# alshai/pfbwt-f

Hardware: AMD Instinct MI355X
Metric: Gbases/s end-to-end BWT+SA build; bit-exact .bwt/.sa vs reference (higher is better)
Workload: dtype u8 text / u32 indices / u64 hash; 1 GPU; S-32G; L=32000000, H=1000, seed=1000, w=10, p=100, flags=-r, uint_t=64, n=32000010000, r=83625322, input=text resident in HBM, outputs (.bwt, .ssa, .esa) left in HBM, per_rank=single GPU

## Files before the change

### include/pfbwt_hip_dev.h

```cpp
#ifndef PFBWT_HIP_DEV_H
#define PFBWT_HIP_DEV_H
#include "pfbwt_hip.h"

#ifdef __cplusplus
extern "C" {
#endif

int pfp_profile_enable(pfp_ctx *ctx, int on);
int pfp_profile_select(pfp_ctx *ctx, const char *kernel_name);
int pfp_profile_reset(pfp_ctx *ctx);
int pfp_profile_get(pfp_ctx *ctx, int idx, const char **name, uint64_t *launches, double *ms, double *bytes);
int pfp_stage_ms(pfp_ctx *ctx, double out[3]);
int pfp_debug_set(pfp_ctx *ctx, const char *key, long long value);
int pfp_debug_sort(pfp_ctx *ctx, uint64_t n, int bits, int reps, double *ms_out, uint32_t *unsorted_pairs);
int pfp_debug_checksum(pfp_ctx *ctx, const void *d_buf, uint64_t bytes, uint64_t global_offset, uint64_t out[2]);

int pfp_debug_check_sample_order(pfp_ctx *ctx, uint64_t out[5]);
int pfp_debug_check_sa(pfp_ctx *ctx, uint64_t out[5]);
int pfp_debug_check_samples(pfp_ctx *ctx, uint64_t out[3]);
int pfp_debug_rows_windowed(pfp_ctx *ctx, uint64_t window_rows, void *host_sa, void *host_lcp);
int pfp_debug_wordsum(pfp_ctx *ctx, const void *d_buf, uint64_t bytes, uint64_t out[2]);

#ifdef __cplusplus
}
#endif
#endif
```

### pfbwt-f_amd/csrc/common.h

```cpp
#pragma once
#include <hip/hip_runtime.h>
#include <cstdint>
#include <cstdio>
#include <cstdlib>
#include <cstring>
#include <chrono>
#include <string>
#include <vector>
#include "../../include/pfbwt_hip.h"
#include "devmem.h"
#include "../../include/pfbwt_hip_dev.h"

namespace pfp {

typedef uint32_t idx_t;

constexpr int BLOCK = 256;
constexpr int WAVE = 64;

constexpr uint8_t Dollar = 2, EndOfWord = 1, EndOfDict = 0;

enum KernelId {
    K_TRIGGER_SCAN, K_PHRASE_ENDS, K_PHRASE_HASH, K_PHRASE_HASH_LONG, K_DEDUP_HEADS, K_DEDUP_LONG,
    K_DICT_BUILD, K_RADIX_HIST, K_RADIX_SCATTER, K_SCAN_REDUCE, K_SCAN_SPINE, K_SCAN_APPLY,
    K_SS_INIT_KEYS, K_SS_HEADS, K_SS_MAKE_KEYS, K_SS_WRITE_RANK, K_SS_FLAG_ACTIVE, K_COMPACT,
    K_WORD_RANK, K_PARSE_RANKS, K_DICT_SORTED, K_PBWT_ROWS, K_EMIT_COUNT, K_EMIT, K_RUNS, K_SAMPLES, K_MISC, K_EMIT_BIG, K_FILL, K_CLASS_SORT, K_FASTA, K_EMIT_LARGE, K_REC_PARSE, K_REC_DEDUP, K_REC_ASSEMBLE, K_DOC, K_LCP_PAIRS, K_LCP_LONG, K_LCP_GATHER, K_THR_TILES, K_THR_QUERIES, K_THR_LONG, K_PLCP_BUILD, K_LCP_SPARSE, K_RUN_MASKS, K_MS_INDEX, K_MS_POINTERS, K_MS_BREAKS, K_MS_LONG, K_MS_FILL,
    K_COUNT_
};
static const char *const kernel_names[K_COUNT_] = {
    "trigger_scan", "phrase_ends", "phrase_hash", "phrase_hash_long", "dedup_heads", "dedup_long",
    "dict_build", "radix_hist", "radix_scatter", "scan_reduce", "scan_spine", "scan_apply",
    "ss_init_keys", "ss_heads", "ss_make_keys", "ss_write_rank", "ss_flag_active", "compact",
    "word_rank", "parse_ranks", "dict_sorted", "pbwt_rows", "emit_count", "emit", "runs", "samples", "misc", "emit_big", "fill", "class_sort", "fasta_strip", "emit_large", "rec_parse", "rec_dedup", "rec_assemble", "doc_array", "lcp_pairs", "lcp_long", "lcp_gather", "thr_tiles", "thr_queries", "thr_long", "plcp_build", "lcp_sparse", "run_masks", "ms_index", "ms_pointers", "ms_breaks", "ms_long", "ms_fill"};

struct ProfRec { uint64_t launches = 0; double ms = 0, bytes = 0; };

struct Arena {
    VmRegion vm;
    char *base = nullptr;
    size_t cap = 0, lo = 0, hi = 0, want = 0;
    size_t peak_lo = 0, peak_hi_bytes = 0;
    bool failed = false;
    void reset() { lo = 0; hi = cap; failed = false; }
    void *alloc_lo(size_t bytes)
    {
        size_t a = (lo + 255) & ~(size_t)255;
        if (a + bytes > hi || !vm.commit(a, a + bytes)) { failed = true; want += bytes; return nullptr; }
        lo = a + bytes; if (lo > peak_lo) peak_lo = lo;
        return base + a;
    }
    void *alloc_hi(size_t bytes)
    {
        size_t b = (bytes + 255) & ~(size_t)255;
        if (b > hi || hi - b < lo || !vm.commit(hi - b, hi)) { failed = true; want += bytes; return nullptr; }
        hi -= b; if (cap - hi > peak_hi_bytes) peak_hi_bytes = cap - hi;
        return base + hi;
    }
    void *reserve_lo(size_t bytes)
    {
        size_t a = (lo + 255) & ~(size_t)255;
        if (a + bytes > hi) { failed = true; want += bytes; return nullptr; }
        lo = a + bytes;
        return base + a;
    }
    bool commit_range(const void *p, size_t bytes) { const size_t o = (size_t)((const char *)p - base); return vm.commit(o, o + bytes); }
    size_t offset_of(const void *p) const { return (size_t)((const char *)p - base); }
    size_t mark_hi() const { return hi; }
    void release_hi(size_t m) { hi = m; }
    size_t mark_lo() const { return lo; }
    void release_lo(size_t m) { lo = m; }
};

struct ResultSlot {
    void *p[3] = {nullptr, nullptr, nullptr};
    size_t lo_mark = (size_t)-1, lo_end = 0;
};
struct MsIndex {
    void *thr = nullptr, *lfhead = nullptr; uint8_t *head = nullptr; uint32_t *sorted = nullptr, *sym = nullptr, *dir = nullptr;
    uint32_t B = 0;
};

struct Tunables {
    int verbose = 0;
    int seg_grid = 768;
    int seg_stage = 1;
    int sort_k = 0;
    int sort_no_table = 0;
    uint32_t class_sort_maxrange = 0;
    int dedup_table_log2 = 0;
    int no_trigger_table = 0;
    uint64_t emit_chunk_rows = 3ULL << 30;
    uint32_t fill_subs = 2;
    int fill_masks = 1;
    int fill_skip = 1;
    uint64_t sample_cap = ~0ULL;
    int no_runaware = 0;
    long big_group_members = -2;
    int force_wide_rows = 0;
    uint64_t ingest_block_bytes = 0;
    int expand_dma = 1;
    int ingest_readers = 0;
    uint32_t emit_group_rows = 4096;
    int dict_text_rounds = -1;
    int force_run_round = 0;
    int int_key_symbols = 3;
    int no_slot_records = 0;
    int group_reduce = 1;
    uint64_t fasta_chunk_bytes = 0;
    int parse_rec = -1;
    int parse_rec_p2 = 4;
    uint64_t parse_rec_min = 1u << 21;
    int parse_rec_depth = 1;
    uint32_t parse_rec_tile_rows = 0;
    int dict_rec = -1;
    int dict_rec_p2 = 16;
    int dedup_variant = -1;
    int64_t dedup_period = 0;
    int64_t dedup_chunk = 0;
    int dedup_packed = 1;
    int scan_waves = 16;
    int dedup_phases = 0;
    int parse_rec_table_log2 = 0;
    uint32_t doc_lds_max = 8192;
    uint32_t lcp_long_min = 512;
    uint32_t thr_long_min = 128;
    uint32_t thr_tile = 1024;
    uint64_t thr_window_rows = 1ULL << 30;
    int ms_dir_log2 = -1;
    uint32_t ms_long_min = 512;
    int plcp_block_log2 = -1;
};

}

struct pfp_ctx {
    int w = 10; uint64_t p = 100; unsigned flags = 0; int device = 0;
    hipStream_t stream = nullptr;
    pfp::Arena arena;
    size_t arena_request = 0;
    uint64_t err_pos = 0; int err_ch = 0;
    pfp::VmRegion text;
    uint8_t *tb = nullptr; size_t tb_cap = 0; uint64_t n = 0; uint64_t text_hint = 0; uint64_t nseq = 0 ;
    struct RowViewPending { const uint8_t *src = nullptr; uint64_t count = 0, len = 0, stride = 0; } view;
    uint64_t left_ctx = 0;
    uint64_t tb_n = 0;
    int stage = 0;
    uint64_t m = 0, dwords = 0, dsize = 0;
    uint64_t *d_ye = nullptr;
    uint32_t *d_pid = nullptr;
    uint32_t *d_parse = nullptr;
    uint8_t *d_last = nullptr;
    uint8_t *d_dict = nullptr;
    uint32_t *d_ws = nullptr;
    uint32_t *d_wordid = nullptr;
    uint32_t *d_wrank = nullptr;
    uint32_t *d_occ = nullptr;
    uint8_t *d_sdict = nullptr;
    uint32_t *d_gsa = nullptr;
    uint8_t *d_sflag = nullptr;
    uint32_t *d_srank = nullptr;
    uint2 *d_grank = nullptr;
    bool gsa_valid = false;
    uint64_t nrows = 0;
    uint8_t *d_bwlast = nullptr; uint32_t *d_ilist = nullptr; uint64_t *d_bwsai = nullptr;
    uint8_t *d_bwl_il = nullptr;
    uint64_t nout = 0, runs = 0, esa_pairs = 0, easy = 0, hard = 0, slice_begin = 0, slice_rows = 0;
    uint8_t *d_bwt = nullptr; void *d_sa = nullptr; void *d_ssa = nullptr; void *d_esa = nullptr;
    bool have_sa = false, have_rssa = false;
    pfp::ResultSlot ma; uint64_t ma_words = 0;
    pfp::ResultSlot da;
    pfp::ResultSlot lcp;
    pfp::ResultSlot thr;
    pfp::ResultSlot msi; pfp::MsIndex msx;
    pfp::ResultSlot ms; uint64_t ms_patterns = 0, ms_bases = 0;
    std::vector<uint64_t> ms_off;
    size_t lo_after_parse = 0, lo_after_pbwt = 0, emit_scratch_mark = 0;
    bool prof_on = false; uint64_t prof_mask = ~0ULL;
    pfp::ProfRec prof[pfp::K_COUNT_];
    struct PendingEv { hipEvent_t a, b; int id; double bytes; };
    std::vector<PendingEv> pending;
    std::vector<hipEvent_t> ev_pool;
    double stage_ms[3] = {0, 0, 0};
    int hip_err = 0;
    uint8_t *hstage[2] = {nullptr, nullptr}; hipEvent_t hstage_ev[2] = {nullptr, nullptr}; bool hstage_used[2] = {false, false};
    pfp::Tunables tun;
    struct FastaIngest {
        uint8_t *raw[2] = {nullptr, nullptr}; size_t rawcap = 0; bool used[2] = {false, false};
        hipStream_t copy = nullptr; bool copy_ready = false; hipEvent_t ev_copied[2] = {nullptr, nullptr}, ev_free[2] = {nullptr, nullptr};
        uint8_t *tiles = nullptr; size_t tiles_cap = 0;
        unsigned long long *d_tot = nullptr, *h_tot = nullptr;
        uint32_t state = 2; bool started = false; uint64_t records = 0;
        std::vector<uint64_t> rec_raw, rec_pos;
    } fa;
    uint8_t *h_bwt = nullptr; void *h_sa = nullptr;
    uint8_t *ing_buf[16] = {};
    uint64_t ing_next_off = 0;
    std::vector<std::string> doc_names; std::vector<uint64_t> doc_starts;
    uint64_t hash_seed = 0x9E3779B97F4A7C15ULL;
    int num_cus = 0;
    uint32_t *d_trigtab = nullptr;
};

namespace pfp {

inline hipEvent_t ev_get(pfp_ctx *c)
{
    if (!c->ev_pool.empty()) { hipEvent_t e = c->ev_pool.back(); c->ev_pool.pop_back(); return e; }
    hipEvent_t e; (void)hipEventCreate(&e); return e;
}
inline void prof_collect(pfp_ctx *c)
{
    if (c->pending.empty()) return;
    (void)hipStreamSynchronize(c->stream);
    for (auto &pe : c->pending) {
        float ms = 0; (void)hipEventElapsedTime(&ms, pe.a, pe.b);
        c->prof[pe.id].launches++; c->prof[pe.id].ms += ms; c->prof[pe.id].bytes += pe.bytes;
        c->ev_pool.push_back(pe.a); c->ev_pool.push_back(pe.b);
    }
    c->pending.clear();
}
struct ProfScope {
    pfp_ctx *c; int id; double bytes; hipEvent_t a = nullptr; bool on = false;
    ProfScope(pfp_ctx *c_, int id_, double bytes_) : c(c_), id(id_), bytes(bytes_)
    {
        on = c->prof_on && ((c->prof_mask >> id) & 1ULL);
        if (on) { a = ev_get(c); (void)hipEventRecord(a, c->stream); }
    }
    ~ProfScope()
    {
        if (on) {
            hipEvent_t b = ev_get(c); (void)hipEventRecord(b, c->stream);
            c->pending.push_back({a, b, id, bytes});
            if (c->pending.size() > 4096) prof_collect(c);
        }
    }
};

#define PFP_LAUNCH(ctx, id, bytes, kernel, grid, ...)                                             \
    do {                                                                                          \
        pfp::ProfScope ps_((ctx), (id), (double)(bytes));                                         \
        if ((ctx)->tun.verbose >= 3) { fprintf(stderr, "[pfbwt_hip] launch %s grid %u\n", #kernel, (unsigned)(grid)); fflush(stderr); } \
        hipLaunchKernelGGL(kernel, dim3((unsigned)(grid)), dim3(pfp::BLOCK), 0, (ctx)->stream, __VA_ARGS__); \
        hipError_t le_ = hipGetLastError();             \
        if ((ctx)->tun.verbose >= 3 && le_ == hipSuccess) le_ = hipStreamSynchronize((ctx)->stream);    \
        if (le_ != hipSuccess) { (ctx)->hip_err = (int)le_; (ctx)->err_ch = (int)le_;                 \
            fprintf(stderr, "[pfbwt_hip] launch of %s failed: %s (%s:%d)\n", #kernel, hipGetErrorString(le_), __FILE__, __LINE__); \
            return PFP_E_HIP; }                                                                       \
    } while (0)

#define PFP_LAUNCH_B(ctx, id, bytes, kernel, grid, block, ...)                                    \
    do {                                                                                          \
        pfp::ProfScope ps_((ctx), (id), (double)(bytes));                                         \
        hipLaunchKernelGGL(kernel, dim3((unsigned)(grid)), dim3((unsigned)(block)), 0, (ctx)->stream, __VA_ARGS__); \
        hipError_t le_ = hipGetLastError();                                                       \
        if (le_ != hipSuccess) { (ctx)->hip_err = (int)le_; (ctx)->err_ch = (int)le_;                 \
            fprintf(stderr, "[pfbwt_hip] launch of %s failed: %s (%s:%d)\n", #kernel, hipGetErrorString(le_), __FILE__, __LINE__); \
            return PFP_E_HIP; }                                                                       \
    } while (0)

#define PFP_HIP(ctx, expr)                                                                        \
    do {                                                                                          \
        hipError_t e_ = (expr);                                                                   \
        if (e_ != hipSuccess) { (ctx)->hip_err = (int)e_; (ctx)->err_ch = (int)e_;                \
            fprintf(stderr, "[pfbwt_hip] %s failed: %s (%s:%d)\n", #expr, hipGetErrorString(e_), __FILE__, __LINE__); \
            return PFP_E_HIP; }                                                                   \
    } while (0)

#define PFP_TRY(expr) do { int rc_ = (expr); if (rc_ != PFP_OK) return rc_; } while (0)

#define PFP_ALLOC_HI(ctx, ptr, T, count)                                                          \
    do { (ptr) = (T *)(ctx)->arena.alloc_hi(sizeof(T) * (size_t)((count) ? (count) : 1));         \
         if (!(ptr)) return PFP_E_NOMEM; } while (0)
#define PFP_ALLOC_LO(ctx, ptr, T, count)                                                          \
    do { (ptr) = (T *)(ctx)->arena.alloc_lo(sizeof(T) * (size_t)((count) ? (count) : 1));         \
         if (!(ptr)) return PFP_E_NOMEM; } while (0)

inline unsigned nblocks(uint64_t items, uint64_t per_block) { return (unsigned)((items + per_block - 1) / per_block); }
inline int bits_for(uint64_t maxval) { int b = 1; while (b < 64 && (maxval >> b)) ++b; return b; }

struct PostResult {
    pfp_ctx *c; ResultSlot &s; size_t mark;
    PostResult(pfp_ctx *c_, ResultSlot &s_) : c(c_), s(s_)
    {
        if (s.lo_mark != (size_t)-1 && c->arena.lo == s.lo_end) c->arena.release_lo(s.lo_mark);
        s = ResultSlot();
        mark = c->arena.mark_lo();
    }
    void commit(void *p0, void *p1 = nullptr, void *p2 = nullptr) { s.p[0] = p0; s.p[1] = p1; s.p[2] = p2; s.lo_mark = mark; s.lo_end = c->arena.mark_lo(); }
};
inline void drop_post_results(pfp_ctx *c) { c->ma = c->da = c->lcp = c->thr = c->msi = c->ms = ResultSlot(); c->ma_words = 0; c->msx = MsIndex(); c->ms_patterns = c->ms_bases = 0; c->ms_off.clear(); }

struct HostTimer {
    std::chrono::steady_clock::time_point t0 = std::chrono::steady_clock::now();
    double ms() const { return std::chrono::duration<double, std::milli>(std::chrono::steady_clock::now() - t0).count(); }
};

}
```

### pfbwt-f_amd/csrc/emit.h

```cpp
#pragma once
#include "prims.h"
#include "parse.h"

namespace pfp {

__global__ __launch_bounds__(BLOCK) void k_pbwt_pack(const uint32_t *P, const uint8_t *last, const tpos_t *sai, uint64_t m, uint4 *rec)
{
    const uint64_t j = (uint64_t)blockIdx.x * BLOCK + threadIdx.x;
    if (j >= m) return;
    const uint64_t v = sai ? (uint64_t)sai[j] : 0ULL;
    rec[j] = make_uint4((uint32_t)v, (uint32_t)(v >> 32), P[j], (uint32_t)last[j ? j - 1 : m - 1]);
}
constexpr int BWL_SHIFT = 29;
__device__ __forceinline__ uint32_t bwl_code(uint32_t c) { return c == 0 ? 0u : c == Dollar ? 1u : c == '-' ? 2u : c == 'A' ? 3u : c == 'C' ? 4u : c == 'G' ? 5u : c == 'N' ? 6u : c == 'T' ? 7u : 8u; }
__device__ __forceinline__ uint8_t bwl_byte(uint32_t code) { return code == 0 ? (uint8_t)0 : code == 1 ? Dollar : code == 2 ? (uint8_t)'-' : code == 3 ? (uint8_t)'A' : code == 4 ? (uint8_t)'C' : code == 5 ? (uint8_t)'G' : code == 6 ? (uint8_t)'N' : (uint8_t)'T'; }
__global__ __launch_bounds__(BLOCK) void k_pbwt_rows(const uint32_t *SAP, const uint4 *rec, uint64_t m, uint8_t *bwlast, tpos_t *bwsai, uint32_t *W, uint32_t *rowid, int pack, uint32_t *bad)
{
    const uint64_t i = (uint64_t)blockIdx.x * BLOCK + threadIdx.x;
    if (i > m) return;
    const uint32_t s = SAP[i];
    if (s == 0) { bwlast[i] = 0; if (bwsai) bwsai[i] = 0; W[i] = 0; rowid[i] = (uint32_t)i; return; }
    const uint4 R = rec[s - 1];
    bwlast[i] = (uint8_t)R.w;
    if (bwsai) bwsai[i] = (tpos_t)(((uint64_t)R.y << 32) | R.x);
    W[i] = R.z;
    uint32_t id = (uint32_t)i;
    if (pack) { const uint32_t code = bwl_code(R.w & 0xFFu); if (code > 7u) *bad = 1u; else id |= code << BWL_SHIFT; }
    rowid[i] = id;
}
__global__ __launch_bounds__(BLOCK) void k_ilist_split(const uint32_t *packed, uint64_t n, uint32_t *ilist, uint8_t *bwl_il)
{
    const uint64_t k = (uint64_t)blockIdx.x * BLOCK + threadIdx.x;
    if (k >= n) return;
    const uint32_t v = packed[k];
    ilist[k] = v & ((1u << BWL_SHIFT) - 1u); bwl_il[k] = bwl_byte(v >> BWL_SHIFT);
}
__global__ __launch_bounds__(BLOCK) void k_bwsai_by_ilist(const uint32_t *ilist, const tpos_t *bwsai, uint64_t n, tpos_t *out)
{
    const uint64_t k = (uint64_t)blockIdx.x * BLOCK + threadIdx.x;
    if (k < n) out[k] = bwsai[ilist[k]];
}
__global__ __launch_bounds__(BLOCK) void k_ilist_gather(const uint32_t *packed, uint64_t n, uint32_t mask, const uint8_t *bwlast, uint32_t *ilist, uint8_t *bwl_il)
{
    const uint64_t k = (uint64_t)blockIdx.x * BLOCK + threadIdx.x;
    if (k >= n) return;
    const uint32_t q = packed[k] & mask;
    ilist[k] = q; bwl_il[k] = bwlast[q];
}

__global__ __launch_bounds__(BLOCK) void k_u32_add_store(const uint32_t *in, uint64_t n, uint32_t add, uint32_t *out)
{
    const uint64_t i = (uint64_t)blockIdx.x * BLOCK + threadIdx.x;
    if (i < n) out[i] = in[i] + add;
}

__global__ __launch_bounds__(BLOCK) void k_wordstart_keys(const uint32_t *ws, const uint2 *grank, uint64_t dwords, uint32_t *keys, uint32_t *vals)
{
    const uint64_t id = (uint64_t)blockIdx.x * BLOCK + threadIdx.x;
    if (id >= dwords) return;
    keys[id] = grank[ws[id]].x; vals[id] = (uint32_t)id;
}
__global__ __launch_bounds__(BLOCK) void k_word_rank(const uint32_t *sorted_ids, uint64_t dwords, const uint32_t *occw, uint32_t *wrank, uint32_t *idofrank, uint32_t *occ)
{
    const uint64_t r = (uint64_t)blockIdx.x * BLOCK + threadIdx.x;
    if (r >= dwords) return;
    const uint32_t id = sorted_ids[r];
    wrank[id] = (uint32_t)r; idofrank[r] = id; occ[r] = occw[id];
}
constexpr int WF_PER_THREAD = 16, WF_TILE = BLOCK * WF_PER_THREAD;
__device__ __forceinline__ uint32_t wf_mask16(const uint8_t *sflag, uint64_t i0, uint64_t n)
{
    uint32_t m = 0;
#pragma unroll
    for (int k = 0; k < WF_PER_THREAD; ++k) if (i0 + k < n && sflag[i0 + k]) m |= 1u << k;
    return m;
}
__global__ __launch_bounds__(BLOCK) void k_flag_tile_count(const uint8_t *sflag, uint64_t n, uint32_t *tilecnt)
{
    __shared__ uint32_t red[4];
    const uint64_t i0 = ((uint64_t)blockIdx.x * BLOCK + threadIdx.x) * WF_PER_THREAD;
    uint32_t tot;
    (void)block_excl_sum((uint32_t)__popc(wf_mask16(sflag, i0, n)), red, &tot);
    if (threadIdx.x == 0) tilecnt[blockIdx.x] = tot;
}
__global__ __launch_bounds__(BLOCK) void k_word_rank_flags(const uint8_t *sflag, const uint32_t *tilebase, const uint32_t *SA, const uint32_t *wordid, uint64_t dsize, uint32_t dwords,
                                                         const uint32_t *occw, uint32_t *wrank, uint32_t *idofrank, uint32_t *occ)
{
    __shared__ uint32_t red[4];
    const uint64_t i0 = ((uint64_t)blockIdx.x * BLOCK + threadIdx.x) * WF_PER_THREAD;
    uint32_t m = wf_mask16(sflag, i0, dsize), tot;
    uint32_t r = tilebase[blockIdx.x] + block_excl_sum((uint32_t)__popc(m), red, &tot);
    while (m) {
        const int k = __ffs((int)m) - 1; m &= m - 1;
        const uint32_t id = wordid[SA[i0 + k]];
        if (r < dwords && id < dwords) { wrank[id] = r; idofrank[r] = id; occ[r] = occw[id]; }
        ++r;
    }
}
__global__ __launch_bounds__(BLOCK) void k_parse_ranks(const uint32_t *pid, const uint32_t *wrank, uint64_t m, uint32_t *parse)
{
    const uint64_t j = (uint64_t)blockIdx.x * BLOCK + threadIdx.x;
    if (j < m) parse[j] = wrank[pid[j]] + 1u;
}
__global__ __launch_bounds__(BLOCK) void k_sorted_lengths(const uint32_t *ws, const uint32_t *idofrank, uint64_t dwords, uint32_t *len1, tpos_t *srcstart)
{
    const uint64_t r = (uint64_t)blockIdx.x * BLOCK + threadIdx.x;
    if (r >= dwords) return;
    const uint32_t id = idofrank[r];
    len1[r] = ws[id + 1] - ws[id]; srcstart[r] = ws[id];
}

__global__ __launch_bounds__(BLOCK) void k_eow_flags(const uint8_t *D, uint64_t dsize, uint32_t *flag)
{
    const uint64_t x = (uint64_t)blockIdx.x * BLOCK + threadIdx.x;
    if (x < dsize) flag[x] = D[x] == EndOfWord ? 1u : 0u;
}
__global__ __launch_bounds__(BLOCK) void k_ws_from_flags(const uint8_t *D, uint64_t dsize, const uint32_t *wordid, uint32_t *ws)
{
    const uint64_t x = (uint64_t)blockIdx.x * BLOCK + threadIdx.x;
    if (x >= dsize) return;
    if (x == 0) ws[0] = 0;
    if (D[x] == EndOfWord) ws[wordid[x] + 1] = (uint32_t)x + 1u;
}

struct EmitArgs {
    const uint8_t *D = nullptr; uint64_t dsize = 0; uint32_t dwords = 0; int w = 0;
    const uint32_t *SA = nullptr, *ws = nullptr, *wrank = nullptr , *occ = nullptr, *F = nullptr, *ilist = nullptr;
    const uint32_t *srank = nullptr;
    const tpos_t *bwsai = nullptr;
    const uint2 *posinfo = nullptr;
    const uint4 *prec = nullptr;
    const uint32_t *wordid = nullptr;
    int use_prec = 0;
    int use_e0 = 0;
    const uint4 *winfo = nullptr;
    const uint8_t *bwlast = nullptr;
    const uint8_t *bwl_il = nullptr;
    const tpos_t *bwsai_il = nullptr;
    const void *EB = nullptr;
    const uint32_t *s_sl = nullptr;
    const uint32_t *s_fb = nullptr;
    const uint8_t *s_fl = nullptr;
    const uint8_t *s_pc = nullptr;
    const uint32_t *s_g0 = nullptr;
    const uint32_t *gk = nullptr;
    const void *cnt = nullptr;
    const uint4 *sinfo = nullptr;
    const uint32_t *tile_slot = nullptr;
    uint64_t *big_keys = nullptr; uint32_t *big_vals = nullptr; unsigned long long *big_count = nullptr;
    uint64_t big_cap = 0, big_total = 0;
    uint64_t nout = 0, n = 0;
    uint64_t e0 = 0, e1 = 0;
    uint64_t w0 = 0, w1 = 0;
    const void *ENB = nullptr; const uint32_t *etile_slot = nullptr, *elist = nullptr, *cpos = nullptr; uint32_t ecount = 0; int special = 0; uint64_t q0 = 0;
    const uint32_t *qspec = nullptr;
    const uint32_t *gqf = nullptr, *gql = nullptr;
    uint8_t *gleft = nullptr, *tile_left = nullptr; uint32_t group_rows_cap = 0; uint32_t rank_members_max = 0;
    const uint4 *cinfo = nullptr;
    const unsigned long long *cgb = nullptr;
    const uint32_t *town = nullptr;
    uint32_t *lglist = nullptr; unsigned long long *lgcount = nullptr; uint64_t lgcap = 0; int qpasses = 0 ;
    unsigned long long *gstat = nullptr;
};
constexpr uint8_t SF_MULTI = 1, SF_FULL = 2, SF_BIG = 4, SF_GFULL = 8, SF_NONUNI = 16, SF_E0 = 32;
__device__ __forceinline__ bool slot_is_special(uint32_t fl) { return (fl & (SF_FULL | SF_GFULL | SF_NONUNI)) != 0; }
constexpr int EG_SLOTS = 2 * BLOCK;
constexpr uint32_t BIG_GROUP_MEMBERS = 64;
constexpr uint32_t WID_MASK = 0x0FFFFFFFu;
__device__ __forceinline__ uint32_t dict_code4(uint32_t c) { return c <= 2 ? c : (c == '-') ? 3u : (c == 'A') ? 4u : (c == 'C') ? 5u : (c == 'G') ? 6u : (c == 'N') ? 7u : 8u; }
__device__ __forceinline__ uint8_t dict_byte4(uint32_t code) { return code <= 2 ? (uint8_t)code : code == 3 ? (uint8_t)'-' : code == 4 ? (uint8_t)'A' : code == 5 ? (uint8_t)'C' : code == 6 ? (uint8_t)'G' : code == 7 ? (uint8_t)'N' : (uint8_t)'T'; }
__global__ __launch_bounds__(BLOCK) void k_pack_winfo(const uint32_t *ws, const uint32_t *wrank , const uint32_t *occ, const uint32_t *F, uint64_t dwords, uint4 *winfo)
{
    const uint64_t id = (uint64_t)blockIdx.x * BLOCK + threadIdx.x;
    if (id >= dwords) return;
    const uint32_t rk = wrank ? wrank[id] : (uint32_t)id;
    winfo[id] = make_uint4(ws[id], ws[id + 1] - 1u, F[rk], occ[rk]);
}
__global__ __launch_bounds__(BLOCK) void k_pack_posinfo(const uint8_t *D, const uint32_t *wordid, uint64_t dsize, uint2 *posinfo)
{
    const uint64_t x = (uint64_t)blockIdx.x * BLOCK + threadIdx.x;
    if (x >= dsize) return;
    posinfo[x] = make_uint2(wordid[x] | (dict_code4(x ? D[x - 1] : 0u) << 28), 0u);
}

constexpr uint32_t PREC_SL_BITS = 26, PREC_FULL = 1u << 30, PREC_VALID = 1u << 31;
__global__ __launch_bounds__(BLOCK) void k_pack_prec(const uint8_t *D, const uint32_t *wordid, const uint4 *winfo, uint64_t dsize, uint32_t dwords, uint4 *prec, const tpos_t *bwsai_il )
{
    const uint64_t x = (uint64_t)blockIdx.x * BLOCK + threadIdx.x;
    if (x >= dsize) return;
    const uint32_t id = wordid[x];
    uint4 R = make_uint4(0u, 0u, 0u, 0u);
    if (id < dwords) {
        const uint4 W = winfo[id];
        uint32_t code = 0, full = 0;
        if ((uint32_t)x == W.x) full = PREC_FULL;
        else { code = dict_code4(D[x - 1]); if (code == Dollar && (uint32_t)x - 1u == W.x) code = 0; }
        R.y = W.z; R.z = W.w; R.w = (W.y - (uint32_t)x) | (code << PREC_SL_BITS) | full | PREC_VALID;
        if (bwsai_il) { if (W.w == 1u) R.x = (uint32_t)bwsai_il[W.z]; }
        else R.x = id;
    }
    prec[x] = R;
}
__global__ __launch_bounds__(BLOCK) void k_pack_wpq(const uint32_t *ilist, const uint32_t *wrank , const uint32_t *occ, const uint32_t *F, uint64_t dwords, uint2 *wpq)
{
    const uint64_t id = (uint64_t)blockIdx.x * BLOCK + threadIdx.x;
    if (id >= dwords) return;
    const uint32_t rk = wrank ? wrank[id] : (uint32_t)id, o = occ[rk], f = F[rk];
    wpq[id] = o ? make_uint2(ilist[f], ilist[f + o - 1u]) : make_uint2(~0u, 0u);
}
__global__ __launch_bounds__(BLOCK) void k_max_word_length(const uint32_t *ws, uint64_t dwords, uint32_t *out)
{
    __shared__ uint32_t red[4];
    const uint64_t id = (uint64_t)blockIdx.x * BLOCK + threadIdx.x;
    uint32_t tot;
    (void)block_incl_max(id < dwords ? ws[id + 1] - ws[id] : 0u, red, &tot);
    if (threadIdx.x == 0) atomicMax(out, tot);
}

__device__ __forceinline__ uint32_t word_rank_of(const EmitArgs &a, uint32_t id) { return a.wrank ? a.wrank[id] : id; }

template <typename T> __device__ __forceinline__ uint32_t upper_bound_t(const T *a, uint32_t n, T x)
{
    uint32_t lo = 0, hi = n;
    while (lo < hi) { uint32_t mid = lo + ((hi - lo) >> 1); if (a[mid] <= x) lo = mid + 1; else hi = mid; }
    return lo;
}

template <typename EBT> __global__ __launch_bounds__(BLOCK) void k_emit_slots(EmitArgs a, EBT *cnt, unsigned long long *hard_rows, uint32_t *s_sl, uint32_t *s_fb, uint8_t *s_fl, uint8_t *s_pc,
                                                                             uint32_t *s_g0, uint32_t *gk , uint8_t *gfl ,
                                                                             uint8_t *gnu ,
                                                                             const uint2 *wpq , uint32_t *gqf, uint32_t *gql)
{
    __shared__ uint8_t hd[BLOCK + 1];
    __shared__ uint8_t pcl[BLOCK + 1];
    __shared__ uint32_t red[4];
    const uint64_t i = (uint64_t)blockIdx.x * BLOCK + threadIdx.x;
    const bool valid = i < a.dsize;
    uint32_t x = 0; uint2 P = make_uint2(0, 0); uint4 R = make_uint4(0, 0, 0, 0);
    if (valid) { x = a.SA[i]; if (a.prec) R = a.prec[x]; else P = a.posinfo[x]; P.y = a.srank[i]; }
    hd[threadIdx.x] = (valid && P.y == (uint32_t)i) ? 1 : 0;
    if (threadIdx.x == 0) {
        const uint64_t nx = (uint64_t)(blockIdx.x + 1) * BLOCK;
        uint8_t h = 1, hp = 0xFF;
        if (nx < a.dsize) {
            const uint32_t xn = a.SA[nx];
            if (a.prec) {
                const uint4 Rn = a.prec[xn];
                h = a.srank[nx] == (uint32_t)nx ? 1 : 0;
                if (!h && (Rn.w & PREC_VALID) && !(Rn.w & PREC_FULL)) hp = dict_byte4((Rn.w >> PREC_SL_BITS) & 15u);
            } else {
            const uint2 Pn = a.posinfo[xn];
            h = a.srank[nx] == (uint32_t)nx ? 1 : 0;
            if (!h) {
                const uint32_t idn = Pn.x & WID_MASK;
                if (idn < a.dwords) {
                    const uint32_t wsn = a.winfo[idn].x;
                    if (xn != wsn) { hp = dict_byte4(Pn.x >> 28); if (hp == Dollar && xn - 1 == wsn) hp = 0; }
                }
            }
            }
        }
        hd[BLOCK] = h; pcl[BLOCK] = hp;
    }
    __syncthreads();
    uint32_t c = 0, sl = 0, fb = 0; uint8_t fl = 0, pc = 0;
    if (a.prec) {
        if (valid && (R.w & PREC_VALID)) {
            sl = R.w & ((1u << PREC_SL_BITS) - 1u);
            if (sl > (uint32_t)a.w) {
                c = R.z; fb = R.y;
                if (!hd[threadIdx.x] || (i + 1 < a.dsize && !hd[threadIdx.x + 1])) fl |= SF_MULTI;
                if (R.w & PREC_FULL) fl |= SF_FULL; else pc = dict_byte4((R.w >> PREC_SL_BITS) & 15u);
                if (a.use_e0 && c == 1u && !(fl & SF_MULTI)) { fl |= SF_E0; P.y = R.x; }
            }
        }
    } else {
    const uint32_t id = P.x & WID_MASK;
    if (valid && id < a.dwords) {
        const uint4 W = a.winfo[id];
        const uint32_t wsid = W.x;
        sl = W.y - x;
        if (sl > (uint32_t)a.w) {
            c = W.w; fb = W.z;
            if (!hd[threadIdx.x] || (i + 1 < a.dsize && !hd[threadIdx.x + 1])) fl |= SF_MULTI;
            if (x == wsid) fl |= SF_FULL;
            else { pc = dict_byte4(P.x >> 28); if (pc == Dollar && x - 1 == wsid) pc = 0; }
        }
    }
    }
    pcl[threadIdx.x] = (fl & SF_FULL) ? (uint8_t)0xFF : pc;
    __syncthreads();
    if (valid) {
        cnt[i] = (EBT)c; s_sl[i] = sl; s_fb[i] = fb; s_fl[i] = fl; s_pc[i] = pc; s_g0[i] = P.y;
        if (fl & SF_MULTI) {
            const bool lastm = i + 1 >= a.dsize || hd[threadIdx.x + 1];
            if (lastm) gk[P.y] = (uint32_t)i - P.y + 1u;
            if (fl & SF_FULL) gfl[P.y] = 1;
            else if (!lastm && pcl[threadIdx.x + 1] != 0xFF && pcl[threadIdx.x + 1] != pc) gnu[P.y] = 1;
        }
    }
    if (wpq && !(a.prec && a.use_e0)) {
        __shared__ uint32_t wk0[BLOCK / WAVE], wkl[BLOCK / WAVE], wmn[BLOCK / WAVE], wmx[BLOCK / WAVE];
        __shared__ uint8_t wef[BLOCK / WAVE], wsp[BLOCK / WAVE];
        const int lane = (int)(threadIdx.x & (WAVE - 1)), wv = (int)(threadIdx.x / WAVE);
        const bool part = (fl & SF_MULTI) != 0;
        uint32_t key = ~0u, mn = ~0u, mx = 0u, ef = 0u;
        if (part) {
            const uint2 q = wpq[a.prec ? R.x : (P.x & WID_MASK)];
            key = P.y; mn = q.x; mx = q.y; ef = (i + 1 >= a.dsize || hd[threadIdx.x + 1]) ? 1u : 0u;
        }
        for (int d = 1; d < WAVE; d <<= 1) {
            const uint32_t k2 = __shfl_down(key, (unsigned)d), n2 = __shfl_down(mn, (unsigned)d), x2 = __shfl_down(mx, (unsigned)d), e2 = __shfl_down(ef, (unsigned)d);
            if (lane + d < WAVE && k2 == key) { mn = n2 < mn ? n2 : mn; mx = x2 > mx ? x2 : mx; ef = e2; }
        }
        const uint32_t klast = __shfl(key, WAVE - 1), kprev = __shfl_up(key, 1u);
        if (lane == 0) { wk0[wv] = key; wmn[wv] = mn; wmx[wv] = mx; wef[wv] = (uint8_t)ef; wsp[wv] = key == klast ? 1 : 0; }
        if (lane == WAVE - 1) wkl[wv] = key;
// ... 228 lines not shown
    const uint32_t lo = a.tile_slot[tb], hi = a.tile_slot[tb + 1];
    return lo + upper_bound_t<EBT>(EB + lo, hi - lo + 1u, (EBT)o) - 1u;
}

template <typename SAT, typename EBT> __global__ __launch_bounds__(BLOCK) void k_emit(EmitArgs a, uint8_t *bwt, SAT *sa, uint32_t *qrow )
{
    __shared__ uint32_t eb[EMIT_LDS_SLOTS];
    __shared__ uint32_t rs[EMIT_TILE];
    __shared__ uint32_t red[4];
    const EBT *EB = reinterpret_cast<const EBT *>(a.EB);
    const EBT *ENB = reinterpret_cast<const EBT *>(a.ENB);
    if (a.tile_left && !a.tile_left[blockIdx.x]) return;
    const uint64_t tb = a.e0 / EMIT_TILE + blockIdx.x;
    const uint64_t o0 = tb * EMIT_TILE > a.e0 ? tb * EMIT_TILE : a.e0;
    const uint64_t o1 = ((tb + 1) * EMIT_TILE < a.e1) ? (tb + 1) * EMIT_TILE : a.e1;
    const uint32_t i0 = a.etile_slot[tb], i1 = a.etile_slot[tb + 1];
    const uint32_t ns = i1 - i0 + 1u;
    const uint64_t ebase = (uint64_t)ENB[i0];
    const bool in_lds = ns <= (uint32_t)EMIT_LDS_SLOTS && o1 - ebase < 0xFFFFFFFFULL;
    if (in_lds) for (uint32_t k = threadIdx.x; k < ns; k += BLOCK) eb[k] = (uint32_t)((uint64_t)ENB[i0 + k] - ebase);
    for (int k = threadIdx.x; k < EMIT_TILE; k += BLOCK) rs[k] = 0;
    __syncthreads();
    if (in_lds) {
        const uint32_t rel0 = (uint32_t)(o0 - ebase), nrow = (uint32_t)(o1 - o0);
        for (uint32_t t = threadIdx.x; t < ns; t += BLOCK) {
            const uint32_t e = eb[t];
            if (e <= rel0) atomicMax(&rs[0], t);
            else if (e - rel0 < nrow) atomicMax(&rs[e - rel0], t);
        }
        __syncthreads();
        uint32_t loc[EMIT_PER_THREAD], run = 0;
#pragma unroll
        for (int j = 0; j < EMIT_PER_THREAD; ++j) { const uint32_t v = rs[threadIdx.x * EMIT_PER_THREAD + j]; run = v > run ? v : run; loc[j] = run; }
        uint32_t tot;
        const uint32_t inc = block_incl_max(run, red, &tot);
        uint32_t prev = __shfl_up(inc, 1);
        if ((threadIdx.x & 63) == 0) prev = 0;
        __shared__ uint32_t wmax[BLOCK / WAVE];
        if ((threadIdx.x & 63) == 63) wmax[threadIdx.x >> 6] = inc;
        __syncthreads();
        if ((threadIdx.x & 63) == 0 && threadIdx.x) prev = wmax[(threadIdx.x >> 6) - 1];
#pragma unroll
        for (int j = 0; j < EMIT_PER_THREAD; ++j) rs[threadIdx.x * EMIT_PER_THREAD + j] = loc[j] > prev ? loc[j] : prev;
        __syncthreads();
    }
#pragma unroll 1
    for (int k = 0; k < EMIT_PER_THREAD; k += EMIT_ROWS_IN_FLIGHT) {
        uint64_t o[EMIT_ROWS_IN_FLIGHT]; uint32_t i[EMIT_ROWS_IN_FLIGHT], r[EMIT_ROWS_IN_FLIGHT], q[EMIT_ROWS_IN_FLIGHT];
        uint4 S[EMIT_ROWS_IN_FLIGHT]; uint8_t fl[EMIT_ROWS_IN_FLIGHT]; bool on[EMIT_ROWS_IN_FLIGHT]; uint64_t sv[EMIT_ROWS_IN_FLIGHT];
#pragma unroll
        for (int u = 0; u < EMIT_ROWS_IN_FLIGHT; ++u) {
            o[u] = o0 + (uint64_t)(k + u) * BLOCK + threadIdx.x;
            on[u] = o[u] < o1;
            const uint64_t oo = on[u] ? o[u] : o0;
            if (in_lds) { const uint32_t j = rs[(uint32_t)(oo - o0)]; i[u] = i0 + j; r[u] = (uint32_t)(oo - ebase) - eb[j]; }
            else { i[u] = upper_bound_t<EBT>(ENB, a.ecount, (EBT)oo) - 1u; r[u] = (uint32_t)(oo - (uint64_t)ENB[i[u]]); }
        }
        uint32_t jc[EMIT_ROWS_IN_FLIGHT];
#pragma unroll
        for (int u = 0; u < EMIT_ROWS_IN_FLIGHT; ++u) jc[u] = i[u];
        if (a.elist) {
#pragma unroll
            for (int u = 0; u < EMIT_ROWS_IN_FLIGHT; ++u) i[u] = a.elist[i[u]];
        }
#pragma unroll
        for (int u = 0; u < EMIT_ROWS_IN_FLIGHT; ++u) { S[u] = a.sinfo[i[u]]; fl[u] = (uint8_t)(S[u].w >> 24); }
        if (a.gleft) {
#pragma unroll
            for (int u = 0; u < EMIT_ROWS_IN_FLIGHT; ++u) {
                const uint32_t jh = (fl[u] & SF_MULTI) ? jc[u] - (i[u] - S[u].z) : jc[u];
                if (on[u] && !a.gleft[jh]) on[u] = false;
            }
        }
#pragma unroll
        for (int u = 0; u < EMIT_ROWS_IN_FLIGHT; ++u) {
            const bool needq = (fl[u] & SF_MULTI) || qrow || ((fl[u] & SF_FULL) && !a.bwl_il) || (sa && !a.bwsai_il);
            q[u] = needq ? a.ilist[S[u].x + r[u]] : 0u;
        }
#pragma unroll
        for (int u = 0; u < EMIT_ROWS_IN_FLIGHT; ++u) sv[u] = (sa && on[u] && !(fl[u] & SF_BIG)) ? ((fl[u] & SF_E0) ? (uint64_t)S[u].z : a.bwsai_il ? (uint64_t)a.bwsai_il[S[u].x + r[u]] : (uint64_t)a.bwsai[q[u]]) : 0ULL;
        uint32_t before[EMIT_ROWS_IN_FLIGHT], gk_[EMIT_ROWS_IN_FLIGHT], maxk = 0;
#pragma unroll
        for (int u = 0; u < EMIT_ROWS_IN_FLIGHT; ++u) {
            const bool plain = on[u] && (fl[u] & SF_MULTI) && !(fl[u] & (SF_GFULL | SF_BIG));
            gk_[u] = plain ? (S[u].w & 0xFFFFFFu) : 0u; before[u] = 0;
            maxk = gk_[u] > maxk ? gk_[u] : maxk;
        }
        for (uint32_t s0 = 0; s0 < maxk; s0 += EMIT_RANK_W) {
            uint32_t mem[EMIT_ROWS_IN_FLIGHT * EMIT_RANK_W], qq[EMIT_ROWS_IN_FLIGHT * EMIT_RANK_W], res[EMIT_ROWS_IN_FLIGHT * EMIT_RANK_W];
#pragma unroll
            for (int u = 0; u < EMIT_ROWS_IN_FLIGHT; ++u)
#pragma unroll
                for (int j = 0; j < EMIT_RANK_W; ++j) {
                    const uint32_t s = S[u].z + s0 + j;
                    mem[u * EMIT_RANK_W + j] = (s0 + j < gk_[u] && s != i[u]) ? s : ~0u; qq[u * EMIT_RANK_W + j] = q[u];
                }
            rank_lists<EMIT_ROWS_IN_FLIGHT * EMIT_RANK_W>(a, mem, qq, res);
#pragma unroll
            for (int u = 0; u < EMIT_ROWS_IN_FLIGHT; ++u)
#pragma unroll
                for (int j = 0; j < EMIT_RANK_W; ++j) before[u] += res[u * EMIT_RANK_W + j];
        }
#pragma unroll
        for (int u = 0; u < EMIT_ROWS_IN_FLIGHT; ++u) {
            const bool self_full = (fl[u] & SF_FULL) != 0;
            uint64_t pos = o[u];
            bool full_emits_eow = false;
            const bool big = on[u] && (fl[u] & SF_BIG) != 0;
            {
                const unsigned long long bm = __ballot(big);
                if (bm) {
                    const int lane = threadIdx.x & 63, leader = __ffsll((long long)bm) - 1;
                    unsigned long long basei = 0;
                    if (lane == leader) basei = atomicAdd(a.big_count, (unsigned long long)__popcll(bm));
                    basei = __shfl(basei, leader);
                    if (big) {
                        const unsigned long long idx = basei + (unsigned long long)__popcll(bm & (lane ? (~0ULL >> (64 - lane)) : 0ULL));
                        if (idx < a.big_cap) { a.big_keys[idx] = ((uint64_t)S[u].z << 32) | q[u]; a.big_vals[idx] = i[u]; }
                        else a.big_count[1] = 1;
                    }
                }
            }
            if (!on[u] || big) continue;
            uint32_t g = i[u];
            if (fl[u] & SF_GFULL) { pos = multi_group_pos<EBT>(a, i[u], r[u], q[u], self_full, &full_emits_eow); g = S[u].z; }
            else if (fl[u] & SF_MULTI) { pos = (uint64_t)EB[S[u].z] + before[u] + r[u]; g = S[u].z; }
            else if (a.special) pos = (uint64_t)EB[i[u]] + r[u];
            if (a.special && qrow) qrow[(uint64_t)ENB[a.cpos[g]] - a.q0 + (pos - (uint64_t)EB[g])] = q[u];
            const uint8_t c = self_full ? (full_emits_eow ? (uint8_t)EndOfWord : a.bwl_il ? a.bwl_il[S[u].x + r[u]] : a.bwlast[q[u]]) : a.s_pc[i[u]];
            if (pos < a.w0 || pos >= a.w1) continue;
            bwt[pos - a.w0] = c;
            if (sa) {
                SAT v = (SAT)((SAT)sv[u] - (SAT)a.s_sl[i[u]]);
                if (pos == 0) v = (SAT)a.n;
                sa[pos - a.w0] = v;
            }
            if (qrow && !a.special) qrow[pos - a.w0] = q[u];
        }
    }
}

constexpr int EG_BUF = 4096, EG_PER_THREAD = EG_BUF / BLOCK;
constexpr int EG1_BUF = 8192, EG2_BUF = 16384;
__device__ __forceinline__ uint32_t group_members(const EmitArgs &a, const uint4 &S) { const uint32_t k = S.w & 0xFFFFFFu; return k == 0xFFFFFFu ? a.gk[S.z] : k; }
template <typename EBT> __global__ __launch_bounds__(BLOCK) void k_special_pack(EmitArgs a, uint32_t nsp, uint4 *cinfo, unsigned long long *cgb)
{
    const uint64_t j = (uint64_t)blockIdx.x * BLOCK + threadIdx.x;
    if (j >= nsp) return;
    const uint32_t i = a.elist[j]; const uint4 S = a.sinfo[i];
    const uint32_t fl = S.w >> 24; const bool multi = (fl & SF_MULTI) != 0;
    cinfo[j] = make_uint4(S.x, multi ? group_members(a, S) : 1u, multi ? i - S.z : 0u, (uint32_t)a.s_pc[i] | (fl << 8));
    cgb[j] = (unsigned long long)reinterpret_cast<const EBT *>(a.EB)[multi ? S.z : i];
}
template <typename EBT> __device__ __forceinline__ uint64_t group_start_at_or_after(const EBT *ENB, const uint4 *cinfo, uint64_t nsp, uint64_t lo, uint64_t v)
{
    while (lo < nsp && (uint64_t)ENB[lo] < v) ++lo;
    if (lo >= nsp) return nsp;
    const uint4 ci = cinfo[lo];
    if (!((ci.w >> 8) & SF_MULTI)) return lo;
    const uint64_t head = lo - ci.z;
    return (uint64_t)ENB[head] < v ? head + ci.y : head;
}
template <typename EBT> __global__ __launch_bounds__(BLOCK) void k_tile_own(const EBT *ENB, const uint4 *cinfo, const uint32_t *etile_slot, uint64_t nsp, uint64_t ntiles, uint32_t *town)
{
    const uint64_t t = (uint64_t)blockIdx.x * BLOCK + threadIdx.x;
    if (t > ntiles) return;
    town[t] = (uint32_t)group_start_at_or_after<EBT>(ENB, cinfo, nsp, etile_slot[t], t * EMIT_TILE);
}
template <typename EBT> __global__ __launch_bounds__(BLOCK) void k_emit_groups(EmitArgs a, uint8_t *bwt, uint32_t *qrow)
{
    __shared__ uint32_t LQ[EG_BUF];
    __shared__ uint32_t s_eb[EG_SLOTS + 1], s_fb[EG_SLOTS], s_kf[EG_SLOTS], s_dl[EG_SLOTS];
    __shared__ uint64_t s_ob[EG_SLOTS];
    __shared__ uint8_t s_pc[EG_SLOTS];
    __shared__ uint32_t red[4];
    __shared__ uint64_t jb[2];
    const EBT *ENB = reinterpret_cast<const EBT *>(a.ENB);
    const uint64_t tile0 = a.e0 / EMIT_TILE, tb = tile0 + blockIdx.x;
    const uint64_t o0 = tb * EMIT_TILE > a.e0 ? tb * EMIT_TILE : a.e0;
    const uint64_t o1 = ((tb + 1) * EMIT_TILE < a.e1) ? (tb + 1) * EMIT_TILE : a.e1;
    if (threadIdx.x < 2) {
        const uint64_t v = threadIdx.x ? o1 : o0;
        const uint64_t tv = threadIdx.x ? tb + 1 : tb;
        uint64_t j;
        if (v == tv * EMIT_TILE) j = a.town[tv];
        else {
            uint64_t lo = a.etile_slot[tb], hi = (uint64_t)a.etile_slot[tb + 1] + 1u;
            if (hi > a.ecount) hi = a.ecount;
            if (lo > hi) lo = hi;
            while (lo < hi) { const uint64_t mid = lo + ((hi - lo) >> 1); if ((uint64_t)ENB[mid] < v) lo = mid + 1; else hi = mid; }
            j = group_start_at_or_after<EBT>(ENB, a.cinfo, a.ecount, lo, v);
        }
        jb[threadIdx.x] = j;
    }
    __syncthreads();
    uint64_t j = jb[0]; const uint64_t jE = jb[1];
    const uint32_t cap = a.group_rows_cap < (uint32_t)EG_BUF ? a.group_rows_cap : (uint32_t)EG_BUF;
    while (j < jE) {
        const uint32_t nload = jE - j < (uint64_t)EG_SLOTS ? (uint32_t)(jE - j) : (uint32_t)EG_SLOTS;
        const uint64_t B0 = (uint64_t)ENB[j];
        uint32_t cand[2] = {0u, 0u}, bad = 0xFFFFFFFFu;
#pragma unroll
        for (int t = 0; t < 2; ++t) {
            const uint32_t s = threadIdx.x + (uint32_t)t * BLOCK;
            if (s < nload) {
                const uint4 ci = a.cinfo[j + s];
                const uint32_t fl = ci.w >> 8, dl = ci.z, k = ci.y;
                const uint64_t e0 = (uint64_t)ENB[j + s] - B0, e1 = (uint64_t)ENB[j + s + 1] - B0;
                s_eb[s] = e0 < 0xFFFFFFFFull ? (uint32_t)e0 : 0xFFFFFFFFu;
                if (s + 1 == nload) s_eb[nload] = e1 < 0xFFFFFFFFull ? (uint32_t)e1 : 0xFFFFFFFFu;
                s_fb[s] = ci.x; s_kf[s] = (k < 0xFFFFFFu ? k : 0xFFFFFFu) | (fl << 24); s_dl[s] = dl; s_pc[s] = (uint8_t)ci.w;
                s_ob[s] = (uint64_t)a.cgb[j + s];
                if (((fl & (SF_GFULL | SF_BIG)) || k > a.rank_members_max) && s < bad) bad = s;
                if (dl + 1u == k && e1 <= (uint64_t)cap) cand[t] = s + 1u;
            }
        }
        uint32_t tot;
        (void)block_incl_max(~bad, red, &tot);
        const uint32_t firstbad = ~tot;
        uint32_t c = 0;
#pragma unroll
        for (int t = 0; t < 2; ++t) if (cand[t] && cand[t] <= firstbad && cand[t] > c) c = cand[t];
        uint32_t cut;
        (void)block_incl_max(c, red, &cut);
        if (cut == 0) {
            const uint32_t k0 = a.cinfo[j].y;
            const uint64_t r0 = B0, r1 = (uint64_t)ENB[j + k0];
            {
                const uint32_t f0 = s_kf[0] >> 24;
                if (threadIdx.x == 0) {
                    unsigned long long idx = ~0ULL;
                    if (a.lglist && (f0 & SF_MULTI) && !(f0 & (SF_GFULL | SF_BIG)) && k0 <= (uint32_t)EG_SLOTS && r1 - r0 <= (uint64_t)EG2_BUF) {
                        const int big = r1 - r0 > (uint64_t)EG1_BUF ? 1 : 0;
                        idx = atomicAdd(a.lgcount + big, 1ULL);
                        if (idx < a.lgcap) a.lglist[(uint64_t)big * a.lgcap + idx] = (uint32_t)j;
                    }
                    jb[0] = idx < a.lgcap ? 1 : 0;
                }
                __syncthreads();
                const bool taken = jb[0] != 0;
                __syncthreads();
                if (taken) { j += k0; continue; }
            }
            if (threadIdx.x == 0) a.gleft[j] = 1;
            if (a.gstat && threadIdx.x == 0) {
                const uint32_t f0 = s_kf[0] >> 24;
                atomicAdd(&a.gstat[(f0 & SF_GFULL) ? 0 : (f0 & SF_BIG) ? 1 : (r1 - r0 > (uint64_t)cap) ? 2 : 3], (unsigned long long)(r1 - r0));
                int b = 0; while (b < 7 && (1024ull << (2 * b)) <= r1 - r0) ++b;
                atomicAdd(&a.gstat[4 + b], (unsigned long long)(r1 - r0));
            }
            if (r1 > r0) for (uint64_t t = r0 / EMIT_TILE + threadIdx.x; t <= (r1 - 1) / EMIT_TILE; t += BLOCK) a.tile_left[t - tile0] = 1;
            j += k0;
            __syncthreads();
            continue;
        }
        __syncthreads();
        const uint32_t nrows = s_eb[cut];
#pragma unroll
        for (int t = 0; t < 2; ++t) { const uint32_t s = threadIdx.x + (uint32_t)t * BLOCK; if (s < cut) s_ob[s] -= (uint64_t)s_eb[s - s_dl[s]]; }
        uint32_t qv[EG_PER_THREAD], sv[EG_PER_THREAD]; uint8_t cv[EG_PER_THREAD];
#pragma unroll
        for (int it = 0; it < EG_PER_THREAD; ++it) {
            const uint32_t r = threadIdx.x + (uint32_t)it * BLOCK;
            sv[it] = 0; qv[it] = 0; cv[it] = 0;
            if (r < nrows) {
                const uint32_t s = upper_bound_t<uint32_t>(s_eb, cut, r) - 1u, at = s_fb[s] + (r - s_eb[s]);
                sv[it] = s; qv[it] = a.ilist[at];
                if (!((s_kf[s] >> 24) & SF_MULTI) && a.bwl_il) cv[it] = a.bwl_il[at];
            }
        }
#pragma unroll
        for (int it = 0; it < EG_PER_THREAD; ++it) {
            const uint32_t r = threadIdx.x + (uint32_t)it * BLOCK;
            if (r < nrows) { LQ[r] = qv[it]; const uint32_t fl = s_kf[sv[it]] >> 24; if (fl & SF_MULTI) cv[it] = s_pc[sv[it]]; else if (!a.bwl_il) cv[it] = a.bwlast[qv[it]]; }
        }
        __syncthreads();
#pragma unroll
        for (int it = 0; it < EG_PER_THREAD; ++it) {
            const uint32_t r = threadIdx.x + (uint32_t)it * BLOCK;
            if (r < nrows) {
                const uint32_t s = sv[it], kf = s_kf[s];
                uint32_t pos = r;
                if ((kf >> 24) & SF_MULTI) {
                    const uint32_t sh = s - s_dl[s], k = kf & 0xFFFFFFu, q = qv[it];
                    uint32_t before = 0;
                    for (uint32_t mm = 0; mm < k; ++mm) {
                        const uint32_t sm = sh + mm;
                        if (sm != s) before += lower_bound_u32(LQ + s_eb[sm], s_eb[sm + 1] - s_eb[sm], q);
                    }
                    pos = s_eb[sh] + before + (r - s_eb[s]);
                }
                if (qrow) qrow[B0 - a.q0 + pos] = qv[it];
                const uint64_t o = s_ob[s] + pos;
                if (o >= a.w0 && o < a.w1) bwt[o - a.w0] = cv[it];
            }
        }
        __syncthreads();
        j += cut;
    }
}

template <int ITEMS> __device__ __forceinline__ void lds_sort_pairs_u32(uint32_t *keys, uint16_t *vals, uint32_t n, int npass, uint32_t (*wh)[RS_RADIX], uint32_t *red)
{
    const int lane = threadIdx.x & 63, wave = threadIdx.x >> 6;
    const uint32_t nit = (n + BLOCK - 1) / BLOCK;
    for (uint32_t j = n + threadIdx.x; j < nit * BLOCK; j += BLOCK) { keys[j] = 0xFFFFFFFFu; vals[j] = 0; }
    const uint32_t base = (uint32_t)wave * (nit * WAVE) + lane;
    for (int p = 0; p < npass; ++p) {
        const int sh = 8 * p;
        uint32_t k[ITEMS], dg[ITEMS]; uint16_t v[ITEMS];
#pragma unroll
        for (int w = 0; w < BLOCK / WAVE; ++w) wh[w][threadIdx.x] = 0;
        __syncthreads();
#pragma unroll
        for (int it = 0; it < ITEMS; ++it) {
            if ((uint32_t)it < nit) {
                const uint32_t i = base + (uint32_t)it * WAVE;
                k[it] = keys[i]; v[it] = vals[i];
                const uint32_t d = (k[it] >> sh) & 255u;
                uint32_t plo = 0xFFFFFFFFu, phi = 0xFFFFFFFFu;
                same_digit_lanes(d, plo, phi);
                const int leader = plo ? __builtin_ctz(plo) : 32 + __builtin_ctz(phi);
                uint32_t old = 0;
                if (lane == leader) { old = wh[wave][d]; wh[wave][d] = old + (uint32_t)__builtin_popcount(plo) + (uint32_t)__builtin_popcount(phi); }
                old = __shfl(old, leader);
                dg[it] = d | ((old + __builtin_amdgcn_mbcnt_hi(phi, __builtin_amdgcn_mbcnt_lo(plo, 0u))) << 8);
            }
        }
        __syncthreads();
        {
            const unsigned d = threadIdx.x;
            uint32_t cw[BLOCK / WAVE]; uint32_t total = 0;
#pragma unroll
            for (int w = 0; w < BLOCK / WAVE; ++w) { cw[w] = wh[w][d]; total += cw[w]; }
            uint32_t tt;
            uint32_t run = block_excl_sum(total, red, &tt);
#pragma unroll
            for (int w = 0; w < BLOCK / WAVE; ++w) { wh[w][d] = run; run += cw[w]; }
        }
        __syncthreads();
#pragma unroll
        for (int it = 0; it < ITEMS; ++it) {
            if ((uint32_t)it < nit) { const uint32_t li = wh[wave][dg[it] & 255u] + (dg[it] >> 8); keys[li] = k[it]; vals[li] = v[it]; }
        }
        __syncthreads();
    }
}
template <typename EBT, int BUF> __global__ __launch_bounds__(BLOCK) void k_emit_groups_large(EmitArgs a, uint8_t *bwt, uint32_t *qrow)
{
    __shared__ uint32_t LQ[BUF];
    __shared__ uint16_t LS[BUF];
    __shared__ uint32_t wh[BLOCK / WAVE][RS_RADIX];
    __shared__ uint32_t s_eb[EG_SLOTS + 1], s_fb[EG_SLOTS];
    __shared__ uint8_t s_pc[EG_SLOTS];
    __shared__ uint32_t red[4];
    const EBT *ENB = reinterpret_cast<const EBT *>(a.ENB);
    constexpr int WHICH = BUF > EG1_BUF ? 1 : 0;
    const unsigned long long have = a.lgcount[WHICH];
    const uint64_t cnt = have < a.lgcap ? have : a.lgcap;
    for (uint64_t g = blockIdx.x; g < cnt; g += gridDim.x) {
        const uint64_t j = a.lglist[(uint64_t)WHICH * a.lgcap + g];
        const uint32_t k = a.cinfo[j].y;
        const uint64_t B0 = (uint64_t)ENB[j], outbase = (uint64_t)a.cgb[j];
        for (uint32_t s = threadIdx.x; s < k; s += BLOCK) {
            const uint4 ci = a.cinfo[j + s];
            s_eb[s] = (uint32_t)((uint64_t)ENB[j + s] - B0); s_fb[s] = ci.x; s_pc[s] = (uint8_t)ci.w;
            if (s + 1 == k) s_eb[k] = (uint32_t)((uint64_t)ENB[j + k] - B0);
        }
        __syncthreads();
        const uint32_t nrows = s_eb[k];
        for (uint32_t r = threadIdx.x; r < nrows; r += BLOCK) { const uint32_t s = upper_bound_t<uint32_t>(s_eb, k, r) - 1u; LQ[r] = a.ilist[s_fb[s] + (r - s_eb[s])]; LS[r] = (uint16_t)s; }
        __syncthreads();
        lds_sort_pairs_u32<BUF / BLOCK>(LQ, LS, nrows, a.qpasses, wh, red);
        for (uint32_t r = threadIdx.x; r < nrows; r += BLOCK) {
            if (qrow) qrow[B0 - a.q0 + r] = LQ[r];
            const uint64_t o = outbase + r;
            if (o >= a.w0 && o < a.w1) bwt[o - a.w0] = s_pc[LS[r]];
        }
        __syncthreads();
    }
}

template <typename EBT> __global__ __launch_bounds__(BLOCK) void k_slice_bounds(EmitArgs a, uint64_t lo, uint64_t hi, unsigned long long *out)
{
    if (blockIdx.x != 0 || threadIdx.x != 0) return;
    const EBT *EB = reinterpret_cast<const EBT *>(a.EB);
    const EBT *ENB = reinterpret_cast<const EBT *>(a.ENB);
    const uint32_t il = slot_of_row<EBT>(a, lo);
    const uint32_t gh = (a.s_fl[il] & SF_MULTI) ? a.s_g0[il] : il;
    out[0] = EB[gh];
    out[2] = a.special ? (unsigned long long)ENB[a.cpos[gh]] : 0ULL;
    out[4] = a.special ? (unsigned long long)a.cpos[gh] : 0ULL;
    if (hi >= a.nout) { out[1] = a.nout; out[3] = a.special ? (unsigned long long)ENB[a.ecount] : 0ULL; out[5] = a.special ? (unsigned long long)a.ecount : 0ULL; return; }
    uint32_t s = slot_of_row<EBT>(a, hi - 1);
    if (a.s_fl[s] & SF_MULTI) { const uint32_t g = a.s_g0[s]; while (s < a.dsize && (a.s_fl[s] & SF_MULTI) && a.s_g0[s] == g) ++s; }
    else ++s;
    {
        uint64_t lo_ = s, hi_ = a.dsize;
        while (lo_ < hi_) { const uint64_t mid = lo_ + ((hi_ - lo_) >> 1); if ((uint64_t)EB[mid] < hi) lo_ = mid + 1; else hi_ = mid; }
        s = (uint32_t)lo_;
    }
    out[1] = s < a.dsize ? (uint64_t)EB[s] : a.nout;
    const uint32_t js = a.special ? (s < a.dsize ? a.cpos[s] : a.ecount) : 0u;
    out[3] = a.special ? (unsigned long long)ENB[js] : 0ULL; out[5] = js;
}

#ifndef PFP_FILL_NT
#define PFP_FILL_NT 0
#endif
__device__ __forceinline__ void fill_store16(uint8_t *dst, uint32_t x0, uint32_t x1, uint32_t x2, uint32_t x3)
{
#if PFP_FILL_NT && !defined(PFBWT_EMU_HIP_RUNTIME_H)
    typedef uint32_t fill_v4u __attribute__((ext_vector_type(4)));
    fill_v4u v = {x0, x1, x2, x3};
    __builtin_nontemporal_store(v, reinterpret_cast<fill_v4u *>(dst));
#else
    *reinterpret_cast<uint4 *>(dst) = make_uint4(x0, x1, x2, x3);
#endif
}
constexpr int FILL_PER_THREAD = 16, FILL_SUB = BLOCK * FILL_PER_THREAD;
constexpr int FILL_GROUPS = 4;
constexpr uint32_t FILL_MAX_SUBS = 8;
static_assert(FILL_SUB % EMIT_TILE == 0, "fill tiles are whole emission tiles");
__device__ __forceinline__ uint32_t run_bits16(uint64_t lo, uint64_t hi, uint64_t prev)
{
    const uint64_t xl = lo ^ ((lo << 8) | prev), xh = hi ^ ((hi << 8) | (lo >> 56));
    uint32_t m = 0;
#pragma unroll
    for (int b = 0; b < 8; ++b) { m |= ((xl >> (8 * b)) & 0xff) ? (1u << b) : 0u; m |= ((xh >> (8 * b)) & 0xff) ? (1u << (8 + b)) : 0u; }
    return m;
}
template <typename EBT, bool MASKS> __global__ __launch_bounds__(BLOCK) void k_fill(EmitArgs a, uint8_t *bwt, uint32_t subs_per_wg, int skip, uint16_t *rmask, uint64_t mrow0)
{
    __shared__ uint32_t eb[FILL_SUB + 2];
    __shared__ uint8_t pcs[FILL_SUB + 2];
    __shared__ uint32_t wcnt[BLOCK / WAVE];
    __shared__ uint32_t sts[FILL_MAX_SUBS * FILL_GROUPS + 1];
    const EBT *EB = reinterpret_cast<const EBT *>(a.EB);
    const EBT *cnt = reinterpret_cast<const EBT *>(a.cnt);
    const uint64_t ntiles = (a.nout + EMIT_TILE - 1) / EMIT_TILE;
    constexpr uint64_t TPS = FILL_SUB / EMIT_TILE;
    constexpr uint64_t SUPER = (uint64_t)FILL_GROUPS * FILL_SUB;
    const uint64_t st0 = a.w0 / SUPER + (uint64_t)blockIdx.x * subs_per_wg;
    const int lane = threadIdx.x & 63, wave = threadIdx.x >> 6;
    const unsigned long long lt = lane ? (~0ULL >> (64 - lane)) : 0ULL;
    for (uint32_t k = threadIdx.x; k <= subs_per_wg * FILL_GROUPS; k += BLOCK) {
        const uint64_t t = (st0 * FILL_GROUPS + k) * TPS;
        sts[k] = a.tile_slot[t < ntiles ? t : ntiles];
    }
    __syncthreads();
    auto compact = [&](uint32_t i0, uint32_t i1, uint64_t base) -> uint32_t {
        const uint32_t ns = i1 - i0 + 1u;
        uint32_t nz = 0;
        for (uint32_t k0 = 0; k0 < ns;) {
            const uint32_t k = k0 + threadIdx.x;
            const EBT cn = k < ns ? cnt[i0 + k] : (EBT)0;
            const uint64_t e = k < ns ? (uint64_t)EB[i0 + k] : 0ULL;
            const uint8_t pc = k < ns ? a.s_pc[i0 + k] : (uint8_t)0;
            const bool has = cn != 0;
            const unsigned long long bal = __ballot(has);
            __syncthreads();
            if (lane == 0) wcnt[wave] = (uint32_t)__popcll(bal);
            __syncthreads();
            uint32_t pos = nz, tot = 0;
#pragma unroll
            for (int v = 0; v < BLOCK / WAVE; ++v) { const uint32_t cw = wcnt[v]; if (v < wave) pos += cw; tot += cw; }
            if (nz + tot > (uint32_t)FILL_SUB + 1u) return ~0u;
            if (has) { pos += (uint32_t)__popcll(bal & lt); eb[pos] = e > base ? (uint32_t)(e - base) : 0u; pcs[pos] = pc; }
            nz += tot;
            uint32_t kn = k0 + (uint32_t)BLOCK;
            if (skip && tot == 0 && kn < ns) {
                const EBT v = EB[i0 + k0];
                uint32_t lo_ = kn, hi_ = ns;
                while (hi_ - lo_ > 1u) { const uint32_t mid = lo_ + ((hi_ - lo_) >> 1); if (EB[i0 + mid] == v) lo_ = mid; else hi_ = mid; }
                kn = lo_;
            }
            k0 = kn;
        }
        if (threadIdx.x == 0) eb[nz] = 0xFFFFFFFFu;
        __syncthreads();
        return nz;
    };
    auto write_group = [&](uint64_t g0, uint64_t base, uint32_t nz) {
        const uint64_t o0 = g0 > a.w0 ? g0 : a.w0;
        const uint64_t o1 = g0 + FILL_SUB < a.w1 ? g0 + FILL_SUB : a.w1;
        const uint64_t ra = g0 + (uint64_t)threadIdx.x * FILL_PER_THREAD;
        const uint64_t lo = ra > o0 ? ra : o0, hi = ra + FILL_PER_THREAD < o1 ? ra + FILL_PER_THREAD : o1;
        if (lo >= hi) return;
        uint32_t wd[FILL_PER_THREAD / 4] = {0, 0, 0, 0};
        uint32_t rel = (uint32_t)(lo - base);
        uint32_t s = upper_bound_t<uint32_t>(eb, nz, rel) - 1u;
        uint32_t nxt = eb[s + 1], c = pcs[s];
        [[maybe_unused]] uint32_t pvb = 0, mk = 0;
        if constexpr (MASKS) pvb = rel > eb[s] ? c : s ? (uint32_t)pcs[s - 1u] : 0u;
        if (lo == ra && hi == ra + FILL_PER_THREAD && nxt >= rel + FILL_PER_THREAD) {
            wd[0] = wd[1] = wd[2] = wd[3] = c * 0x01010101u;
            if constexpr (MASKS) mk = pvb != c ? 1u : 0u;
        } else {
#pragma unroll
            for (int j = 0; j < FILL_PER_THREAD; ++j) {
                const uint64_t o = ra + j;
                if (o >= lo && o < hi) {
                    while (rel >= nxt) { ++s; nxt = eb[s + 1]; c = pcs[s]; }
                    wd[j >> 2] |= c << (8 * (j & 3));
                    ++rel;
                }
            }
            if constexpr (MASKS) mk = run_bits16((uint64_t)wd[0] | ((uint64_t)wd[1] << 32), (uint64_t)wd[2] | ((uint64_t)wd[3] << 32), (uint64_t)pvb);
        }
        uint8_t *dst = bwt + (ra - a.w0);
        if constexpr (MASKS) { if (lo == ra && hi == ra + FILL_PER_THREAD && ra >= mrow0) rmask[(ra - mrow0) / FILL_PER_THREAD] = (uint16_t)mk; }
        if (lo == ra && hi == ra + FILL_PER_THREAD) fill_store16(dst, wd[0], wd[1], wd[2], wd[3]);
        else for (uint64_t o = lo; o < hi; ++o) { const int j = (int)(o - ra); dst[j] = (uint8_t)(wd[j >> 2] >> (8 * (j & 3))); }
    };
    for (uint32_t ss = 0; ss < subs_per_wg; ++ss) {
        const uint64_t tstart = (st0 + ss) * SUPER;
        if (tstart >= a.w1) break;
        const uint64_t tend = tstart + SUPER < a.w1 ? tstart + SUPER : a.w1;
        const uint32_t ng = (uint32_t)((tend - tstart + FILL_SUB - 1) / FILL_SUB);
        const uint32_t *gs = sts + ss * FILL_GROUPS;
        uint32_t nz = compact(gs[0], gs[ng], tstart);
        if (nz != ~0u) {
            for (uint32_t g = 0; g < ng; ++g) write_group(tstart + (uint64_t)g * FILL_SUB, tstart, nz);
        } else {
            for (uint32_t g = 0; g < ng; ++g) {
                const uint64_t g0 = tstart + (uint64_t)g * FILL_SUB;
                nz = compact(gs[g], gs[g + 1], g0);
                write_group(g0, g0, nz);
            }
        }
    }
}

__global__ __launch_bounds__(BLOCK) void k_run_count(const uint8_t *bwt, uint64_t nout, int has_prev, unsigned long long *runs)
{
    __shared__ uint32_t red[4];
    const uint64_t o0 = ((uint64_t)blockIdx.x * BLOCK + threadIdx.x) * 16;
    uint32_t cntr = 0;
    if (o0 < nout) {
        uint8_t prev = (o0 || has_prev) ? *(bwt + o0 - 1) : (uint8_t)0;
        for (int k = 0; k < 16 && o0 + k < nout; ++k) { const uint8_t cc = bwt[o0 + k]; cntr += cc != prev; prev = cc; }
    }
    uint32_t tot;
    (void)block_excl_sum(cntr, red, &tot);
    if (threadIdx.x == 0 && tot) atomicAdd(runs, (unsigned long long)tot);
}
constexpr int RUN_PER_THREAD = 16, RUN_TILE = BLOCK * RUN_PER_THREAD;
__device__ __forceinline__ uint32_t run_mask16(const uint8_t *bwt, uint64_t j0, uint64_t rows, int has_prev)
{
    if (j0 >= rows) return 0;
    const uint64_t lo = ld8(bwt + j0), hi = ld8(bwt + j0 + 8);
    const uint64_t prev = (j0 || has_prev) ? (uint64_t)*(bwt + j0 - 1) : 0ULL;
    const uint32_t m = run_bits16(lo, hi, prev);
    const uint64_t left = rows - j0;
    return left >= 16 ? m : (m & ((1u << left) - 1u));
}
__global__ __launch_bounds__(BLOCK) void k_run_tile_count(const uint8_t *bwt, uint64_t rows, int has_prev, uint32_t *tilecnt, uint16_t *rmask)
{
    __shared__ uint32_t red[4];
    const uint64_t g = (uint64_t)blockIdx.x * BLOCK + threadIdx.x;
    const uint32_t m = run_mask16(bwt, g * RUN_PER_THREAD, rows, has_prev);
    if (rmask) rmask[g] = (uint16_t)m;
    uint32_t tot;
    (void)block_excl_sum((uint32_t)__popc(m), red, &tot);
    if (threadIdx.x == 0) tilecnt[blockIdx.x] = tot;
}
template <typename EBT> __global__ __launch_bounds__(BLOCK) void k_run_masks_fix(EmitArgs a, const uint8_t *bwt, uint64_t cs, uint64_t rows, int has_prev, uint64_t j0, uint64_t j1, uint32_t nsb, uint16_t *rmask)
{
    __shared__ uint32_t pcx[BLOCK + 1];
    __shared__ uint64_t pf[BLOCK];
    __shared__ uint32_t red[4];
    const uint64_t npieces = (rows + RUN_PER_THREAD - 1) / RUN_PER_THREAD, ce = cs + rows;
    if (blockIdx.x >= nsb) {
        const uint64_t t = (uint64_t)(blockIdx.x - nsb) * BLOCK + threadIdx.x;
        uint64_t p = 0;
        if (t == 1) p = npieces - 1;
        else if (t > 1) {
            const uint64_t r = (cs / FILL_SUB + (t - 1)) * FILL_SUB;
            if (r >= ce) return;
            p = (r - cs) / RUN_PER_THREAD;
        }
        rmask[p] = (uint16_t)run_mask16(bwt, p * RUN_PER_THREAD, rows, has_prev);
        return;
    }
    const EBT *ENB = reinterpret_cast<const EBT *>(a.ENB);
    const uint64_t j = j0 + (uint64_t)blockIdx.x * BLOCK + threadIdx.x;
    uint32_t np = 0; uint64_t first = 0;
    if (j < j1) {
        uint64_t head, gb; uint32_t k;
        if (a.cinfo) { const uint4 ci = a.cinfo[j]; head = j - ci.z; k = ci.y; gb = (uint64_t)a.cgb[j]; }
        else {
            const uint32_t i = a.elist[j]; const uint4 S = a.sinfo[i]; const bool multi = ((S.w >> 24) & SF_MULTI) != 0;
            head = multi ? (uint64_t)a.cpos[S.z] : j; k = multi ? group_members(a, S) : 1u; gb = (uint64_t)reinterpret_cast<const EBT *>(a.EB)[multi ? S.z : i];
        }
        if (head == j && j + k <= (uint64_t)a.ecount) {
            const uint64_t ge = gb + ((uint64_t)ENB[j + k] - (uint64_t)ENB[j]);
            if (ge > gb && ge >= cs && gb < ce) {
                const uint64_t r0 = gb > cs ? gb : cs, r1 = ge < ce - 1 ? ge : ce - 1;
                first = (r0 - cs) / RUN_PER_THREAD; np = (uint32_t)((r1 - cs) / RUN_PER_THREAD - first + 1);
            }
        }
    }
    uint32_t tot;
    pcx[threadIdx.x] = block_excl_sum(np, red, &tot); pf[threadIdx.x] = first;
    __syncthreads();
    for (uint32_t t = threadIdx.x; t < tot; t += BLOCK) {
        const uint32_t s = upper_bound_t<uint32_t>(pcx, BLOCK, t) - 1u;
        const uint64_t p = pf[s] + (t - pcx[s]);
        rmask[p] = (uint16_t)run_mask16(bwt, p * RUN_PER_THREAD, rows, has_prev);
    }
}
// ... 84 lines not shown
```

### pfbwt-f_amd/csrc/emit_host.h

```cpp
#pragma once

__global__ __launch_bounds__(BLOCK) void k_flag_special(const uint8_t *s_fl, uint64_t dsize, uint32_t *flag)
{
    const uint64_t i = (uint64_t)blockIdx.x * BLOCK + threadIdx.x;
    if (i < dsize) flag[i] = slot_is_special(s_fl[i]) ? 1u : 0u;
}
template <typename EBT> __global__ __launch_bounds__(BLOCK) void k_gather_counts(const EBT *cnt, const uint32_t *list, uint64_t n, EBT *out)
{
    const uint64_t j = (uint64_t)blockIdx.x * BLOCK + threadIdx.x;
    if (j < n) out[j] = cnt[list[j]];
}

struct EmitVisit { uint64_t window_rows; std::function<int(uint64_t first_row, uint64_t rows, const void *d_sa_window)> fn; };
struct EmitWin { uint64_t cs, ce, cl, e0, e1, q0, q1, j0, j1; };
static uint64_t slice_first_row(uint64_t total, int slice, int nslices)
{
    const uint64_t k = (uint64_t)nslices, s = (uint64_t)slice;
    return total / k * s + (total % k) * s / k;
}
static void print_left_rows(const unsigned long long *d_gstat)
{
    unsigned long long h[12];
    if (hipMemcpy(h, d_gstat, 96, hipMemcpyDeviceToHost) != hipSuccess) return;
    fprintf(stderr, "[pfbwt_hip] special rows left to the row-wise kernel (counted once per window that enumerates them): whole-word member %llu, sort route %llu, too many rows %llu, too many slots %llu; by group rows (<1K <4K <16K <64K <256K <1M <4M more):",
            h[0], h[1], h[2], h[3]);
    for (int b = 0; b < 8; ++b) fprintf(stderr, " %llu", h[4 + b]);
    fprintf(stderr, "\n");
}

template <typename SAT, typename EBT> struct Emission {
    pfp_ctx *const c; EmitArgs ea; const bool want_rssa; const uint64_t tot2 ; const EmitVisit *const visit;
    const uint64_t total, s0, s1;
    const uint64_t lead;
    const uint64_t nrows, chunk_rows, nchunks;
    const bool windowed, runaware;
    const bool keep_sa;
    uint8_t *bwtbuf = nullptr; SAT *sabuf = nullptr; unsigned long long *d_b = nullptr;
    std::vector<EmitWin> wins; uint64_t maxq = 0, maxrows = 0;
    uint64_t *bk0 = nullptr, *bk1 = nullptr; uint32_t *bv0 = nullptr, *bv1 = nullptr, *btg = nullptr;
    uint32_t *tilecnt = nullptr, *tilebase = nullptr, *d_cnt = nullptr, *qtmp = nullptr; uint16_t *rmask = nullptr;
    bool fill_masks = false;
    std::vector<hipEvent_t> wev;

    Emission(pfp_ctx *c_, const EmitArgs &ea_, bool want_sa, bool want_rssa_, int slice, int nslices, uint64_t tot2_, const EmitVisit *visit_)
        : c(c_), ea(ea_), want_rssa(want_rssa_), tot2(tot2_), visit(visit_), total(ea_.nout), s0(slice_first_row(total, slice, nslices)), s1(slice_first_row(total, slice + 1, nslices)),
          lead(s0 ? 1 : 0), nrows(s1 - s0), chunk_rows(visit_ ? visit_->window_rows : c_->tun.emit_chunk_rows ? c_->tun.emit_chunk_rows : (3ULL << 30)), nchunks((nrows + chunk_rows - 1) / chunk_rows),
          windowed(nslices > 1 || nchunks > 1), runaware(ea_.special != 0), keep_sa(want_sa && !visit_) {}
    ~Emission() { for (auto e : wev) (void)hipEventDestroy(e); }

    int run()
    {
        PFP_TRY(place_outputs());
        PFP_TRY(plan_windows());
        PFP_TRY(alloc_routes());
        struct LeftRows { const EmitArgs &ea; ~LeftRows() { if (ea.gstat) print_left_rows(ea.gstat); } } left_rows{ea};
        if (visit) return run_visit();
        if (!want_rssa || keep_sa) return run_bwt_then_exact_samples(false);
        bool overflow = false;
        PFP_TRY(run_one_pass_samples(&overflow));
        return overflow ? run_bwt_then_exact_samples(true) : PFP_OK;
    }

    int place_outputs()
    {
        if (!visit) { c->slice_begin = s0; c->slice_rows = nrows; }
        uint8_t *bwtraw = nullptr;
        if (!visit) PFP_ALLOC_LO(c, bwtraw, uint8_t, nrows + lead + 48);
        bwtbuf = bwtraw + ((s0 - lead) & 15);
        if (keep_sa) PFP_ALLOC_LO(c, sabuf, SAT, nrows + lead);
        if (!visit) { c->d_bwt = bwtbuf + lead; c->d_sa = sabuf ? sabuf + lead : nullptr; c->d_ssa = c->d_esa = nullptr; }
        PFP_ALLOC_HI(c, d_b, unsigned long long, 6);
        return PFP_OK;
    }
    uint8_t *bwt_of(const EmitWin &wn) const { return bwtbuf + (wn.cs - wn.cl - (s0 - lead)); }
    SAT *sa_of(const EmitWin &wn) const { return sabuf ? sabuf + (wn.cs - wn.cl - (s0 - lead)) : (SAT *)nullptr; }

    int plan_windows()
    {
        wins.resize((size_t)nchunks);
        for (uint64_t ch = 0; ch < nchunks; ++ch) {
            EmitWin &wn = wins[(size_t)ch];
            wn.cs = s0 + ch * chunk_rows; wn.ce = (wn.cs + chunk_rows < s1) ? wn.cs + chunk_rows : s1; wn.cl = wn.cs ? 1 : 0;
            wn.e0 = 0; wn.e1 = total; wn.q0 = 0; wn.q1 = tot2; wn.j0 = 0; wn.j1 = runaware ? ea.ecount : 0;
        }
        if (windowed) {
            unsigned long long *d_bounds; PFP_ALLOC_HI(c, d_bounds, unsigned long long, 6 * nchunks);
            for (uint64_t ch = 0; ch < nchunks; ++ch)
                PFP_LAUNCH(c, K_MISC, 64, (k_slice_bounds<EBT>), 1, ea, wins[(size_t)ch].cs - wins[(size_t)ch].cl, wins[(size_t)ch].ce, d_bounds + 6 * ch);
            std::vector<unsigned long long> hb(6 * (size_t)nchunks);
            PFP_HIP(c, hipMemcpyAsync(hb.data(), d_bounds, hb.size() * 8, hipMemcpyDeviceToHost, c->stream));
            PFP_HIP(c, hipStreamSynchronize(c->stream));
            for (uint64_t ch = 0; ch < nchunks; ++ch) { EmitWin &wn = wins[(size_t)ch]; const unsigned long long *b = &hb[6 * (size_t)ch]; wn.e0 = b[0]; wn.e1 = b[1]; wn.q0 = b[2]; wn.q1 = b[3]; wn.j0 = b[4]; wn.j1 = b[5]; }
        }
        for (const EmitWin &wn : wins) { if (wn.q1 - wn.q0 > maxq) maxq = wn.q1 - wn.q0; if (wn.ce - wn.cs > maxrows) maxrows = wn.ce - wn.cs; }
        return PFP_OK;
    }

    int alloc_routes()
    {
        if (ea.big_total) {
            if (ea.big_total >= 0xFFFFFFF0ULL) return PFP_E_TOO_LARGE;
            PFP_ALLOC_HI(c, bk0, uint64_t, ea.big_total); PFP_ALLOC_HI(c, bk1, uint64_t, ea.big_total);
            PFP_ALLOC_HI(c, bv0, uint32_t, ea.big_total); PFP_ALLOC_HI(c, bv1, uint32_t, ea.big_total); PFP_ALLOC_HI(c, btg, uint32_t, ea.big_total);
        }
        ea.big_keys = bk0; ea.big_vals = bv0; ea.big_count = d_b + 4; ea.big_cap = ea.big_total;
        ea.group_rows_cap = c->tun.emit_group_rows; ea.rank_members_max = c->tun.big_group_members != -2 ? 0xFFFFFFFFu : c->tun.emit_group_rows >= (uint32_t)EG_BUF ? BIG_GROUP_MEMBERS : 3u;
        const uint64_t max_etiles = maxq / EMIT_TILE + 3;
        if (runaware && ea.group_rows_cap && tot2 && ea.cinfo) {
            PFP_ALLOC_HI(c, ea.gleft, uint8_t, (size_t)ea.ecount + 1); PFP_ALLOC_HI(c, ea.tile_left, uint8_t, max_etiles);
            PFP_HIP(c, hipMemsetAsync(ea.gleft, 0, (size_t)ea.ecount + 1, c->stream));
        }
        ea.qpasses = (bits_for(c->nrows ? c->nrows : 0xFFFFFFFFULL) + 7) / 8;
        if (ea.gleft) {
            const uint32_t cap = ea.group_rows_cap < (uint32_t)EG_BUF ? ea.group_rows_cap : (uint32_t)EG_BUF;
            ea.lgcap = maxq / cap + 2;
            PFP_ALLOC_HI(c, ea.lglist, uint32_t, 2 * ea.lgcap); PFP_ALLOC_HI(c, ea.lgcount, unsigned long long, 2);
        }
        if (ea.gleft && c->tun.verbose) { PFP_ALLOC_HI(c, ea.gstat, unsigned long long, 12); PFP_HIP(c, hipMemsetAsync(ea.gstat, 0, 96, c->stream)); }
        return PFP_OK;
    }

    int emit_window(const EmitWin &wn, uint8_t *bwt_at, SAT *sa_at, uint32_t *q_at, bool fill)
    {
        ea.w0 = wn.cs - wn.cl; ea.w1 = wn.ce;
        if (ea.big_total) PFP_HIP(c, hipMemsetAsync(ea.big_count, 0, 16, c->stream));
        if (runaware) PFP_TRY(emit_runaware(wn, bwt_at, q_at, fill));
        else PFP_TRY(emit_all_rows(wn, bwt_at, sa_at, q_at));
        return ea.big_total ? place_big_groups(bwt_at, sa_at, q_at) : PFP_OK;
    }
    int emit_runaware(const EmitWin &wn, uint8_t *bwt_at, uint32_t *q_at, bool fill)
    {
        ea.e0 = wn.q0; ea.e1 = wn.q1; ea.q0 = wn.q0;
        if (fill) {
            const uint32_t fill_subs = c->tun.fill_subs < 1u ? 1u : c->tun.fill_subs > FILL_MAX_SUBS ? FILL_MAX_SUBS : c->tun.fill_subs;
            const uint64_t super = (uint64_t)FILL_GROUPS * FILL_SUB;
            const uint64_t nsub = (ea.w1 - 1) / super - ea.w0 / super + 1;
            const int skip = c->tun.fill_skip ? 1 : 0;
            if (fill_masks) PFP_LAUNCH(c, K_FILL, (ea.w1 - ea.w0) * 9 / 8, (k_fill<EBT, true>), nblocks(nsub, fill_subs), ea, bwt_at, fill_subs, skip, rmask, wn.cs);
            else PFP_LAUNCH(c, K_FILL, ea.w1 - ea.w0, (k_fill<EBT, false>), nblocks(nsub, fill_subs), ea, bwt_at, fill_subs, skip, (uint16_t *)nullptr, (uint64_t)0);
        }
        if (ea.e1 <= ea.e0) return PFP_OK;
        const unsigned ge = (unsigned)((ea.e1 - 1) / EMIT_TILE - ea.e0 / EMIT_TILE + 1);
        if (ea.gleft) {
            PFP_HIP(c, hipMemsetAsync(ea.tile_left, 0, (size_t)ge, c->stream));
            PFP_HIP(c, hipMemsetAsync(ea.lgcount, 0, 16, c->stream));
            PFP_LAUNCH(c, K_EMIT, (ea.e1 - ea.e0) * (1 + 4 + (q_at ? 4 : 0)), (k_emit_groups<EBT>), ge, ea, bwt_at, q_at);
            PFP_LAUNCH(c, K_EMIT_LARGE, 0, (k_emit_groups_large<EBT, EG1_BUF>), ge < 1024u ? ge : 1024u, ea, bwt_at, q_at);
            PFP_LAUNCH(c, K_EMIT_LARGE, 0, (k_emit_groups_large<EBT, EG2_BUF>), ge < 512u ? ge : 512u, ea, bwt_at, q_at);
            PFP_LAUNCH(c, K_EMIT_BIG, 0, (k_emit<SAT, EBT>), ge, ea, bwt_at, (SAT *)nullptr, q_at);
        } else
            PFP_LAUNCH(c, K_EMIT, (ea.e1 - ea.e0) * (1 + 4 + (q_at ? 4 : 0)), (k_emit<SAT, EBT>), ge, ea, bwt_at, (SAT *)nullptr, q_at);
        return PFP_OK;
    }
    int emit_all_rows(const EmitWin &wn, uint8_t *bwt_at, SAT *sa_at, uint32_t *q_at)
    {
        ea.e0 = wn.e0; ea.e1 = wn.e1; ea.q0 = 0;
        PFP_LAUNCH(c, K_EMIT, (ea.w1 - ea.w0) * (1 + 4 + (sa_at ? 8 + sizeof(SAT) : 0) + (q_at ? 4 : 0)),
                   (k_emit<SAT, EBT>), (unsigned)((ea.e1 - 1) / EMIT_TILE - ea.e0 / EMIT_TILE + 1), ea, bwt_at, sa_at, q_at);
        return PFP_OK;
    }
    int place_big_groups(uint8_t *bwt_at, SAT *sa_at, uint32_t *q_at)
    {
        unsigned long long hb[2];
        PFP_HIP(c, hipMemcpyAsync(hb, ea.big_count, 16, hipMemcpyDeviceToHost, c->stream));
        PFP_HIP(c, hipStreamSynchronize(c->stream));
        if (hb[1] || hb[0] > ea.big_total) return PFP_E_CORRUPT;
        const uint64_t nb = hb[0];
        if (!nb) return PFP_OK;
        const BitRange big_ranges[2] = {{0, bits_for(c->nrows)}, {32, 32 + bits_for(ea.dsize)}};
        uint64_t *sk; uint32_t *sv;
        PFP_TRY(radix_sort_pairs<uint64_t>(c, bk0, bv0, bk1, bv1, nb, big_ranges, 2, &sk, &sv));
        PFP_LAUNCH(c, K_EMIT_BIG, nb * 12, k_big_heads, nblocks(nb, BLOCK), (const uint64_t *)sk, nb, btg);
        PFP_TRY((device_scan<uint32_t, 1>(c, btg, btg, nb, nullptr)));
        PFP_LAUNCH(c, K_EMIT_BIG, nb * (30 + sizeof(SAT)), (k_big_place<SAT, EBT>), nblocks(nb, BLOCK), ea, (const uint64_t *)sk, (const uint32_t *)sv, (const uint32_t *)btg, nb, bwt_at, sa_at, q_at);
        return PFP_OK;
    }

    int stream_out(const EmitWin &wn)
    {
        if (!c->h_bwt && !c->h_sa) return PFP_OK;
        const uint64_t r0 = wn.cs - wn.cl < s0 ? s0 : wn.cs - wn.cl, r1 = wn.ce == s1 ? wn.ce : wn.ce - 1;
        if (r1 <= r0) return PFP_OK;
        hipEvent_t e; PFP_HIP(c, hipEventCreateWithFlags(&e, hipEventDisableTiming)); wev.push_back(e);
        PFP_HIP(c, hipEventRecord(e, c->stream));
        PFP_HIP(c, hipStreamWaitEvent(c->fa.copy, e, 0));
        const uint64_t rows = r1 - r0;
        if (c->h_bwt) PFP_HIP(c, hipMemcpyAsync(c->h_bwt + (r0 - s0), bwtbuf + (r0 - (s0 - lead)), (size_t)rows, hipMemcpyDeviceToHost, c->fa.copy));
        if (c->h_sa && sabuf) PFP_HIP(c, hipMemcpyAsync((char *)c->h_sa + (r0 - s0) * sizeof(SAT), sabuf + (r0 - (s0 - lead)), (size_t)rows * sizeof(SAT), hipMemcpyDeviceToHost, c->fa.copy));
        return PFP_OK;
    }

    int alloc_sample_scratch(bool with_q)
    {
        const uint64_t maxtiles = nblocks(maxrows, RUN_TILE);
        PFP_ALLOC_HI(c, tilecnt, uint32_t, maxtiles); PFP_ALLOC_HI(c, tilebase, uint32_t, maxtiles); PFP_ALLOC_HI(c, d_cnt, uint32_t, 1);
        PFP_ALLOC_HI(c, rmask, uint16_t, maxtiles * BLOCK);
        qtmp = nullptr;
        if (with_q) PFP_ALLOC_HI(c, qtmp, uint32_t, (runaware ? maxq : maxrows) + 1);
        ea.qspec = qtmp;
        return PFP_OK;
    }
    int count_window_runs(const EmitWin &wn, uint32_t *rc, bool masks_filled)
    {
        const uint64_t rows = wn.ce - wn.cs, ntiles = nblocks(rows, RUN_TILE);
        const uint8_t *bytes = bwt_of(wn) + wn.cl;
        if (masks_filled) {
            const uint64_t nsp = wn.j1 > wn.j0 ? wn.j1 - wn.j0 : 0, nedge = 2 + (wn.ce - 1) / FILL_SUB - wn.cs / FILL_SUB;
            const unsigned nsb = nblocks(nsp, BLOCK);
            PFP_LAUNCH(c, K_RUN_MASKS, (wn.q1 - wn.q0) * 9 / 8 + nsp * 24, (k_run_masks_fix<EBT>), nsb + nblocks(nedge, BLOCK), ea, bytes, wn.cs, rows, (int)wn.cl, wn.j0, wn.j1, (uint32_t)nsb, rmask);
            PFP_LAUNCH(c, K_RUN_MASKS, rows / 8, k_mask_tile_count, nblocks(ntiles, MT_TILES), (const uint16_t *)rmask, rows, (uint64_t)ntiles, tilecnt);
        } else
            PFP_LAUNCH(c, K_RUNS, rows, k_run_tile_count, ntiles, bytes, rows, (int)wn.cl, tilecnt, rmask);
        PFP_TRY((device_scan<uint32_t, 0>(c, tilecnt, tilebase, ntiles, d_cnt)));
        return d2h_u32(c, d_cnt, rc);
    }
    int sample_window(const EmitWin &wn, uint32_t rc, uint64_t run_base, uint64_t r_total, SAT *ssa, SAT *esa_w, const SAT *sa_win)
    {
        const uint64_t rows = wn.ce - wn.cs, ntiles = nblocks(rows, RUN_TILE);
        const bool last = wn.ce == total;
        PFP_LAUNCH(c, K_SAMPLES, rows / 8 + (uint64_t)rc * 4 * sizeof(SAT), (k_sample_rows<SAT>), nblocks(ntiles, SR_TILES), (const uint16_t *)rmask, rows, (uint64_t)ntiles, (const uint32_t *)tilebase, wn.cs, run_base, total,
                   last ? r_total + 1 : (uint64_t)0, ssa, esa_w);
        PFP_LAUNCH(c, K_SAMPLES, (uint64_t)rc * (2 * 60 + 4 * sizeof(SAT)), (k_sample_values<SAT, EBT>), nblocks((uint64_t)rc + 1, BLOCK), ea, sa_win, (const uint32_t *)qtmp, wn.cs - wn.cl, (uint64_t)rc, run_base,
                   (int)last, last ? (uint64_t)(r_total - 1) : (uint64_t)0, ssa, esa_w);
        return PFP_OK;
    }
    void publish_run_count(uint64_t r) { c->runs = r; c->esa_pairs = r - (s0 == 0 ? 1 : 0) + (s1 == total ? 1 : 0); }

    int run_visit()
    {
        const uint64_t wrows = (chunk_rows < nrows ? chunk_rows : nrows) + 1;
        uint8_t *wbraw; SAT *wsa;
        PFP_ALLOC_HI(c, wbraw, uint8_t, wrows + 48); PFP_ALLOC_HI(c, wsa, SAT, wrows);
        for (const EmitWin &wn : wins) {
            PFP_TRY(emit_window(wn, wbraw + ((wn.cs - wn.cl) & 15), wsa, (uint32_t *)nullptr, false));
            PFP_TRY(visit->fn(wn.cs, wn.ce - wn.cs, (const void *)(wsa + wn.cl)));
        }
        return PFP_OK;
    }

    int run_one_pass_samples(bool *overflowed)
    {
        const size_t lo_mark = c->arena.mark_lo(), hi_mark = c->arena.mark_hi();
        PFP_TRY(alloc_sample_scratch(true));
        fill_masks = c->tun.fill_masks && runaware;
        for (const EmitWin &wn : wins) if (wn.cs % FILL_PER_THREAD) fill_masks = false;
        struct MasksOff { bool &f; ~MasksOff() { f = false; } } masks_off{fill_masks};
        const bool masks_filled = fill_masks;
        const size_t freeb = c->arena.hi > c->arena.lo + ((size_t)256 << 20) ? c->arena.hi - c->arena.lo - ((size_t)256 << 20) : 0;
        uint64_t cap = freeb / (4 * sizeof(SAT));
        if (cap > nrows) cap = nrows;
        if (c->tun.sample_cap < cap) cap = c->tun.sample_cap;
        SAT *samp = nullptr;
        if (cap) { samp = (SAT *)c->arena.reserve_lo(sizeof(SAT) * (4 * cap + 4)); if (!samp) return PFP_E_NOMEM; }
        SAT *ssa = samp, *esa = samp ? samp + 2 * cap : nullptr;
        SAT *esa_w = esa ? esa + 2 * lead : nullptr;
        uint64_t run_base = 0; bool overflow = cap == 0;
        for (const EmitWin &wn : wins) {
            PFP_TRY(emit_window(wn, bwt_of(wn), (SAT *)nullptr, qtmp, true));
            PFP_TRY(stream_out(wn));
            uint32_t rc = 0; PFP_TRY(count_window_runs(wn, &rc, masks_filled));
            if (!overflow && run_base + rc > cap) overflow = true;
            if (!overflow && !(c->arena.commit_range(ssa + 2 * run_base, sizeof(SAT) * (2 * (size_t)rc + 4)) && c->arena.commit_range(esa + 2 * run_base, sizeof(SAT) * (2 * (size_t)rc + 8)))) overflow = true;
            if (!overflow) PFP_TRY(sample_window(wn, rc, run_base, run_base + rc, ssa, esa_w, (const SAT *)nullptr));
            run_base += rc;
        }
        publish_run_count(run_base);
        c->arena.release_hi(hi_mark);
        *overflowed = overflow;
        if (overflow) { c->arena.release_lo(lo_mark); return PFP_OK; }
        c->d_ssa = ssa; c->d_esa = esa;
        c->arena.release_lo(c->arena.offset_of(esa) + sizeof(SAT) * (2 * (size_t)run_base + 8));
        return PFP_OK;
    }

    int run_bwt_then_exact_samples(bool bwt_done)
    {
        if (!bwt_done) {
            for (const EmitWin &wn : wins) {
                PFP_TRY(emit_window(wn, bwt_of(wn), sa_of(wn), (uint32_t *)nullptr, true));
                PFP_TRY(stream_out(wn));
            }
            PFP_TRY(count_slice_runs());
        }
        return want_rssa ? exact_samples() : PFP_OK;
    }
    int count_slice_runs()
    {
        unsigned long long *d_runs = d_b + 2;
        PFP_HIP(c, hipMemsetAsync(d_runs, 0, 8, c->stream));
        PFP_LAUNCH(c, K_RUNS, nrows, k_run_count, nblocks(nrows, 16 * BLOCK), (const uint8_t *)c->d_bwt, nrows, (int)lead, d_runs);
        unsigned long long r = 0;
        PFP_HIP(c, hipMemcpyAsync(&r, d_runs, 8, hipMemcpyDeviceToHost, c->stream));
        PFP_HIP(c, hipStreamSynchronize(c->stream));
        publish_run_count(r);
        return PFP_OK;
    }
    int exact_samples()
    {
        const uint64_t r = c->runs;
        if (sabuf) {
            PFP_HIP(c, hipStreamSynchronize(c->stream));
            c->arena.release_hi(c->emit_scratch_mark);
        }
        SAT *ssa, *esa;
        PFP_ALLOC_LO(c, ssa, SAT, 2 * r + 2); PFP_ALLOC_LO(c, esa, SAT, 2 * r + 4);
        c->d_ssa = ssa; c->d_esa = esa;
        SAT *esa_w = esa + 2 * lead;
        PFP_TRY(alloc_sample_scratch(!sabuf));
        uint64_t run_base = 0;
        for (const EmitWin &wn : wins) {
            if (!sabuf) PFP_TRY(emit_window(wn, bwt_of(wn), (SAT *)nullptr, qtmp, false));
            uint32_t rc = 0; PFP_TRY(count_window_runs(wn, &rc, false));
            if (run_base + rc > r) return PFP_E_CORRUPT;
            PFP_TRY(sample_window(wn, rc, run_base, r, ssa, esa_w, (const SAT *)sa_of(wn)));
            run_base += rc;
        }
        return run_base == r ? PFP_OK : PFP_E_CORRUPT;
    }
};

template <typename EBT> struct SlotStage {
    pfp_ctx *const c; EmitArgs ea; const bool runaware; const uint64_t dsize;
    EBT *cnt = nullptr, *EB = nullptr, *d_tot = nullptr, *cnt2 = nullptr; unsigned long long *d_hard = nullptr;
    uint32_t *s_g0 = nullptr, *gk = nullptr, *gqf = nullptr, *gql = nullptr; uint8_t *gfl = nullptr, *gnu = nullptr;
    bool gq_done = false;
    EBT tot = 0;
    unsigned long long hh[2] = {0, 0};
    uint64_t tot2 = 0;

    int alloc_slot_arrays()
    {
        PFP_ALLOC_HI(c, cnt, EBT, dsize); PFP_ALLOC_HI(c, EB, EBT, dsize); PFP_ALLOC_HI(c, d_hard, unsigned long long, 2); PFP_ALLOC_HI(c, d_tot, EBT, 2);
        PFP_HIP(c, hipMemsetAsync(d_hard, 0, 16, c->stream));
        PFP_ALLOC_HI(c, s_g0, uint32_t, dsize); PFP_ALLOC_HI(c, gk, uint32_t, dsize); PFP_ALLOC_HI(c, gfl, uint8_t, dsize); PFP_ALLOC_HI(c, gnu, uint8_t, dsize);
        PFP_HIP(c, hipMemsetAsync(gfl, 0, dsize, c->stream));
        PFP_HIP(c, hipMemsetAsync(gnu, 0, dsize, c->stream));
        if (runaware) {
            PFP_ALLOC_HI(c, cnt2, EBT, dsize); PFP_ALLOC_HI(c, gqf, uint32_t, dsize); PFP_ALLOC_HI(c, gql, uint32_t, dsize);
            PFP_HIP(c, hipMemsetAsync(gqf, 0xFF, dsize * 4, c->stream));
            PFP_HIP(c, hipMemsetAsync(gql, 0, dsize * 4, c->stream));
        }
        ea.EB = EB; ea.s_g0 = s_g0; ea.gk = gk; ea.cnt = cnt; ea.gqf = gqf; ea.gql = gql;
        return PFP_OK;
    }
    int slot_prepass()
    {
        const size_t mkp = c->arena.mark_hi();
        if (ea.use_prec) {
            uint4 *prec; PFP_ALLOC_HI(c, prec, uint4, dsize);
            PFP_LAUNCH(c, K_EMIT_COUNT, dsize * 29, k_pack_prec, nblocks(dsize, BLOCK), ea.D, ea.wordid, ea.winfo, dsize, ea.dwords, prec, ea.use_e0 ? ea.bwsai_il : (const tpos_t *)nullptr);
            ea.prec = prec;
        } else {
            uint2 *posinfo; PFP_ALLOC_HI(c, posinfo, uint2, dsize);
            PFP_LAUNCH(c, K_EMIT_COUNT, dsize * 17, k_pack_posinfo, nblocks(dsize, BLOCK), ea.D, ea.wordid, dsize, posinfo);
            ea.posinfo = posinfo;
        }
        uint2 *wpq = nullptr;
        if (runaware && c->tun.group_reduce && !ea.use_e0) {
            PFP_ALLOC_HI(c, wpq, uint2, ea.dwords);
            PFP_LAUNCH(c, K_EMIT_COUNT, (uint64_t)ea.dwords * 24, k_pack_wpq, nblocks(ea.dwords, BLOCK), ea.ilist, ea.wrank, ea.occ, ea.F, (uint64_t)ea.dwords, wpq);
        }
        PFP_LAUNCH(c, K_EMIT_COUNT, dsize * (30 + sizeof(EBT)) + (wpq ? dsize * 8 : 0), (k_emit_slots<EBT>), nblocks(dsize, BLOCK), ea, cnt, d_hard, (uint32_t *)ea.s_sl, (uint32_t *)ea.s_fb, (uint8_t *)ea.s_fl, (uint8_t *)ea.s_pc, s_g0, gk, gfl, gnu,
                   (const uint2 *)wpq, gqf, gql);
        if (wpq) gq_done = true;
        c->arena.release_hi(mkp);
        ea.prec = nullptr; ea.posinfo = nullptr;
        return PFP_OK;
    }
    int mark_big_groups()
    {
        uint4 *sinfo; PFP_ALLOC_HI(c, sinfo, uint4, dsize); ea.sinfo = sinfo;
        const long big_members = c->tun.big_group_members == -2 ? (long)BIG_GROUP_MEMBERS : c->tun.big_group_members;
        PFP_TRY((device_scan<EBT, 0>(c, cnt, EB, dsize, d_tot)));
        const uint32_t big_rows = !(runaware && big_members >= 0 && c->tun.emit_group_rows) ? 0u : c->tun.emit_group_rows >= (uint32_t)EG_BUF ? (uint32_t)EG2_BUF : 4u * c->tun.emit_group_rows;
        PFP_LAUNCH(c, K_EMIT_COUNT, dsize * 14, (k_big_mark<EBT>), nblocks(dsize, BLOCK), (const EBT *)cnt, (const uint32_t *)s_g0, (const uint32_t *)gk, (const uint8_t *)gfl, (const uint8_t *)gnu, (const uint32_t *)ea.s_fb, ea.ilist, dsize,
                   big_members >= 0 ? (uint32_t)big_members : 0xFFFFFFFFu, runaware ? 1 : 0, (uint8_t *)ea.s_fl, sinfo, cnt2, gq_done ? nullptr : gqf, gq_done ? nullptr : gql, d_hard + 1, (const EBT *)EB, (const EBT *)d_tot, big_rows, (big_rows && c->tun.big_group_members == -2) ? 1 : 0);
        PFP_HIP(c, hipMemcpyAsync(hh, d_hard, 16, hipMemcpyDeviceToHost, c->stream));
        PFP_HIP(c, hipMemcpyAsync(&tot, d_tot, sizeof(EBT), hipMemcpyDeviceToHost, c->stream));
        PFP_HIP(c, hipStreamSynchronize(c->stream));
        ea.big_total = hh[1];
        return PFP_OK;
    }
    int build_tile_index()
    {
        const uint64_t ntiles = ((uint64_t)tot + EMIT_TILE - 1) / EMIT_TILE;
        uint32_t *tile_slot; PFP_ALLOC_HI(c, tile_slot, uint32_t, ntiles + 1);
        PFP_LAUNCH(c, K_EMIT_COUNT, dsize * 2 * sizeof(EBT) + ntiles * 4, (k_tile_slots<EBT>), nblocks(dsize, BLOCK), (const EBT *)cnt, (const EBT *)EB, dsize, ntiles, tile_slot);
        ea.tile_slot = tile_slot;
        ea.ENB = EB; ea.etile_slot = tile_slot; ea.ecount = (uint32_t)dsize;
        return PFP_OK;
    }
    int build_special_list()
    {
        uint32_t *flag, *cpos, *spl, *d_cnt;
        PFP_ALLOC_HI(c, flag, uint32_t, dsize); PFP_ALLOC_HI(c, cpos, uint32_t, dsize + 1); PFP_ALLOC_HI(c, d_cnt, uint32_t, 1);
        PFP_LAUNCH(c, K_EMIT_COUNT, dsize * 5, k_flag_special, nblocks(dsize, BLOCK), (const uint8_t *)ea.s_fl, dsize, flag);
        PFP_TRY((device_scan<uint32_t, 0>(c, flag, cpos, dsize, d_cnt)));
        uint32_t nsp = 0; PFP_TRY(d2h_u32(c, d_cnt, &nsp));
        PFP_ALLOC_HI(c, spl, uint32_t, (size_t)nsp + 1);
        if (nsp) PFP_LAUNCH(c, K_COMPACT, dsize * 12, k_compact_scatter, nblocks(dsize, BLOCK), (const uint32_t *)nullptr, (const uint32_t *)flag, (const uint32_t *)cpos, dsize, spl);
        EBT *cntc, *ENBc;
        PFP_ALLOC_HI(c, cntc, EBT, (size_t)nsp + 1); PFP_ALLOC_HI(c, ENBc, EBT, (size_t)nsp + 1);
        uint64_t ntiles2 = 0;
        if (nsp) {
            PFP_LAUNCH(c, K_EMIT_COUNT, (uint64_t)nsp * (4 + 2 * sizeof(EBT)), (k_gather_counts<EBT>), nblocks(nsp, BLOCK), (const EBT *)cnt, (const uint32_t *)spl, (uint64_t)nsp, cntc);
            PFP_TRY((device_scan<EBT, 0>(c, cntc, ENBc, nsp, ENBc + nsp)));
            EBT t2 = 0;
            PFP_HIP(c, hipMemcpyAsync(&t2, ENBc + nsp, sizeof(EBT), hipMemcpyDeviceToHost, c->stream));
            PFP_HIP(c, hipStreamSynchronize(c->stream));
            tot2 = (uint64_t)t2;
            ntiles2 = (tot2 + EMIT_TILE - 1) / EMIT_TILE;
            uint32_t *et; PFP_ALLOC_HI(c, et, uint32_t, ntiles2 + 1);
            PFP_LAUNCH(c, K_EMIT_COUNT, (uint64_t)nsp * 2 * sizeof(EBT) + ntiles2 * 4, (k_tile_slots<EBT>), nblocks(nsp, BLOCK), (const EBT *)cntc, (const EBT *)ENBc, (uint64_t)nsp, ntiles2, et);
            ea.etile_slot = et;
        } else PFP_HIP(c, hipMemsetAsync(ENBc, 0, sizeof(EBT), c->stream));
        ea.ENB = ENBc; ea.elist = spl; ea.cpos = cpos; ea.ecount = nsp; ea.special = 1;
        if (nsp && c->tun.emit_group_rows) {
            uint4 *cinfo; unsigned long long *cgb; uint32_t *town;
            PFP_ALLOC_HI(c, cinfo, uint4, nsp); PFP_ALLOC_HI(c, cgb, unsigned long long, nsp); PFP_ALLOC_HI(c, town, uint32_t, ntiles2 + 1);
            PFP_LAUNCH(c, K_EMIT_COUNT, (uint64_t)nsp * 50, (k_special_pack<EBT>), nblocks(nsp, BLOCK), ea, nsp, cinfo, cgb);
            PFP_LAUNCH(c, K_EMIT_COUNT, (ntiles2 + 1) * 40, (k_tile_own<EBT>), nblocks(ntiles2 + 1, BLOCK), (const EBT *)ENBc, (const uint4 *)cinfo, (const uint32_t *)ea.etile_slot, (uint64_t)nsp, ntiles2, town);
            ea.cinfo = cinfo; ea.cgb = cgb; ea.town = town;
        }
        return PFP_OK;
    }
    int print_group_stats()
    {
        unsigned long long *d_hist, hist[64]; PFP_ALLOC_HI(c, d_hist, unsigned long long, 64);
        PFP_HIP(c, hipMemsetAsync(d_hist, 0, 512, c->stream));
        PFP_LAUNCH(c, K_MISC, dsize * 20, (k_group_stats<EBT>), nblocks(dsize, BLOCK), (const EBT *)cnt, (const EBT *)EB, (const uint32_t *)s_g0, (const uint32_t *)gk, (const uint8_t *)ea.s_fl, dsize, (uint64_t)tot, d_hist);
        PFP_HIP(c, hipMemcpyAsync(hist, d_hist, 512, hipMemcpyDeviceToHost, c->stream));
        PFP_HIP(c, hipStreamSynchronize(c->stream));
        fprintf(stderr, "[pfbwt_hip] rows by group members (rows) x group rows (cols: <1K <4K <16K <64K <256K <1M <4M more); hard %llu, sort-route %llu of %llu; run-aware %d: %llu rows of %u special slots enumerated\n",
                hh[0], hh[1], (unsigned long long)tot, (int)runaware, (unsigned long long)tot2, (unsigned)ea.ecount);
        static const char *kn[8] = {"1", "2-3", "4-7", "8-15", "16-31", "32-63", "64-127", "128+"};
        for (int a = 0; a < 8; ++a) { fprintf(stderr, "[pfbwt_hip]  k %-7s", kn[a]); for (int b = 0; b < 8; ++b) fprintf(stderr, " %13llu", hist[a * 8 + b]); fprintf(stderr, "\n"); }
        return PFP_OK;
    }
};
template <typename EBT> static int emit_stage(pfp_ctx *c, const EmitArgs &prepass, int want_sa, int want_rssa, int slice, int nslices, const EmitVisit *visit)
{
    SlotStage<EBT> st{c, prepass, !want_sa && !c->tun.no_runaware, c->dsize};
    PFP_TRY(st.alloc_slot_arrays());
    PFP_TRY(st.slot_prepass());
    PFP_TRY(st.mark_big_groups());
    PFP_TRY(st.build_tile_index());
    if (st.runaware) PFP_TRY(st.build_special_list());
    if (c->tun.verbose) PFP_TRY(st.print_group_stats());
    const uint64_t nout = st.tot;
    if (nout < 2) return PFP_E_CORRUPT;
    if (c->n && nout != c->n + 1) return PFP_E_CORRUPT;
    if (!c->n) c->n = nout - 1;
    st.ea.nout = nout; st.ea.n = c->n;
    if (!visit) { c->nout = nout; c->hard = st.hh[0]; c->easy = nout - st.hh[0]; }
    if (c->flags & PFP_FLAG_U64) return Emission<uint64_t, EBT>(c, st.ea, want_sa != 0, want_rssa != 0, slice, nslices, st.tot2, visit).run();
    if (nout > 0xFFFFFFFFULL) return PFP_E_TOO_LARGE;
    return Emission<uint32_t, EBT>(c, st.ea, want_sa != 0, want_rssa != 0, slice, nslices, st.tot2, visit).run();
}

static int emit_prepass_and_run(pfp_ctx *c, int want_sa, int want_rssa, int slice, int nslices, const EmitVisit *visit)
{
    const uint64_t dsize = c->dsize, dwords = c->dwords;
    uint32_t *F, *s_sl, *s_fb; uint8_t *s_fl, *s_pc; uint4 *winfo;
    if (dwords > WID_MASK) return PFP_E_TOO_LARGE;
    PFP_ALLOC_HI(c, F, uint32_t, dwords + 1);
    PFP_ALLOC_HI(c, s_sl, uint32_t, dsize); PFP_ALLOC_HI(c, s_fb, uint32_t, dsize);
    PFP_ALLOC_HI(c, s_fl, uint8_t, dsize); PFP_ALLOC_HI(c, s_pc, uint8_t, dsize);
    PFP_TRY((device_scan<uint32_t, 0>(c, c->d_occ, F, dwords, nullptr)));
    PFP_LAUNCH(c, K_MISC, dwords * 8, k_u32_add_store, nblocks(dwords, BLOCK), (const uint32_t *)F, dwords, 1u, F);
    EmitArgs ea;
    ea.D = c->d_dict; ea.dsize = dsize; ea.dwords = (uint32_t)dwords; ea.w = c->w;
    ea.SA = c->d_gsa; ea.srank = c->d_srank; ea.ws = c->d_ws; ea.wrank = c->d_wrank;
    ea.occ = c->d_occ; ea.F = F; ea.ilist = c->d_ilist; ea.bwsai = c->d_bwsai; ea.bwlast = c->d_bwlast; ea.bwl_il = c->d_bwl_il;
    PFP_ALLOC_HI(c, winfo, uint4, dwords);
    PFP_LAUNCH(c, K_MISC, dwords * 32, k_pack_winfo, nblocks(dwords, BLOCK), (const uint32_t *)c->d_ws, (const uint32_t *)c->d_wrank, (const uint32_t *)c->d_occ, (const uint32_t *)F, dwords, winfo);
    ea.winfo = winfo;
    uint32_t maxlen = 0;
    {
        uint32_t *d_ml; PFP_ALLOC_HI(c, d_ml, uint32_t, 1);
        PFP_HIP(c, hipMemsetAsync(d_ml, 0, 4, c->stream));
        PFP_LAUNCH(c, K_MISC, dwords * 4, k_max_word_length, nblocks(dwords, BLOCK), (const uint32_t *)c->d_ws, dwords, d_ml);
        PFP_TRY(d2h_u32(c, d_ml, &maxlen));
    }
    if (want_sa && c->d_bwsai && c->nrows) {
        tpos_t *E; PFP_ALLOC_HI(c, E, tpos_t, c->nrows);
        PFP_LAUNCH(c, K_MISC, c->nrows * 20, k_bwsai_by_ilist, nblocks(c->nrows, BLOCK), (const uint32_t *)c->d_ilist, (const tpos_t *)c->d_bwsai, c->nrows, E);
        ea.bwsai_il = E;
        ea.use_e0 = (c->n != 0 && c->n + (uint64_t)c->w + 2 < 0xFFFFFFFFULL && !c->tun.no_slot_records) ? 1 : 0;
    }
    ea.wordid = c->d_wordid; ea.use_prec = (maxlen < (1u << PREC_SL_BITS) && !c->tun.no_slot_records) ? 1 : 0;
    ea.s_sl = s_sl; ea.s_fb = s_fb; ea.s_fl = s_fl; ea.s_pc = s_pc;
    if (!visit) { c->have_sa = want_sa != 0; c->have_rssa = want_rssa != 0; }
    const bool force_wide = c->tun.force_wide_rows != 0;
    const bool wide = force_wide || c->n == 0 || c->n + 2 >= 0xFFFFFFFFULL;
    return wide ? emit_stage<uint64_t>(c, ea, want_sa, want_rssa, slice, nslices, visit) : emit_stage<uint32_t>(c, ea, want_sa, want_rssa, slice, nslices, visit);
}

static int bwt_build_body(pfp_ctx *c, int want_sa, int want_rssa, int slice, int nslices, pfp_bwt_sizes *out)
{
    HostTimer timer;
    const size_t mk = c->arena.mark_hi();
    c->emit_scratch_mark = mk;
    PFP_TRY(emit_prepass_and_run(c, want_sa, want_rssa, slice, nslices, nullptr));
    PFP_HIP(c, hipStreamSynchronize(c->stream));
    c->arena.release_hi(mk);
    c->stage = 3;
    c->stage_ms[2] = timer.ms();
    if (out) { out->nout = c->nout; out->r = c->runs; out->easy_cases = c->easy; out->hard_cases = c->hard; }
    return PFP_OK;
}
static int bwt_build_impl(pfp_ctx *c, int want_sa, int want_rssa, int slice, int nslices, pfp_bwt_sizes *out)
{
    if (!c || nslices < 1 || slice < 0 || slice >= nslices) return PFP_E_ARG;
    if (c->stage < 2) return PFP_E_STATE;
    if ((want_sa || want_rssa) && !c->d_bwsai) return PFP_E_STATE;
    PFP_HIP(c, hipSetDevice(c->device));
    c->arena.release_lo(c->lo_after_pbwt);
    drop_post_results(c);
    if (!c->gsa_valid) {
        ArenaGuard gs(c);
        const int rs = gs.done(sort_dict_suffixes(c));
        if (rs != PFP_OK) { c->gsa_valid = false; return rs; }
        c->lo_after_pbwt = c->arena.mark_lo();
    }
    ArenaGuard g(c);
    const int rc = g.done(bwt_build_body(c, want_sa, want_rssa, slice, nslices, out));
    if (rc != PFP_OK) { c->stage = 2; c->d_bwt = nullptr; c->d_sa = c->d_ssa = c->d_esa = nullptr; }
    return rc;
}
static int visit_sa_windows(pfp_ctx *c, uint64_t window_rows, std::function<int(uint64_t, uint64_t, const void *)> fn)
{
    if (!c->d_bwsai) return PFP_E_STATE;
    const size_t mk = c->arena.mark_hi();
    const EmitVisit visit{window_rows, std::move(fn)};
    PFP_TRY(emit_prepass_and_run(c, 1, 0, 0, 1, &visit));
    PFP_HIP(c, hipStreamSynchronize(c->stream));
    c->arena.release_hi(mk);
    return PFP_OK;
}

extern "C" {
int pfp_bwt_build(pfp_ctx *c, int want_sa, int want_rssa, pfp_bwt_sizes *out) { return bwt_build_impl(c, want_sa, want_rssa, 0, 1, out); }
int pfp_bwt_build_stream(pfp_ctx *c, int want_sa, int want_rssa, uint8_t *host_bwt, void *host_sa, pfp_bwt_sizes *out)
{
    if (!c || !host_bwt || (want_sa && !host_sa)) return PFP_E_ARG;
    PFP_HIP(c, hipSetDevice(c->device));
    PFP_TRY(ensure_copy_stream(c));
    c->h_bwt = host_bwt; c->h_sa = want_sa ? host_sa : nullptr;
    const int rc = bwt_build_impl(c, want_sa, want_rssa, 0, 1, out);
    c->h_bwt = nullptr; c->h_sa = nullptr;
    const hipError_t e = hipStreamSynchronize(c->fa.copy);
    if (rc == PFP_OK && e != hipSuccess) { c->hip_err = (int)e; return PFP_E_HIP; }
    return rc;
}
int pfp_text_length(pfp_ctx *c, uint64_t *n) { if (!c || !n) return PFP_E_ARG; *n = c->n; return PFP_OK; }
int pfp_bwt_build_slice(pfp_ctx *c, int want_sa, int want_rssa, int slice, int nslices, pfp_bwt_sizes *out, uint64_t *slice_begin, uint64_t *slice_rows, uint64_t *esa_pairs)
{
    int rc = bwt_build_impl(c, want_sa, want_rssa, slice, nslices, out);
    if (rc != PFP_OK) return rc;
    if (slice_begin) *slice_begin = c->slice_begin;
    if (slice_rows) *slice_rows = c->slice_rows;
    if (esa_pairs) *esa_pairs = c->esa_pairs;
    return PFP_OK;
}

int pfp_bwt_get(pfp_ctx *c, uint8_t *bwt, void *sa, void *ssa, void *esa)
{
    if (!c) return PFP_E_ARG;
    if (c->stage < 3) return PFP_E_STATE;
    PFP_HIP(c, hipSetDevice(c->device));
    const size_t U = (c->flags & PFP_FLAG_U64) ? 8 : 4;
    if (bwt) PFP_HIP(c, hipMemcpy(bwt, c->d_bwt, c->slice_rows, hipMemcpyDeviceToHost));
    if (sa) { if (!c->d_sa) return PFP_E_STATE; PFP_HIP(c, hipMemcpy(sa, c->d_sa, c->slice_rows * U, hipMemcpyDeviceToHost)); }
    if (ssa) { if (!c->d_ssa) return PFP_E_STATE; PFP_HIP(c, hipMemcpy(ssa, c->d_ssa, c->runs * 2 * U, hipMemcpyDeviceToHost)); }
    if (esa) { if (!c->d_esa) return PFP_E_STATE; PFP_HIP(c, hipMemcpy(esa, c->d_esa, c->esa_pairs * 2 * U, hipMemcpyDeviceToHost)); }
    return PFP_OK;
}

int pfp_bwt_device_ptrs(pfp_ctx *c, const void **d_bwt, const void **d_sa, const void **d_ssa, const void **d_esa)
{
    if (!c) return PFP_E_ARG;
    if (c->stage < 3) return PFP_E_STATE;
    if (d_bwt) *d_bwt = c->d_bwt;
    if (d_sa) *d_sa = c->d_sa;
    if (d_ssa) *d_ssa = c->d_ssa;
    if (d_esa) *d_esa = c->d_esa;
    return PFP_OK;
}
}
```

### pfbwt-f_amd/csrc/pfbwt_hip.hip

```cpp
#include "common.h"
#include "prims.h"
#include "parse.h"
#include "fasta.h"
#include "sufsort.h"
#include "recsort.h"
#include "dictrec.h"
#include "emit.h"
#include "markers.h"
#include "docarray.h"
#include "lcparray.h"
#include "thresholds.h"
#include "matchstats.h"
#include <algorithm>
#include <functional>
#include <map>
#include <sched.h>
#include <thread>
#if defined(__SSE2__)
#include <emmintrin.h>
#endif

using namespace pfp;

#ifndef PFP_BACKEND_NAME
#define PFP_BACKEND_NAME "hip-gfx950"
#endif

static int ensure_arena(pfp_ctx *c, uint64_t n_hint)
{
    size_t want = c->arena_request ? c->arena_request : (size_t)(96ULL * n_hint + (64ULL << 20));
    if (!c->arena_request) {
        size_t fr = 0, tot = 0;
        if (hipMemGetInfo(&fr, &tot) == hipSuccess) {
            const size_t avail = fr + c->arena.vm.committed;
            const size_t cap = avail - avail / 16;
            if (want > cap) want = cap;
        }
    }
    want &= ~(size_t)4095;
    if (c->arena.base && c->arena.cap >= want) return PFP_OK;
    VmRegion nv;
    if (nv.reserve(want, c->device) != hipSuccess) { c->arena.want = want; return PFP_E_NOMEM; }
    if (c->arena.base) { PFP_HIP(c, hipStreamSynchronize(c->stream)); (void)hipDeviceSynchronize(); c->arena.vm.destroy(); c->arena.base = nullptr; c->arena.cap = 0; }
    c->arena.vm = nv; nv.base = nullptr;
    c->arena.base = c->arena.vm.base; c->arena.cap = want; c->arena.reset();
    return PFP_OK;
}

static int ensure_text(pfp_ctx *c, uint64_t need_n)
{
    const size_t need = 16 + (((size_t)need_n + 4095) / 4096) * 4096 + 4096 + 64;
    if (c->tb && c->tb_cap >= need) return PFP_OK;
    if (!c->text.live() || need > c->text.va_bytes) {
        size_t fr = 0, tot = 0;
        if (hipMemGetInfo(&fr, &tot) != hipSuccess) { (void)hipGetLastError(); tot = (size_t)1 << 38; }
        size_t va = c->text_hint ? (size_t)c->text_hint + (size_t)c->text_hint / 8 + ((size_t)64 << 20) : (4 * need > ((size_t)64 << 20) ? 4 * need : ((size_t)64 << 20));
        if (!c->text_hint && c->text.live() && va < 2 * c->text.va_bytes) va = 2 * c->text.va_bytes;
        if (!c->text_hint && va > tot && tot > need + need / 4) va = tot;
        if (va < need) va = need + need / 4;
        VmRegion nr;
        if (nr.reserve(va, c->device) != hipSuccess) return PFP_E_NOMEM;
        if (c->tb) {
            if (!nr.commit(0, 16 + (size_t)c->n)) { nr.destroy(); return PFP_E_NOMEM; }
            PFP_HIP(c, hipMemcpyAsync(nr.base, c->tb, 16 + (size_t)c->n, hipMemcpyDeviceToDevice, c->stream));
            PFP_HIP(c, hipStreamSynchronize(c->stream));
            c->text.destroy();
        }
        c->text = nr; nr.base = nullptr;
        c->tb = (uint8_t *)c->text.base; c->tb_cap = 0;
    }
    if (!c->text.commit(0, need)) return PFP_E_NOMEM;
    c->tb_cap = c->text.vmm ? (c->text.lo_edge < c->text.va_bytes ? c->text.lo_edge : c->text.va_bytes) : c->text.va_bytes;
    return PFP_OK;
}

static void reset_results(pfp_ctx *c)
{
    c->stage = 0; c->n = 0; c->nseq = 0; c->tb_n = 0; c->left_ctx = 0; c->view.src = nullptr; c->m = c->dwords = c->dsize = 0; c->nrows = 0; c->nout = c->runs = c->esa_pairs = 0;
    c->gsa_valid = false; c->d_wrank = nullptr; c->d_bwt = nullptr; c->d_sa = c->d_ssa = c->d_esa = nullptr;
    c->d_bwlast = nullptr; c->d_ilist = nullptr; c->d_bwsai = nullptr; c->d_bwl_il = nullptr;
    drop_post_results(c);
    c->d_ye = nullptr; c->d_pid = nullptr; c->d_parse = nullptr; c->d_last = nullptr; c->d_dict = nullptr; c->d_ws = nullptr; c->d_wordid = nullptr;
    c->d_occ = nullptr; c->d_sdict = nullptr; c->d_gsa = nullptr; c->d_grank = nullptr; c->d_srank = nullptr; c->d_sflag = nullptr;
    c->arena.reset();
    c->fa.started = false; c->fa.state = 2; c->fa.records = 0; c->fa.rec_raw.clear(); c->fa.rec_pos.clear();
}

static const char *const tunable_names[] = {"verbose", "seg_grid", "seg_stage", "sort_k", "sort_no_table", "class_sort_maxrange", "dedup_table_log2", "no_trigger_table",
                                            "emit_chunk_rows", "fill_subs", "sample_cap", "no_runaware", "big_group_members", "force_wide_rows", "fasta_chunk_bytes", "ingest_block_bytes", "emit_group_rows", "no_slot_records", "dict_text_rounds", "int_key_symbols", "force_run_round",
                                            "ingest_readers", "expand_dma", "parse_rec", "parse_rec_p2", "parse_rec_min", "parse_rec_depth", "parse_rec_tile_rows", "parse_rec_table_log2", "dict_rec", "dict_rec_p2", "dedup_variant", "dedup_phases", "dedup_period", "dedup_chunk", "doc_lds_max", "dedup_packed", "group_reduce", "scan_waves", "lcp_long_min", "thr_long_min", "thr_tile", "thr_window_rows", "plcp_block_log2", "fill_masks", "fill_skip", "ms_dir_log2", "ms_long_min"};
static int set_tunable(pfp_ctx *c, const char *key, long long v)
{
    Tunables &t = c->tun;
    if (!strcmp(key, "verbose")) t.verbose = (int)v;
    else if (!strcmp(key, "seg_grid")) t.seg_grid = (int)v;
    else if (!strcmp(key, "seg_stage")) t.seg_stage = (int)v;
    else if (!strcmp(key, "sort_k")) t.sort_k = (int)v;
    else if (!strcmp(key, "sort_no_table")) t.sort_no_table = (int)v;
    else if (!strcmp(key, "class_sort_maxrange")) t.class_sort_maxrange = (uint32_t)v;
    else if (!strcmp(key, "dedup_table_log2")) t.dedup_table_log2 = (int)v;
    else if (!strcmp(key, "no_trigger_table")) t.no_trigger_table = (int)v;
    else if (!strcmp(key, "emit_chunk_rows")) t.emit_chunk_rows = v > 0 ? (uint64_t)v : (3ULL << 30);
    else if (!strcmp(key, "fill_subs")) t.fill_subs = (uint32_t)v;
    else if (!strcmp(key, "fill_masks")) t.fill_masks = (int)v;
    else if (!strcmp(key, "fill_skip")) t.fill_skip = (int)v;
    else if (!strcmp(key, "sample_cap")) t.sample_cap = v < 0 ? ~0ULL : (uint64_t)v;
    else if (!strcmp(key, "no_runaware")) t.no_runaware = (int)v;
    else if (!strcmp(key, "big_group_members")) t.big_group_members = (long)v;
    else if (!strcmp(key, "force_wide_rows")) t.force_wide_rows = (int)v;
    else if (!strcmp(key, "fasta_chunk_bytes")) t.fasta_chunk_bytes = v > 0 ? (uint64_t)v : 0;
    else if (!strcmp(key, "ingest_block_bytes")) t.ingest_block_bytes = v > 0 ? (uint64_t)v : 0;
    else if (!strcmp(key, "emit_group_rows")) t.emit_group_rows = v > 0 ? (uint32_t)v : 0u;
    else if (!strcmp(key, "no_slot_records")) t.no_slot_records = (int)v;
    else if (!strcmp(key, "dict_text_rounds")) t.dict_text_rounds = (int)v;
    else if (!strcmp(key, "int_key_symbols")) t.int_key_symbols = (int)v;
    else if (!strcmp(key, "force_run_round")) t.force_run_round = (int)v;
    else if (!strcmp(key, "ingest_readers")) t.ingest_readers = (int)v;
    else if (!strcmp(key, "expand_dma")) t.expand_dma = (int)v;
    else if (!strcmp(key, "parse_rec")) t.parse_rec = (int)v;
    else if (!strcmp(key, "parse_rec_p2")) t.parse_rec_p2 = (int)v;
    else if (!strcmp(key, "parse_rec_min")) t.parse_rec_min = v > 0 ? (uint64_t)v : 0;
    else if (!strcmp(key, "parse_rec_depth")) t.parse_rec_depth = (int)v;
    else if (!strcmp(key, "parse_rec_tile_rows")) t.parse_rec_tile_rows = v > 0 ? (uint32_t)v : 0u;
    else if (!strcmp(key, "parse_rec_table_log2")) t.parse_rec_table_log2 = (int)v;
    else if (!strcmp(key, "dict_rec")) t.dict_rec = (int)v;
    else if (!strcmp(key, "dict_rec_p2")) t.dict_rec_p2 = (int)v;
    else if (!strcmp(key, "dedup_variant")) t.dedup_variant = (int)v;
    else if (!strcmp(key, "dedup_phases")) t.dedup_phases = (int)v;
    else if (!strcmp(key, "dedup_packed")) t.dedup_packed = (int)v;
    else if (!strcmp(key, "group_reduce")) t.group_reduce = (int)v;
    else if (!strcmp(key, "scan_waves")) t.scan_waves = (int)v;
    else if (!strcmp(key, "dedup_period")) t.dedup_period = (int64_t)v;
    else if (!strcmp(key, "dedup_chunk")) t.dedup_chunk = (int64_t)v;
    else if (!strcmp(key, "doc_lds_max")) t.doc_lds_max = v < 2 ? 2u : v > (long long)DOC_LDS_CAP ? DOC_LDS_CAP : (uint32_t)v;
    else if (!strcmp(key, "lcp_long_min")) t.lcp_long_min = v < 16 ? 16u : v > (1LL << 30) ? (1u << 30) : (((uint32_t)v + 15u) & ~15u);
    else if (!strcmp(key, "thr_long_min")) t.thr_long_min = v < 1 ? 1u : v > (1LL << 30) ? (1u << 30) : (uint32_t)v;
    else if (!strcmp(key, "thr_tile")) { uint32_t p2 = 16; while (p2 < (1u << 20) && (long long)p2 < v) p2 *= 2; t.thr_tile = p2; }
    else if (!strcmp(key, "thr_window_rows")) t.thr_window_rows = v < 1 ? (1ULL << 30) : (uint64_t)v;
    else if (!strcmp(key, "plcp_block_log2")) t.plcp_block_log2 = v < 0 ? -1 : v > PLCP_BLOCK_LOG2_MAX ? PLCP_BLOCK_LOG2_MAX : (int)v;
    else if (!strcmp(key, "ms_dir_log2")) t.ms_dir_log2 = v < 0 ? -1 : v > MS_DIR_LOG2_MAX ? MS_DIR_LOG2_MAX : (int)v;
    else if (!strcmp(key, "ms_long_min")) t.ms_long_min = v < 1 ? 1u : v > (1LL << 30) ? (1u << 30) : (uint32_t)v;
    else return PFP_E_ARG;
    return PFP_OK;
}
static void load_tunables_from_env(pfp_ctx *c)
{
    if (getenv("PFP_VERBOSE")) c->tun.verbose = 1;
    const char *hooks = getenv("PFP_TEST_HOOKS");
    if (!hooks || strcmp(hooks, "1")) return;
    for (const char *name : tunable_names) {
        char env[64] = "PFP_"; size_t k = 4;
        for (const char *q = name; *q && k + 1 < sizeof env; ++q) env[k++] = (char)((*q >= 'a' && *q <= 'z') ? *q - 32 : *q);
        env[k] = 0;
        const char *e = getenv(env);
        if (e) (void)set_tunable(c, name, *e ? atoll(e) : 1LL);
    }
}

extern "C" {

const char *pfp_backend(void) { return PFP_BACKEND_NAME; }
int pfp_debug_set(pfp_ctx *c, const char *key, long long value) { return (c && key) ? set_tunable(c, key, value) : PFP_E_ARG; }

const char *pfp_strerror(int s)
{
    switch (s) {
    case PFP_OK: return "ok";
    case PFP_E_ARG: return "invalid argument";
    case PFP_E_INVALID_CHAR: return "error, invalid character";
    case PFP_E_TOO_LARGE: return "input too long for 32-bit device indices";
    case PFP_E_NOMEM: return "device workspace exhausted";
    case PFP_E_HIP: return "HIP runtime error";
    case PFP_E_ONE_WORD: return "error: only one dict word total. Re-run with a smaller p modulus";
    case PFP_E_STATE: return "call order violated";
    case PFP_E_CORRUPT: return "something went wrong!";
    case PFP_E_IO: return "failed to open file!";
    default: return "unknown status";
    }
}

pfp_ctx *pfp_create(int w, uint64_t p, unsigned flags, int device, uint64_t workspace_bytes, int *status)
{
    int st = PFP_OK;
    pfp_ctx *c = nullptr;
    if (w < 1 || w > 32 || p == 0) st = PFP_E_ARG;
    else {
        int ndev = 0;
        if (hipGetDeviceCount(&ndev) != hipSuccess || ndev <= 0 || device < 0 || device >= ndev) st = PFP_E_HIP;
        else if (hipSetDevice(device) != hipSuccess) st = PFP_E_HIP;
        else {
            c = new pfp_ctx();
            c->w = w; c->p = p; c->flags = flags; c->device = device; c->arena_request = (size_t)workspace_bytes;
            load_tunables_from_env(c);
            if (hipStreamCreateWithFlags(&c->stream, hipStreamNonBlocking) != hipSuccess) { delete c; c = nullptr; st = PFP_E_HIP; }
        }
    }
    if (status) *status = st;
    return c;
}

void pfp_destroy(pfp_ctx *c)
{
    if (!c) return;
    (void)hipSetDevice(c->device);
    if (c->stream) (void)hipStreamSynchronize(c->stream);
    (void)hipDeviceSynchronize();
    prof_collect(c);
    for (auto e : c->ev_pool) (void)hipEventDestroy(e);
    c->text.destroy();
    for (int k = 0; k < 2; ++k) { if (c->fa.raw[k]) (void)hipFree(c->fa.raw[k]); if (c->fa.ev_copied[k]) (void)hipEventDestroy(c->fa.ev_copied[k]); if (c->fa.ev_free[k]) (void)hipEventDestroy(c->fa.ev_free[k]); }
    if (c->fa.tiles) (void)hipFree(c->fa.tiles);
    if (c->fa.d_tot) (void)hipFree(c->fa.d_tot);
    if (c->fa.h_tot) (void)hipHostFree(c->fa.h_tot);
    if (c->fa.copy_ready) (void)hipStreamDestroy(c->fa.copy);
    for (auto &q : c->ing_buf) if (q) (void)hipHostFree(q);
    if (c->d_trigtab) (void)hipFree(c->d_trigtab);
    for (int k = 0; k < 2; ++k) { if (c->hstage[k]) (void)hipHostFree(c->hstage[k]); if (c->hstage_ev[k]) (void)hipEventDestroy(c->hstage_ev[k]); }
    c->arena.vm.destroy();
    if (c->stream) (void)hipStreamDestroy(c->stream);
    delete c;
}

int pfp_error_detail(pfp_ctx *c, uint64_t *pos, int *ch)
{
    if (!c) return PFP_E_ARG;
    if (pos) *pos = c->err_pos;
    if (ch) *ch = c->err_ch;
    return PFP_OK;
}
uint64_t pfp_workspace_needed(pfp_ctx *c) { return c ? (uint64_t)(c->arena.cap + c->arena.want) : 0; }
int pfp_reset(pfp_ctx *c)
{
    if (!c) return PFP_E_ARG;
    PFP_HIP(c, hipSetDevice(c->device));
    PFP_HIP(c, hipStreamSynchronize(c->stream));
    reset_results(c);
    return PFP_OK;
}

int pfp_profile_enable(pfp_ctx *c, int on) { if (!c) return PFP_E_ARG; prof_collect(c); c->prof_on = on != 0; c->prof_mask = ~0ULL; return PFP_OK; }
int pfp_profile_select(pfp_ctx *c, const char *kernel)
{
    if (!c || !kernel) return PFP_E_ARG;
    prof_collect(c);
    for (int i = 0; i < K_COUNT_; ++i) if (!strcmp(kernel, kernel_names[i])) { c->prof_on = true; c->prof_mask = 1ULL << i; return PFP_OK; }
    return PFP_E_ARG;
}
int pfp_profile_reset(pfp_ctx *c) { if (!c) return PFP_E_ARG; prof_collect(c); for (auto &r : c->prof) r = ProfRec(); return PFP_OK; }
int pfp_profile_get(pfp_ctx *c, int idx, const char **name, uint64_t *launches, double *ms, double *bytes)
{
    if (!c || idx < 0 || idx >= K_COUNT_) return PFP_E_ARG;
    prof_collect(c);
    if (name) *name = kernel_names[idx];
    if (launches) *launches = c->prof[idx].launches;
    if (ms) *ms = c->prof[idx].ms;
    if (bytes) *bytes = c->prof[idx].bytes;
    return PFP_OK;
}
// ... 1273 lines not shown
    PFP_HIP(c, hipSetDevice(c->device));
    unsigned long long *d_out; PFP_HIP(c, hipMalloc((void **)&d_out, 16));
    PFP_HIP(c, hipMemsetAsync(d_out, 0, 16, c->stream));
    const uint64_t per = (uint64_t)1 << 34;
    for (uint64_t off = 0; off < bytes; off += per) {
        const uint64_t nb = bytes - off < per ? bytes - off : per;
        PFP_LAUNCH(c, K_MISC, nb, k_checksum, nblocks(nb, 16 * BLOCK), (const uint8_t *)d_buf + off, nb, global_offset + off, d_out);
    }
    unsigned long long h[2];
    PFP_HIP(c, hipMemcpyAsync(h, d_out, 16, hipMemcpyDeviceToHost, c->stream));
    PFP_HIP(c, hipStreamSynchronize(c->stream));
    PFP_HIP(c, hipFree(d_out));
    out[0] = h[0]; out[1] = h[1];
    return PFP_OK;
}

__global__ __launch_bounds__(BLOCK) void k_wordsum(const uint8_t *p, uint64_t bytes, unsigned long long *out)
{
    __shared__ unsigned long long red[4];
    const uint64_t nw = (bytes + 7) / 8;
    unsigned long long a = 0, b = 0;
    for (uint64_t i = (uint64_t)blockIdx.x * BLOCK + threadIdx.x; i < nw; i += (uint64_t)gridDim.x * BLOCK) {
        unsigned long long v = 0;
        if (8 * i + 8 <= bytes) v = ld8(p + 8 * i); else for (uint64_t k = 0; 8 * i + k < bytes; ++k) v |= (unsigned long long)p[8 * i + k] << (8 * k);
        a += v; b += v * (i + 1);
    }
    unsigned long long ta, tb;
    (void)block_excl_sum(a, red, &ta); (void)block_excl_sum(b, red, &tb);
    if (threadIdx.x == 0) { atomicAdd(&out[0], ta); atomicAdd(&out[1], tb); }
}
int pfp_debug_wordsum(pfp_ctx *c, const void *d_buf, uint64_t bytes, uint64_t out[2])
{
    if (!c || (!d_buf && bytes) || !out) return PFP_E_ARG;
    PFP_HIP(c, hipSetDevice(c->device));
    unsigned long long *d_out; PFP_HIP(c, hipMalloc((void **)&d_out, 16));
    PFP_HIP(c, hipMemsetAsync(d_out, 0, 16, c->stream));
    if (bytes) PFP_LAUNCH(c, K_MISC, bytes, k_wordsum, 4096, (const uint8_t *)d_buf, bytes, d_out);
    unsigned long long h[2];
    PFP_HIP(c, hipMemcpyAsync(h, d_out, 16, hipMemcpyDeviceToHost, c->stream));
    PFP_HIP(c, hipStreamSynchronize(c->stream));
    PFP_HIP(c, hipFree(d_out));
    out[0] = h[0]; out[1] = h[1];
    return PFP_OK;
}
extern "C++" {
template <typename SAT> __global__ __launch_bounds__(BLOCK) void k_check_sample_order(const uint8_t *X, uint64_t n, const SAT *ssa, const SAT *esa, uint64_t r, unsigned long long *out)
{
    const uint64_t k = (uint64_t)blockIdx.x * BLOCK + threadIdx.x;
    if (k + 1 >= r) return;
    const uint64_t ra = esa[2 * k], a = esa[2 * k + 1], rb = ssa[2 * k + 2], b = ssa[2 * k + 3];
    if (ra + 1 != rb) atomicAdd(&out[2], 1ULL);
    uint64_t h = 0; bool ok = false;
    for (;;) {
        const uint64_t pa = a + h, pb = b + h;
        if (pa > n || pb > n) break;
        const uint64_t va = ld8(X + pa), vb = ld8(X + pb);
        if (va != vb) {
            const int sh = (__ffsll((long long)(va ^ vb)) - 1) & ~7;
            const uint64_t q = (uint64_t)sh >> 3;
            if (pa + q > n || pb + q > n) break;
            ok = ((va >> sh) & 0xFF) < ((vb >> sh) & 0xFF); h += q;
            break;
        }
        h += 8;
    }
    if (!ok) atomicAdd(&out[1], 1ULL);
    atomicAdd(&out[0], 1ULL); atomicMax(&out[3], (unsigned long long)h); atomicAdd(&out[4], (unsigned long long)h);
}
}
int pfp_debug_check_sample_order(pfp_ctx *c, uint64_t out[5])
{
    if (!c || !out) return PFP_E_ARG;
    if (c->stage < 3 || !c->d_ssa || !c->d_esa || !c->tb || c->tb_n != c->n || c->slice_rows != c->nout) return PFP_E_STATE;
    PFP_HIP(c, hipSetDevice(c->device));
    unsigned long long *d_out; PFP_HIP(c, hipMalloc((void **)&d_out, 40));
    PFP_HIP(c, hipMemsetAsync(d_out, 0, 40, c->stream));
    const uint64_t r = c->runs;
    if (r > 1) {
        if (c->flags & PFP_FLAG_U64) PFP_LAUNCH(c, K_MISC, r * 64, (k_check_sample_order<uint64_t>), nblocks(r, BLOCK), (const uint8_t *)c->tb + 16, c->n, (const uint64_t *)c->d_ssa, (const uint64_t *)c->d_esa, r, d_out);
        else PFP_LAUNCH(c, K_MISC, r * 64, (k_check_sample_order<uint32_t>), nblocks(r, BLOCK), (const uint8_t *)c->tb + 16, c->n, (const uint32_t *)c->d_ssa, (const uint32_t *)c->d_esa, r, d_out);
    }
    unsigned long long h[5];
    PFP_HIP(c, hipMemcpyAsync(h, d_out, 40, hipMemcpyDeviceToHost, c->stream));
    PFP_HIP(c, hipStreamSynchronize(c->stream));
    PFP_HIP(c, hipFree(d_out));
    for (int i = 0; i < 5; ++i) out[i] = h[i];
    return PFP_OK;
}
extern "C++" {
template <typename SAT> __global__ __launch_bounds__(BLOCK) void k_check_sa(const uint8_t *X, uint64_t n, const SAT *sa, const uint8_t *bwt, uint64_t rows, uint32_t *seen, unsigned long long *out)
{
    const uint64_t i = (uint64_t)blockIdx.x * BLOCK + threadIdx.x;
    if (i >= rows) return;
    const uint64_t v = sa[i];
    if (v > n) { atomicAdd(&out[1], 1ULL); return; }
    const uint32_t bit = 1u << (v & 31);
    if (atomicOr(&seen[v >> 5], bit) & bit) atomicAdd(&out[2], 1ULL);
    const uint8_t want = v == 0 ? (uint8_t)0 : X[v - 1];
    if (bwt[i] != want || (i == 0 && v != n)) atomicAdd(&out[3], 1ULL);
    if (bwt[i] == 0) atomicAdd(&out[4], 1ULL);
}
}
int pfp_debug_check_sa(pfp_ctx *c, uint64_t out[5])
{
    if (!c || !out) return PFP_E_ARG;
    if (c->stage < 3 || !c->d_sa || !c->have_sa || !c->d_bwt || !c->tb || c->tb_n != c->n || c->slice_rows != c->nout) return PFP_E_STATE;
    PFP_HIP(c, hipSetDevice(c->device));
    const uint64_t rows = c->nout, words = (c->n + 32) / 32 + 1;
    unsigned long long *d_out; uint32_t *seen;
    PFP_HIP(c, hipMalloc((void **)&d_out, 40)); PFP_HIP(c, hipMalloc((void **)&seen, words * 4));
    PFP_HIP(c, hipMemsetAsync(d_out, 0, 40, c->stream)); PFP_HIP(c, hipMemsetAsync(seen, 0, words * 4, c->stream));
    if (c->flags & PFP_FLAG_U64) PFP_LAUNCH(c, K_MISC, rows * 10, (k_check_sa<uint64_t>), nblocks(rows, BLOCK), (const uint8_t *)c->tb + 16, c->n, (const uint64_t *)c->d_sa, (const uint8_t *)c->d_bwt, rows, seen, d_out);
    else PFP_LAUNCH(c, K_MISC, rows * 6, (k_check_sa<uint32_t>), nblocks(rows, BLOCK), (const uint8_t *)c->tb + 16, c->n, (const uint32_t *)c->d_sa, (const uint8_t *)c->d_bwt, rows, seen, d_out);
    unsigned long long h[5];
    PFP_HIP(c, hipMemcpyAsync(h, d_out, 40, hipMemcpyDeviceToHost, c->stream));
    PFP_HIP(c, hipStreamSynchronize(c->stream));
    PFP_HIP(c, hipFree(d_out)); PFP_HIP(c, hipFree(seen));
    out[0] = rows; for (int i = 1; i < 5; ++i) out[i] = h[i];
    return PFP_OK;
}
extern "C++" {
template <typename SAT> __global__ __launch_bounds__(BLOCK) void k_check_samples(const SAT *ssa, const SAT *esa, uint64_t r, const SAT *sa, const uint8_t *bwt, uint64_t rows, unsigned long long *out)
{
    const uint64_t k = (uint64_t)blockIdx.x * BLOCK + threadIdx.x;
    if (k >= r) return;
    const uint64_t rs = ssa[2 * k], vs = ssa[2 * k + 1], re = esa[2 * k], ve = esa[2 * k + 1];
    bool row_ok = rs < rows && re < rows && rs <= re;
    if (row_ok) {
        row_ok = (k == 0 ? rs == 0 : bwt[rs] != bwt[rs - 1]) && (k + 1 == r ? re + 1 == rows : (uint64_t)ssa[2 * k + 2] == re + 1) && bwt[rs] == bwt[re];
    }
    if (!row_ok) { atomicAdd(&out[1], 1ULL); return; }
    if ((uint64_t)sa[rs] != vs || (uint64_t)sa[re] != ve) atomicAdd(&out[2], 1ULL);
}
}
int pfp_debug_check_samples(pfp_ctx *c, uint64_t out[3])
{
    if (!c || !out) return PFP_E_ARG;
    if (c->stage < 3 || !c->d_sa || !c->have_sa || !c->have_rssa || !c->d_ssa || !c->d_esa || c->slice_rows != c->nout || c->esa_pairs != c->runs) return PFP_E_STATE;
    PFP_HIP(c, hipSetDevice(c->device));
    unsigned long long *d_out; PFP_HIP(c, hipMalloc((void **)&d_out, 24));
    PFP_HIP(c, hipMemsetAsync(d_out, 0, 24, c->stream));
    const uint64_t r = c->runs;
    if (r) {
        if (c->flags & PFP_FLAG_U64) PFP_LAUNCH(c, K_MISC, r * 50, (k_check_samples<uint64_t>), nblocks(r, BLOCK), (const uint64_t *)c->d_ssa, (const uint64_t *)c->d_esa, r, (const uint64_t *)c->d_sa, (const uint8_t *)c->d_bwt, c->nout, d_out);
        else PFP_LAUNCH(c, K_MISC, r * 30, (k_check_samples<uint32_t>), nblocks(r, BLOCK), (const uint32_t *)c->d_ssa, (const uint32_t *)c->d_esa, r, (const uint32_t *)c->d_sa, (const uint8_t *)c->d_bwt, c->nout, d_out);
    }
    unsigned long long h[3];
    PFP_HIP(c, hipMemcpyAsync(h, d_out, 24, hipMemcpyDeviceToHost, c->stream));
    PFP_HIP(c, hipStreamSynchronize(c->stream));
    PFP_HIP(c, hipFree(d_out));
    out[0] = r; out[1] = h[1]; out[2] = h[2];
    return PFP_OK;
}
int pfp_host_register(void *p, uint64_t bytes) { if (!p || !bytes) return PFP_E_ARG; if (hipHostRegister(p, (size_t)bytes, hipHostRegisterDefault) != hipSuccess) { (void)hipGetLastError(); return PFP_E_HIP; } return PFP_OK; }
int pfp_host_unregister(void *p) { if (!p) return PFP_E_ARG; if (hipHostUnregister(p) != hipSuccess) { (void)hipGetLastError(); return PFP_E_HIP; } return PFP_OK; }

__global__ __launch_bounds__(BLOCK) void k_debug_fill(uint64_t *keys, uint32_t *vals, uint64_t n, int bits, uint64_t seed)
{
    const uint64_t i = (uint64_t)blockIdx.x * BLOCK + threadIdx.x;
    if (i >= n) return;
    uint64_t z = (i + seed) * 0x9E3779B97F4A7C15ULL; z = (z ^ (z >> 30)) * 0xBF58476D1CE4E5B9ULL; z = (z ^ (z >> 27)) * 0x94D049BB133111EBULL; z ^= z >> 31;
    keys[i] = bits >= 64 ? z : (z & ((1ULL << bits) - 1ULL)); vals[i] = (uint32_t)i;
}
__global__ __launch_bounds__(BLOCK) void k_debug_check_sorted(const uint64_t *keys, uint64_t n, uint32_t *bad)
{
    const uint64_t i = (uint64_t)blockIdx.x * BLOCK + threadIdx.x;
    if (i + 1 < n && keys[i] > keys[i + 1]) atomicAdd(bad, 1u);
}
int pfp_debug_sort(pfp_ctx *c, uint64_t n, int bits, int reps, double *ms_out, uint32_t *unsorted_pairs)
{
    if (!c || n < 2 || bits < 1 || bits > 64) return PFP_E_ARG;
    PFP_HIP(c, hipSetDevice(c->device));
    PFP_TRY(ensure_arena(c, n));
    c->arena.reset(); c->stage = 0;
    uint64_t *k0, *k1; uint32_t *v0, *v1, *d_bad;
    PFP_ALLOC_HI(c, k0, uint64_t, n); PFP_ALLOC_HI(c, k1, uint64_t, n); PFP_ALLOC_HI(c, v0, uint32_t, n); PFP_ALLOC_HI(c, v1, uint32_t, n); PFP_ALLOC_HI(c, d_bad, uint32_t, 1);
    BitRange br = {0, bits};
    double best = 1e30;
    uint64_t *sk = k0; uint32_t *sv = v0;
    for (int r = 0; r < reps; ++r) {
        PFP_LAUNCH(c, K_MISC, n * 12, k_debug_fill, nblocks(n, BLOCK), k0, v0, n, bits, (uint64_t)r * 7919);
        PFP_HIP(c, hipStreamSynchronize(c->stream));
        HostTimer t;
        int rc = radix_sort_pairs<uint64_t>(c, k0, v0, k1, v1, n, &br, 1, &sk, &sv);
        if (rc != PFP_OK) return rc;
        PFP_HIP(c, hipStreamSynchronize(c->stream));
        const double ms = t.ms();
        if (ms < best) best = ms;
    }
    PFP_HIP(c, hipMemsetAsync(d_bad, 0, 4, c->stream));
    PFP_LAUNCH(c, K_MISC, n * 8, k_debug_check_sorted, nblocks(n, BLOCK), (const uint64_t *)sk, n, d_bad);
    uint32_t bad = 0; PFP_TRY(d2h_u32(c, d_bad, &bad));
    if (ms_out) *ms_out = best;
    if (unsorted_pairs) *unsorted_pairs = bad;
    c->arena.reset();
    return PFP_OK;
}

static int sacak_int_impl(const uint32_t *s, void *SA, uint64_t n, uint64_t k, bool u64)
{
    if (!s || !SA || n == 0) return -1;
    if (n + 64 >= 0xFFFFFFFFULL) return -1;
    int st = 0;
    pfp_ctx *c = pfp_create(10, 100, 0, 0, (uint64_t)(80 * n + (32ULL << 20)), &st);
    if (!c) return -1;
    int rounds = -1;
    do {
        if (ensure_arena(c, n) != PFP_OK) break;
        uint32_t *dS = (uint32_t *)c->arena.alloc_lo(n * 4), *dSA = (uint32_t *)c->arena.alloc_lo(n * 4), *dR = (uint32_t *)c->arena.alloc_lo(n * 4);
        if (!dS || !dSA || !dR) break;
        if (hipMemcpy(dS, s, n * 4, hipMemcpyHostToDevice) != hipSuccess) break;
        int r = 0;
        if (sort_int_suffixes(c, dS, n, k ? k - 1 : 0, dSA, dR, &r) != PFP_OK) break;
        if (hipStreamSynchronize(c->stream) != hipSuccess) break;
        if (!u64) { if (hipMemcpy(SA, dSA, n * 4, hipMemcpyDeviceToHost) != hipSuccess) break; }
        else {
            std::vector<uint32_t> tmp((size_t)n);
            if (hipMemcpy(tmp.data(), dSA, n * 4, hipMemcpyDeviceToHost) != hipSuccess) break;
            for (uint64_t i = 0; i < n; ++i) ((uint64_t *)SA)[i] = tmp[(size_t)i];
        }
        rounds = r;
    } while (0);
    pfp_destroy(c);
    return rounds;
}
extern "C++" {
template <typename LT> __global__ __launch_bounds__(BLOCK) void k_gsa_lcp(const uint8_t *D, const uint32_t *SA, const uint32_t *M, uint64_t n, LT *lcp)
{
    const uint64_t i = (uint64_t)blockIdx.x * BLOCK + threadIdx.x;
    if (i >= n) return;
    if (i == 0) { lcp[0] = 0; return; }
    const uint64_t x = SA[i - 1], y = SA[i];
    uint64_t h = 0;
    for (;;) {
        const uint64_t px = x + h, py = y + h;
        if (px >= n || py >= n) break;
        const uint8_t cx = D[px];
        if (cx != D[py] || cx <= EndOfWord) break;
        const uint32_t ix = (uint32_t)(n - 1 - px), iy = (uint32_t)(n - 1 - py);
        const uint64_t rx = ix - M[ix] + 1u, ry = iy - M[iy] + 1u;
        if (rx >= 16 && ry >= 16) { h += rx < ry ? rx : ry; continue; }
        const uint64_t a = ld8(D + px), b = ld8(D + py);
        const uint64_t stop = (a ^ b) | (((a - 0x0202020202020202ULL) & ~a & 0x8080808080808080ULL));
        if (stop) { h += (uint64_t)(__ffsll((long long)stop) - 1) >> 3; break; }
        h += 8;
    }
    lcp[i] = (LT)h;
}
template <typename LT> __global__ __launch_bounds__(BLOCK) void k_gsa_da(const uint32_t *SA, const uint32_t *wordid, uint64_t n, LT *da)
{
    const uint64_t i = (uint64_t)blockIdx.x * BLOCK + threadIdx.x;
    if (i < n) da[i] = (LT)wordid[SA[i]];
}
static int gsacak_impl(const uint8_t *s, void *SA, void *LCP, void *DA, uint64_t n, bool u64)
{
    if (!s || !SA || n < 2) return -1;
    if (n + 64 >= 0xFFFFFFFFULL) return -1;
    bool seen[256] = {false};
    for (uint64_t i = 0; i < n; ++i) seen[s[i]] = true;
    if (s[n - 1] != 0) return -1;
    for (uint64_t i = 0; i + 1 < n; ++i) if (s[i] == 0) return -1;
    bool dict_alphabet = true;
    for (int b = 3; b < 256; ++b) if (seen[b] && !(b == '-' || b == 'A' || b == 'C' || b == 'G' || b == 'N' || b == 'T')) dict_alphabet = false;
    uint8_t code[256]; uint32_t sigma = 2;
    for (int b = 0; b < 256; ++b) code[b] = (uint8_t)(b <= 1 ? b : 0);
    for (int b = 2; b < 256; ++b) if (seen[b]) code[b] = (uint8_t)sigma++;
    uint32_t chars = 0; { unsigned __int128 v = 1; while (chars < 16 && v * sigma < ((unsigned __int128)1 << 51)) { v *= sigma; ++chars; } }
    int st = 0;
    pfp_ctx *c = pfp_create(10, 100, u64 ? PFP_FLAG_U64 : 0u, 0, (uint64_t)(72 * n + (64ULL << 20)), &st);
    if (!c) return -1;
    int rounds = -1;
    auto body = [&]() -> int {
        PFP_TRY(ensure_arena(c, n));
        c->arena.reset();
        c->dsize = n;
        PFP_ALLOC_LO(c, c->d_dict, uint8_t, n + 16);
        PFP_HIP(c, hipMemsetAsync(c->d_dict + n, 0, 16, c->stream));
        PFP_TRY(h2d_copy(c, c->d_dict, s, n));
        uint64_t *k0, *k1; uint32_t *v0, *v1;
        PFP_ALLOC_LO(c, c->d_gsa, uint32_t, n); PFP_ALLOC_LO(c, c->d_grank, uint2, n);
        const size_t mk = c->arena.mark_hi();
        PFP_ALLOC_HI(c, k0, uint64_t, n); PFP_ALLOC_HI(c, k1, uint64_t, n); PFP_ALLOC_HI(c, v0, uint32_t, n); PFP_ALLOC_HI(c, v1, uint32_t, n);
        if (dict_alphabet) {
            PFP_LAUNCH(c, K_SS_INIT_KEYS, n * 13, k_dict_init_keys, nblocks(n, DK_TILE), (const uint8_t *)c->d_dict, n, k0, v0);
            BitRange full = {0, DK_KEY_BITS};
            PFP_TRY(suffix_sort_doubling<true>(c, n, k0, v0, k1, v1, &full, 1, DK_CHARS, c->d_dict, c->d_gsa, (uint32_t *)nullptr, c->d_grank, &rounds));
        } else {
            uint8_t *d_code; PFP_ALLOC_HI(c, d_code, uint8_t, 256);
            PFP_HIP(c, hipMemcpyAsync(d_code, code, 256, hipMemcpyHostToDevice, c->stream));
            PFP_HIP(c, hipStreamSynchronize(c->stream));
            PFP_LAUNCH(c, K_SS_INIT_KEYS, n * 13, k_dict_init_keys_any, nblocks(n, BLOCK), (const uint8_t *)c->d_dict, n, (const uint8_t *)d_code, sigma, chars, k0, v0);
            BitRange full = {0, 51};
            PFP_TRY(suffix_sort_doubling<true>(c, n, k0, v0, k1, v1, &full, 1, chars, c->d_dict, c->d_gsa, (uint32_t *)nullptr, c->d_grank, &rounds, sigma));
        }
        c->arena.release_hi(mk);
        PFP_HIP(c, hipStreamSynchronize(c->stream));
        if (!u64) PFP_HIP(c, hipMemcpy(SA, c->d_gsa, n * 4, hipMemcpyDeviceToHost));
        else PFP_TRY(get_u32_as(c, c->d_gsa, n, SA, true));
        if (LCP) {
            uint32_t *M; PFP_ALLOC_HI(c, M, uint32_t, n);
            PFP_LAUNCH(c, K_MISC, n * 5, k_ss_runend_marks, nblocks(n, BLOCK), (const uint8_t *)c->d_dict, n, M);
            PFP_TRY((device_scan<uint32_t, 1>(c, M, M, n, nullptr)));
            if (u64) { int64_t *d; PFP_ALLOC_HI(c, d, int64_t, n); PFP_LAUNCH(c, K_MISC, n * 40, (k_gsa_lcp<int64_t>), nblocks(n, BLOCK), (const uint8_t *)c->d_dict, (const uint32_t *)c->d_gsa, (const uint32_t *)M, n, d);
                       PFP_HIP(c, hipStreamSynchronize(c->stream)); PFP_HIP(c, hipMemcpy(LCP, d, n * 8, hipMemcpyDeviceToHost)); }
            else { int32_t *d; PFP_ALLOC_HI(c, d, int32_t, n); PFP_LAUNCH(c, K_MISC, n * 36, (k_gsa_lcp<int32_t>), nblocks(n, BLOCK), (const uint8_t *)c->d_dict, (const uint32_t *)c->d_gsa, (const uint32_t *)M, n, d);
                   PFP_HIP(c, hipStreamSynchronize(c->stream)); PFP_HIP(c, hipMemcpy(LCP, d, n * 4, hipMemcpyDeviceToHost)); }
// ... 29 lines not shown
```

### pfbwt-f_amd/python/pfbwt_hip.py

```python
import ctypes as C
import os
import numpy as np

_HERE = os.path.dirname(os.path.abspath(__file__))
DEFAULT_LIB = os.path.join(os.path.dirname(_HERE), "lib", "libpfbwt_hip.so")

PFP_OK = 0
FLAG_U64, FLAG_NON_ACGT_TO_A, FLAG_SAI = 1, 2, 4
DA_ROWS, DA_RUNS = 1, 2
LCP_ROWS, LCP_RUNS = 1, 2
E_ARG = -1
E_INVALID_CHAR, E_TOO_LARGE, E_NOMEM, E_HIP, E_ONE_WORD, E_STATE, E_CORRUPT = -2, -3, -4, -5, -6, -7, -8


class PfpError(RuntimeError):
    def __init__(self, status, msg, pos=None, ch=None):
        super().__init__("pfbwt_hip: %s (status %d)" % (msg, status))
        self.status, self.pos, self.ch = status, pos, ch


class ParseSizes(C.Structure):
    _fields_ = [("n", C.c_uint64), ("m", C.c_uint64), ("dwords", C.c_uint64), ("dsize", C.c_uint64)]


class BwtSizes(C.Structure):
    _fields_ = [("nout", C.c_uint64), ("r", C.c_uint64), ("easy_cases", C.c_uint64), ("hard_cases", C.c_uint64)]


class ShardView(C.Structure):
    _fields_ = [("n", C.c_uint64), ("m", C.c_uint64), ("dwords", C.c_uint64), ("dsize", C.c_uint64),
                ("d_dict", C.c_void_p), ("d_ws", C.c_void_p), ("d_pid", C.c_void_p), ("d_ye", C.c_void_p), ("d_last", C.c_void_p),
                ("left_context", C.c_uint64)]

    def nbytes(self, compact=False):
        return [self.dsize, 4 * (self.dwords + 1), 4 * self.m] + ([] if compact else [8 * self.m, self.m])


_libs = {}


class ThrInfo(C.Structure):
    _fields_ = [("runs", C.c_uint64), ("none", C.c_uint64), ("long_queries", C.c_uint64), ("max_span", C.c_uint64)]


class MsInfo(C.Structure):
    _fields_ = [(k, C.c_uint64) for k in ("patterns", "bases", "match", "up", "down", "absent", "breaks", "long_breaks", "max_len")]


class LcpInfo(C.Structure):
    _fields_ = [("pairs", C.c_uint64), ("max_lcp", C.c_uint64), ("sum_lcp", C.c_uint64), ("long_pairs", C.c_uint64)]


class IngestInfo(C.Structure):
    _fields_ = [("raw_bytes", C.c_uint64), ("records", C.c_uint64), ("n", C.c_uint64), ("read_wait_ms", C.c_double), ("total_ms", C.c_double), ("mode", C.c_int)]


def load_library(path=None):
    path = os.path.abspath(path or os.environ.get("PFBWT_HIP_LIB") or DEFAULT_LIB)
    if path in _libs:
        return _libs[path]
    if not os.path.exists(path):
        raise OSError("HIP library %s not built: run `make -C pfbwt-f_amd` (hipcc --offload-arch=gfx950)" % path)
    L = C.CDLL(path)
    vp, u64, i32 = C.c_void_p, C.c_uint64, C.c_int
    L.pfp_create.restype = vp
    L.pfp_create.argtypes = [i32, u64, C.c_uint, i32, u64, C.POINTER(i32)]
    L.pfp_destroy.argtypes = [vp]
    L.pfp_destroy.restype = None
    L.pfp_strerror.restype = C.c_char_p
    L.pfp_strerror.argtypes = [i32]
    L.pfp_backend.restype = C.c_char_p
    L.pfp_error_detail.argtypes = [vp, C.POINTER(u64), C.POINTER(i32)]
    L.pfp_workspace_needed.restype = u64
    L.pfp_workspace_needed.argtypes = [vp]
    L.pfp_reset.argtypes = [vp]
    L.pfp_parse_feed.argtypes = [vp, vp, u64, i32]
    L.pfp_parse_feed_batch.argtypes = [vp, vp, u64, u64, u64]
    L.pfp_parse_feed_device.argtypes = [vp, vp, u64, i32]
    L.pfp_parse_finalize.argtypes = [vp, C.POINTER(ParseSizes)]
    L.pfp_parse_finalize_shard.argtypes = [vp, C.POINTER(ParseSizes)]
    L.pfp_parse_get.argtypes = [vp, vp, vp, vp, vp, vp]
    L.pfp_parse_bwt.argtypes = [vp]
    L.pfp_parse_bwt_get.argtypes = [vp, vp, vp, vp]
    L.pfp_bwt_load.argtypes = [vp, vp, u64, vp, u64, vp, vp, vp, u64, u64]
    L.pfp_bwt_build.argtypes = [vp, i32, i32, C.POINTER(BwtSizes)]
    L.pfp_parse_feed_device_batch.argtypes = [vp, vp, u64, u64, u64]
    L.pfp_bwt_build_slice.argtypes = [vp, i32, i32, i32, i32, C.POINTER(BwtSizes), C.POINTER(u64), C.POINTER(u64), C.POINTER(u64)]
    L.pfp_bwt_get.argtypes = [vp, vp, vp, vp, vp]
    L.pfp_bwt_device_ptrs.argtypes = [vp, C.POINTER(vp), C.POINTER(vp), C.POINTER(vp), C.POINTER(vp)]
    L.pfp_shard_view_get.argtypes = [vp, C.POINTER(ShardView)]
    L.pfp_parse_feed_left_context.argtypes = [vp]
    L.pfp_shard_load.argtypes = [vp, vp, u64, vp, u64]
    L.pfp_device_copy.argtypes = [vp, vp, vp, u64]
    L.pfp_merge_shards.argtypes = [vp, i32, C.POINTER(ShardView), C.POINTER(ParseSizes)]
    L.pfp_sacak_int_u32.argtypes = [vp, vp, C.c_uint32, C.c_uint32]
    L.pfp_sacak_int_u64.argtypes = [vp, vp, u64, u64]
    L.pfp_marker_array.argtypes = [vp, vp, u64, vp, u64, C.POINTER(u64)]
    L.pfp_marker_array_get.argtypes = [vp, vp]
    L.pfp_gsacak_u32.argtypes = [vp, vp, vp, vp, C.c_uint32]
    L.pfp_gsacak_u64.argtypes = [vp, vp, vp, vp, u64]
    L.pfp_profile_enable.argtypes = [vp, i32]
    L.pfp_profile_reset.argtypes = [vp]
    L.pfp_profile_select.argtypes = [vp, C.c_char_p]
    L.pfp_profile_get.argtypes = [vp, i32, C.POINTER(C.c_char_p), C.POINTER(u64), C.POINTER(C.c_double), C.POINTER(C.c_double)]
    L.pfp_stage_ms.argtypes = [vp, C.POINTER(C.c_double)]
    L.pfp_debug_set.argtypes = [vp, C.c_char_p, C.c_longlong]
    L.pfp_parse_feed_fasta.argtypes = [vp, vp, u64, C.c_uint, C.POINTER(u64)]
    L.pfp_parse_fasta_records.argtypes = [vp, vp, vp]
    L.pfp_parse_reserve.argtypes = [vp, u64]
    L.pfp_parse_feed_fasta_file.argtypes = [vp, C.c_char_p, C.c_uint, C.POINTER(IngestInfo)]
    L.pfp_bwt_build_stream.argtypes = [vp, i32, i32, vp, vp, C.POINTER(BwtSizes)]
    L.pfp_text_length.argtypes = [vp, C.POINTER(u64)]
    L.pfp_bwt_get_expanded.argtypes = [vp, vp, vp, i32]
    L.pfp_text_view.argtypes = [vp, C.POINTER(vp), C.POINTER(u64)]
    L.pfp_host_register.argtypes = [vp, u64]
    L.pfp_host_unregister.argtypes = [vp]
    L.pfp_debug_wordsum.argtypes = [vp, vp, u64, C.POINTER(u64)]
    L.pfp_debug_check_sample_order.argtypes = [vp, C.POINTER(u64)]
    L.pfp_debug_check_sa.argtypes = [vp, C.POINTER(u64)]
    L.pfp_parse_feed_device_view.argtypes = [vp, vp, u64, u64, u64]
    L.pfp_debug_check_samples.argtypes = [vp, C.POINTER(u64)]
    L.pfp_sharded_create.restype = vp
    L.pfp_sharded_create.argtypes = [i32, u64, C.c_uint, i32, C.POINTER(i32), u64, C.POINTER(i32)]
    L.pfp_sharded_destroy.argtypes = [vp]; L.pfp_sharded_destroy.restype = None
    L.pfp_sharded_ctx.restype = vp; L.pfp_sharded_ctx.argtypes = [vp, i32]
    L.pfp_sharded_ranks.argtypes = [vp]
    L.pfp_sharded_build.argtypes = [vp, i32, i32, vp, vp, C.POINTER(u64), C.POINTER(u64), C.POINTER(u64)]
    L.pfp_sharded_reset.argtypes = [vp]
    L.pfp_sharded_error.restype = C.c_char_p; L.pfp_sharded_error.argtypes = [vp]
    L.pfp_parse_docs.argtypes = [vp, C.POINTER(u64)]
    L.pfp_parse_doc_get.argtypes = [vp, u64, C.POINTER(C.c_char_p), C.POINTER(u64)]
    L.pfp_doc_array.argtypes = [vp, vp, u64, C.c_uint]
    L.pfp_doc_array_get.argtypes = [vp, vp, vp, vp]
    L.pfp_doc_array_device_ptrs.argtypes = [vp, C.POINTER(vp), C.POINTER(vp), C.POINTER(vp)]
    L.pfp_doc_array_write.argtypes = [vp, i32, i32, i32]
    L.pfp_lcp_array.argtypes = [vp, C.c_uint, C.POINTER(LcpInfo)]
    L.pfp_lcp_array_get.argtypes = [vp, vp, vp]
    L.pfp_lcp_array_device_ptrs.argtypes = [vp, C.POINTER(vp), C.POINTER(vp)]
    L.pfp_lcp_array_write.argtypes = [vp, i32, i32]
    L.pfp_thresholds.argtypes = [vp, C.POINTER(ThrInfo)]
    L.pfp_thresholds_get.argtypes = [vp, vp, vp]
    L.pfp_thresholds_device_ptrs.argtypes = [vp, C.POINTER(vp), C.POINTER(vp)]
    L.pfp_thresholds_write.argtypes = [vp, i32, i32]
    L.pfp_thresholds_windowed.argtypes = [vp, u64, C.POINTER(ThrInfo), C.POINTER(u64)]
    L.pfp_debug_rows_windowed.argtypes = [vp, u64, vp, vp]
    L.pfp_ms_index.argtypes = [vp]
    L.pfp_ms_query.argtypes = [vp, vp, vp, u64, C.POINTER(MsInfo)]
    L.pfp_ms_query_file.argtypes = [vp, C.c_char_p, C.POINTER(MsInfo)]
    L.pfp_ms_offsets_get.argtypes = [vp, vp, C.POINTER(u64)]
    L.pfp_ms_get.argtypes = [vp, vp, vp]
    L.pfp_ms_device_ptrs.argtypes = [vp, C.POINTER(vp), C.POINTER(vp)]
    L.pfp_ms_write.argtypes = [vp, i32, i32]
    _libs[path] = L
    return L


def _ptr(a):
    return None if a is None else a.ctypes.data_as(C.c_void_p)


class PfpContext:

    def __init__(self, w=10, p=100, u64=True, non_acgt_to_a=False, sai=True, device=0, workspace_bytes=0, lib=None):
        self.L = load_library(lib)
        self.u64 = bool(u64)
        self.udt = np.uint64 if u64 else np.uint32
        flags = (FLAG_U64 if u64 else 0) | (FLAG_NON_ACGT_TO_A if non_acgt_to_a else 0) | (FLAG_SAI if sai else 0)
        self.sai = bool(sai)
        st = C.c_int(0)
        self.h = self.L.pfp_create(int(w), int(p), flags, int(device), int(workspace_bytes), C.byref(st))
        if not self.h:
            raise PfpError(st.value, self.L.pfp_strerror(st.value).decode())
        self.sizes = None
        self.bsizes = None

    def debug_set(self, **switches):
        for k, v in switches.items():
            self._check(self.L.pfp_debug_set(self.h, k.encode(), int(v)))

    def close(self):
        if getattr(self, "h", None):
            if not getattr(self, "_borrowed", False):
                self.L.pfp_destroy(self.h)
            self.h = None

    def __del__(self):
        try:
            self.close()
        except Exception:
            pass

    def _check(self, st):
        if st != PFP_OK:
            pos, ch = C.c_uint64(0), C.c_int(0)
            self.L.pfp_error_detail(self.h, C.byref(pos), C.byref(ch))
            raise PfpError(st, self.L.pfp_strerror(st).decode(), pos.value, ch.value)

    def reset(self):
        self._check(self.L.pfp_reset(self.h))

    def feed(self, bases, end_of_seq=True):
        a = np.frombuffer(bases, dtype=np.uint8) if isinstance(bases, (bytes, bytearray, memoryview)) else np.ascontiguousarray(bases, dtype=np.uint8)
        self._check(self.L.pfp_parse_feed(self.h, _ptr(a) if a.size else None, a.size, 1 if end_of_seq else 0))

    def reserve(self, text_bytes):
        self._check(self.L.pfp_parse_reserve(self.h, int(text_bytes)))

    def feed_fasta(self, raw, final=True, records=False, ptr=None, nbytes=None):
        if ptr is None:
            a = np.frombuffer(raw, dtype=np.uint8) if isinstance(raw, (bytes, bytearray, memoryview)) else np.ascontiguousarray(raw, dtype=np.uint8)
            ptr, nbytes = a.ctypes.data, a.size
        nrec = C.c_uint64(0)
        self._check(self.L.pfp_parse_feed_fasta(self.h, C.c_void_p(ptr), int(nbytes), (1 if final else 0) | (2 if records else 0), C.byref(nrec)))
        if not records:
            return None
        ro = np.empty(nrec.value, np.uint64); tp = np.empty(nrec.value, np.uint64)
        self._check(self.L.pfp_parse_fasta_records(self.h, _ptr(ro), _ptr(tp)))
        return ro, tp

    def feed_fasta_file(self, path, records=False):
        info = IngestInfo()
        self._check(self.L.pfp_parse_feed_fasta_file(self.h, os.fsencode(path), 2 if records else 0, C.byref(info)))
        return info

    def text_length(self):
        n = C.c_uint64(0); self._check(self.L.pfp_text_length(self.h, C.byref(n))); return n.value

    def bwt_build_stream(self, host_bwt_ptr, host_sa_ptr=None, rssa=False):
        b = BwtSizes()
        self._check(self.L.pfp_bwt_build_stream(self.h, 1 if host_sa_ptr else 0, 1 if rssa else 0, C.c_void_p(host_bwt_ptr), C.c_void_p(host_sa_ptr) if host_sa_ptr else None, C.byref(b)))
        self.bsizes, self._want, self._rows, self.esa_pairs = b, (bool(host_sa_ptr), bool(rssa)), b.nout, b.r
        return b

    def check_sample_order(self):
        o = (C.c_uint64 * 5)()
        self._check(self.L.pfp_debug_check_sample_order(self.h, o))
        return {"pairs": int(o[0]), "order_violations": int(o[1]), "rows_not_adjacent": int(o[2]), "max_lcp": int(o[3]), "mean_lcp": (int(o[4]) / int(o[0])) if o[0] else 0.0}

    def check_sa(self):
        o = (C.c_uint64 * 5)()
        self._check(self.L.pfp_debug_check_sa(self.h, o))
        return {"rows": int(o[0]), "out_of_range": int(o[1]), "duplicates": int(o[2]), "bwt_mismatches": int(o[3]), "eos_bytes": int(o[4])}

    def check_samples(self):
        o = (C.c_uint64 * 3)()
        self._check(self.L.pfp_debug_check_samples(self.h, o))
        return {"runs": int(o[0]), "row_errors": int(o[1]), "value_errors": int(o[2])}

    def bwt_get_expanded(self, host_bwt_ptr, ssa=None, threads=16):
        self._check(self.L.pfp_bwt_get_expanded(self.h, C.c_void_p(host_bwt_ptr), _ptr(ssa), int(threads)))

    def samples_get(self, out=None):
        b = self.bsizes
        ssa = out["ssa"] if out else np.empty(2 * b.r, self.udt); esa = out["esa"] if out else np.empty(2 * b.r, self.udt)
        self._check(self.L.pfp_bwt_get(self.h, None, None, _ptr(ssa), _ptr(esa)))
        return ssa, esa

    def feed_host_batch(self, host_ptr, count, length, stride):
        self._check(self.L.pfp_parse_feed_batch(self.h, C.c_void_p(int(host_ptr)), int(count), int(length), int(stride)))

    def feed_device_view(self, dptr, count, length, stride):
        self._check(self.L.pfp_parse_feed_device_view(self.h, C.c_void_p(int(dptr)), int(count), int(length), int(stride)))

    def feed_device(self, dptr, nbytes, end_of_seq=True):
        self._check(self.L.pfp_parse_feed_device(self.h, C.c_void_p(int(dptr)), int(nbytes), 1 if end_of_seq else 0))

    def finalize(self, shard=False):
        s = ParseSizes()
        self._check((self.L.pfp_parse_finalize_shard if shard else self.L.pfp_parse_finalize)(self.h, C.byref(s)))
        self.sizes = s
        return s

    def parse_get(self):
        s = self.sizes
        out = {"dict": np.empty(s.dsize, np.uint8), "occ": np.empty(s.dwords, self.udt), "parse": np.empty(s.m, np.uint32),
               "last": np.empty(s.m, np.uint8), "sai": np.empty(s.m, self.udt) if self.sai else None}
        self._check(self.L.pfp_parse_get(self.h, _ptr(out["dict"]), _ptr(out["occ"]), _ptr(out["parse"]), _ptr(out["last"]), _ptr(out["sai"])))
        return out

    def parse_bwt(self):
        self._check(self.L.pfp_parse_bwt(self.h))

    def parse_bwt_get(self):
        nr = self.sizes.m + 1
        out = {"bwlast": np.empty(nr, np.uint8), "ilist": np.empty(nr, self.udt), "bwsai": np.empty(nr, self.udt) if self.sai else None}
        self._check(self.L.pfp_parse_bwt_get(self.h, _ptr(out["bwlast"]), _ptr(out["ilist"]), _ptr(out["bwsai"])))
        return out

    def feed_device_batch(self, dev_ptr, count, length, stride):
        self._check(self.L.pfp_parse_feed_device_batch(self.h, C.c_void_p(int(dev_ptr)), int(count), int(length), int(stride)))

    def feed_left_context(self, w=None):
        self._check(self.L.pfp_parse_feed_left_context(self.h))

    def shard_load(self, dict_image, parse):
        d = np.ascontiguousarray(dict_image, np.uint8); p = np.ascontiguousarray(parse, np.uint32)
        self._check(self.L.pfp_shard_load(self.h, _ptr(d), d.size, _ptr(p), p.size))

    def shard_view(self):
        v = ShardView()
        self._check(self.L.pfp_shard_view_get(self.h, C.byref(v)))
        return v

    def device_copy(self, dst_ptr, src_ptr, nbytes):
        self._check(self.L.pfp_device_copy(self.h, C.c_void_p(int(dst_ptr)), C.c_void_p(int(src_ptr)), int(nbytes)))

    def merge_shards(self, views):
        arr = (ShardView * len(views))(*views)
        s = ParseSizes()
        self._check(self.L.pfp_merge_shards(self.h, len(views), arr, C.byref(s)))
        self.sizes = s
        return s

    def bwt_load(self, dict_, occ, bwlast, ilist, bwsai=None, n_hint=0):
        d = np.ascontiguousarray(dict_, np.uint8); o = np.ascontiguousarray(occ, self.udt)
        bl = np.ascontiguousarray(bwlast, np.uint8); il = np.ascontiguousarray(ilist, self.udt)
        bs = None if bwsai is None else np.ascontiguousarray(bwsai, self.udt)
        if il.size != bl.size or (bs is not None and bs.size != bl.size):
            raise PfpError(E_CORRUPT, "bwlast / ilist / bwsai hold different numbers of rows")
        self._check(self.L.pfp_bwt_load(self.h, _ptr(d), d.size, _ptr(o), o.size, _ptr(bl), _ptr(il), _ptr(bs), bl.size, int(n_hint)))

    def bwt_build(self, sa=True, rssa=False):
        b = BwtSizes()
        self._check(self.L.pfp_bwt_build(self.h, 1 if sa else 0, 1 if rssa else 0, C.byref(b)))
        self.bsizes, self._want, self._rows, self.esa_pairs = b, (bool(sa), bool(rssa)), b.nout, b.r
        return b

    def bwt_build_slice(self, slice_index, nslices, sa=True, rssa=False):
        b = BwtSizes(); beg, rows, ep = C.c_uint64(0), C.c_uint64(0), C.c_uint64(0)
        self._check(self.L.pfp_bwt_build_slice(self.h, 1 if sa else 0, 1 if rssa else 0, int(slice_index), int(nslices), C.byref(b), C.byref(beg), C.byref(rows), C.byref(ep)))
        self.bsizes, self._want, self._rows, self.esa_pairs = b, (bool(sa), bool(rssa)), rows.value, ep.value
        return b, beg.value, rows.value

    def bwt_get(self, out=None):
        b = self.bsizes
        sa, rssa = self._want
        if out is not None:
            need = {"bwt": self._rows, "sa": self._rows if sa else None, "ssa": 2 * b.r if rssa else None, "esa": 2 * getattr(self, "esa_pairs", b.r) if rssa else None}
            for k, cnt in need.items():
                if cnt is not None and (out.get(k) is None or out[k].size < cnt or out[k].dtype != (np.uint8 if k == "bwt" else self.udt)):
                    raise ValueError("bwt_get: out[%r] missing, too small or of the wrong type" % k)
            self._check(self.L.pfp_bwt_get(self.h, _ptr(out["bwt"]), _ptr(out["sa"]) if sa else None, _ptr(out["ssa"]) if rssa else None, _ptr(out["esa"]) if rssa else None))
            return out
        out = {"bwt": np.empty(self._rows, np.uint8), "sa": np.empty(self._rows, self.udt) if sa else None,
               "ssa": np.empty(2 * b.r, self.udt) if rssa else None, "esa": np.empty(2 * getattr(self, "esa_pairs", b.r), self.udt) if rssa else None}
        self._check(self.L.pfp_bwt_get(self.h, _ptr(out["bwt"]), _ptr(out["sa"]), _ptr(out["ssa"]), _ptr(out["esa"])))
        return out

    def bwt_device_ptrs(self):
        p = [C.c_void_p(0) for _ in range(4)]
        self._check(self.L.pfp_bwt_device_ptrs(self.h, *[C.byref(x) for x in p]))
        return [x.value for x in p]

    def marker_array(self, mps, sa=None):
        mps = np.ascontiguousarray(mps, np.uint64)
        n = C.c_uint64(0)
        if sa is None:
            self._check(self.L.pfp_marker_array(self.h, _ptr(mps), mps.size, None, 0, C.byref(n)))
        else:
            sa = np.ascontiguousarray(sa, self.udt)
            self._check(self.L.pfp_marker_array(self.h, _ptr(mps), mps.size, _ptr(sa), sa.size, C.byref(n)))
        out = np.empty(n.value, np.uint64)
        self._check(self.L.pfp_marker_array_get(self.h, _ptr(out) if n.value else None))
        return out

    def doc_array(self, starts, rows=True, runs=True):
        st = np.ascontiguousarray(starts, np.uint64)
        self._check(self.L.pfp_doc_array(self.h, _ptr(st), st.size, (DA_ROWS if rows else 0) | (DA_RUNS if runs else 0)))
        b = self.bsizes
        da = np.empty(self._rows, self.udt) if rows else None
        sda = np.empty(2 * b.r, self.udt) if runs else None
        eda = np.empty(2 * getattr(self, "esa_pairs", b.r), self.udt) if runs else None
        self._check(self.L.pfp_doc_array_get(self.h, _ptr(da), _ptr(sda), _ptr(eda)))
        return da, sda, eda

    def doc_array_device_ptrs(self):
        p = [C.c_void_p(0) for _ in range(3)]
        self._check(self.L.pfp_doc_array_device_ptrs(self.h, *[C.byref(x) for x in p]))
        return [x.value for x in p]

    def lcp_array(self, rows=True, runs=True):
        inf = LcpInfo()
        self._check(self.L.pfp_lcp_array(self.h, (LCP_ROWS if rows else 0) | (LCP_RUNS if runs else 0), C.byref(inf)))
        lcp = np.empty(self._rows, self.udt) if rows else None
        slcp = np.empty(2 * self.bsizes.r, self.udt) if runs else None
        self._check(self.L.pfp_lcp_array_get(self.h, _ptr(lcp), _ptr(slcp)))
        return lcp, slcp, {k: int(getattr(inf, k)) for k, _ in LcpInfo._fields_}

    def lcp_array_device_ptrs(self):
        p = [C.c_void_p(0) for _ in range(2)]
        self._check(self.L.pfp_lcp_array_device_ptrs(self.h, *[C.byref(x) for x in p]))
        return [x.value for x in p]

    def thresholds(self):
        inf = ThrInfo()
        self._check(self.L.pfp_thresholds(self.h, C.byref(inf)))
        thr = np.empty(2 * self.bsizes.r, self.udt)
        tlcp = np.empty(2 * self.bsizes.r, self.udt)
        self._check(self.L.pfp_thresholds_get(self.h, _ptr(thr), _ptr(tlcp)))
        return thr, tlcp, {k: int(getattr(inf, k)) for k, _ in ThrInfo._fields_}

# ... 161 lines not shown
```

Before: 136.7 Gbases/s.

## Skip ranking of majority-byte rows in multi-member emit groups

Adds a pre-pass that finds, for each non-uniform multi-member group, the BWT byte covering the most rows, and records it in a per-slot fill array used by the later fill pass. The group-emission kernel then ranks by bisection only the minority-byte rows. Majority rows are left to the fill, with group boundary and neighbour qrow values written explicitly so run-boundary samples stay exact. This targets the per-row binary searches across group members, at the cost of an extra kernel, a device copy of s_pc, rank-statistics atomics and a launch-bounds occupancy hint.

Result: no change. 136.6 Gbases/s (-0.0%).

```diff
diff --git a/include/pfbwt_hip_dev.h b/include/pfbwt_hip_dev.h
--- a/include/pfbwt_hip_dev.h
+++ b/include/pfbwt_hip_dev.h
@@ -18,6 +18,7 @@
 int pfp_debug_check_sample_order(pfp_ctx *ctx, uint64_t out[5]);
 int pfp_debug_check_sa(pfp_ctx *ctx, uint64_t out[5]);
 int pfp_debug_check_samples(pfp_ctx *ctx, uint64_t out[3]);
+int pfp_debug_emit_rank_stat(pfp_ctx *ctx, uint64_t out[5]);
 int pfp_debug_rows_windowed(pfp_ctx *ctx, uint64_t window_rows, void *host_sa, void *host_lcp);
 int pfp_debug_wordsum(pfp_ctx *ctx, const void *d_buf, uint64_t bytes, uint64_t out[2]);
 
diff --git a/pfbwt-f_amd/csrc/common.h b/pfbwt-f_amd/csrc/common.h
--- a/pfbwt-f_amd/csrc/common.h
+++ b/pfbwt-f_amd/csrc/common.h
@@ -93,6 +93,8 @@
     uint32_t fill_subs = 2;
     int fill_masks = 1;
     int fill_skip = 1;
+    int rank_minority = 1;
+    int rank_stat_detail = 0;
     uint64_t sample_cap = ~0ULL;
     int no_runaware = 0;
     long big_group_members = -2;
@@ -165,6 +167,7 @@
     uint8_t *d_bwlast = nullptr; uint32_t *d_ilist = nullptr; uint64_t *d_bwsai = nullptr;
     uint8_t *d_bwl_il = nullptr;
     uint64_t nout = 0, runs = 0, esa_pairs = 0, easy = 0, hard = 0, slice_begin = 0, slice_rows = 0;
+    uint64_t emit_rank_stat[5] = {0, 0, 0, 0, 0};
     uint8_t *d_bwt = nullptr; void *d_sa = nullptr; void *d_ssa = nullptr; void *d_esa = nullptr;
     bool have_sa = false, have_rssa = false;
     pfp::ResultSlot ma; uint64_t ma_words = 0;
diff --git a/pfbwt-f_amd/csrc/emit.h b/pfbwt-f_amd/csrc/emit.h
--- a/pfbwt-f_amd/csrc/emit.h
+++ b/pfbwt-f_amd/csrc/emit.h
@@ -160,9 +160,12 @@
     const unsigned long long *cgb = nullptr;
     const uint32_t *town = nullptr;
     uint32_t *lglist = nullptr; unsigned long long *lgcount = nullptr; uint64_t lgcap = 0; int qpasses = 0 ;
+    const uint8_t *s_fill = nullptr; int rank_all = 1; int rstat_detail = 0 ;
+    unsigned long long *rstat = nullptr;
     unsigned long long *gstat = nullptr;
 };
 constexpr uint8_t SF_MULTI = 1, SF_FULL = 2, SF_BIG = 4, SF_GFULL = 8, SF_NONUNI = 16, SF_E0 = 32;
+constexpr uint32_t CI_MAJ = 1u << 24;
 __device__ __forceinline__ bool slot_is_special(uint32_t fl) { return (fl & (SF_FULL | SF_GFULL | SF_NONUNI)) != 0; }
 constexpr int EG_SLOTS = 2 * BLOCK;
 constexpr uint32_t BIG_GROUP_MEMBERS = 64;
@@ -697,6 +700,26 @@
     cinfo[j] = make_uint4(S.x, multi ? group_members(a, S) : 1u, multi ? i - S.z : 0u, (uint32_t)a.s_pc[i] | (fl << 8));
     cgb[j] = (unsigned long long)reinterpret_cast<const EBT *>(a.EB)[multi ? S.z : i];
 }
+template <typename EBT> __global__ __launch_bounds__(BLOCK) void k_group_majority(EmitArgs a, uint32_t nsp, uint4 *cinfo, uint8_t *s_fill)
+{
+    const uint64_t j = (uint64_t)blockIdx.x * BLOCK + threadIdx.x;
+    if (j >= nsp) return;
+    const EBT *ENB = reinterpret_cast<const EBT *>(a.ENB);
+    const uint4 ci = cinfo[j];
+    const uint32_t fl = (ci.w >> 8) & 0xFFu, k = ci.y;
+    if (!(fl & SF_MULTI) || !(fl & SF_NONUNI) || (fl & (SF_GFULL | SF_BIG)) || ci.z != 0u || k > (uint32_t)EG_SLOTS || j + k > (uint64_t)nsp) return;
+    uint64_t best = 0; uint32_t bestc = 0;
+    for (uint32_t code = 0; code < 9u; ++code) {
+        const uint32_t b = dict_byte4(code);
+        uint64_t rows = 0;
+        for (uint32_t m = 0; m < k; ++m) if ((cinfo[j + m].w & 0xFFu) == b) rows += (uint64_t)ENB[j + m + 1] - (uint64_t)ENB[j + m];
+        if (rows > best) { best = rows; bestc = b; }
+    }
+    for (uint32_t m = 0; m < k; ++m) {
+        cinfo[j + m].w = (cinfo[j + m].w & 0xFFFFu) | (bestc << 16) | CI_MAJ;
+        s_fill[a.elist[j + m]] = (uint8_t)bestc;
+    }
+}
 template <typename EBT> __device__ __forceinline__ uint64_t group_start_at_or_after(const EBT *ENB, const uint4 *cinfo, uint64_t nsp, uint64_t lo, uint64_t v)
 {
     while (lo < nsp && (uint64_t)ENB[lo] < v) ++lo;
@@ -712,14 +735,16 @@
     if (t > ntiles) return;
     town[t] = (uint32_t)group_start_at_or_after<EBT>(ENB, cinfo, nsp, etile_slot[t], t * EMIT_TILE);
 }
-template <typename EBT> __global__ __launch_bounds__(BLOCK) void k_emit_groups(EmitArgs a, uint8_t *bwt, uint32_t *qrow)
+template <typename EBT, bool MINOR > __global__ __launch_bounds__(BLOCK, 4) void k_emit_groups(EmitArgs a, uint8_t *bwt, uint32_t *qrow)
 {
     __shared__ uint32_t LQ[EG_BUF];
     __shared__ uint32_t s_eb[EG_SLOTS + 1], s_fb[EG_SLOTS], s_kf[EG_SLOTS], s_dl[EG_SLOTS];
     __shared__ uint64_t s_ob[EG_SLOTS];
     __shared__ uint8_t s_pc[EG_SLOTS];
+    __shared__ uint8_t s_md[EG_SLOTS];
     __shared__ uint32_t red[4];
     __shared__ uint64_t jb[2];
+    __shared__ uint32_t s_cnt[5];
     const EBT *ENB = reinterpret_cast<const EBT *>(a.ENB);
     const uint64_t tile0 = a.e0 / EMIT_TILE, tb = tile0 + blockIdx.x;
     const uint64_t o0 = tb * EMIT_TILE > a.e0 ? tb * EMIT_TILE : a.e0;
@@ -738,6 +763,7 @@
         }
         jb[threadIdx.x] = j;
     }
+    if (threadIdx.x < 5) s_cnt[threadIdx.x] = 0;
     __syncthreads();
     uint64_t j = jb[0]; const uint64_t jE = jb[1];
     const uint32_t cap = a.group_rows_cap < (uint32_t)EG_BUF ? a.group_rows_cap : (uint32_t)EG_BUF;
@@ -755,6 +781,7 @@
                 s_eb[s] = e0 < 0xFFFFFFFFull ? (uint32_t)e0 : 0xFFFFFFFFu;
                 if (s + 1 == nload) s_eb[nload] = e1 < 0xFFFFFFFFull ? (uint32_t)e1 : 0xFFFFFFFFu;
                 s_fb[s] = ci.x; s_kf[s] = (k < 0xFFFFFFu ? k : 0xFFFFFFu) | (fl << 24); s_dl[s] = dl; s_pc[s] = (uint8_t)ci.w;
+                s_md[s] = (!MINOR || !(ci.w & CI_MAJ)) ? (uint8_t)0 : ((ci.w >> 16) & 0xFFu) == (ci.w & 0xFFu) ? (uint8_t)2 : (uint8_t)1;
                 s_ob[s] = (uint64_t)a.cgb[j + s];
                 if (((fl & (SF_GFULL | SF_BIG)) || k > a.rank_members_max) && s < bad) bad = s;
                 if (dl + 1u == k && e1 <= (uint64_t)cap) cand[t] = s + 1u;
@@ -803,6 +830,16 @@
         const uint32_t nrows = s_eb[cut];
 #pragma unroll
         for (int t = 0; t < 2; ++t) { const uint32_t s = threadIdx.x + (uint32_t)t * BLOCK; if (s < cut) s_ob[s] -= (uint64_t)s_eb[s - s_dl[s]]; }
+        if (a.rstat) {
+            uint32_t g = 0, rk = 0;
+#pragma unroll
+            for (int t = 0; t < 2; ++t) {
+                const uint32_t s = threadIdx.x + (uint32_t)t * BLOCK;
+                if (s < cut && ((s_kf[s] >> 24) & SF_MULTI)) { const uint32_t rows = s_eb[s + 1] - s_eb[s]; g += rows; if (s_md[s] != 2) rk += rows; }
+            }
+            for (int d = WAVE / 2; d >= 1; d >>= 1) { g += __shfl_down(g, (unsigned)d); rk += __shfl_down(rk, (unsigned)d); }
+            if ((threadIdx.x & (WAVE - 1)) == 0 && g) { atomicAdd(&s_cnt[0], rk); atomicAdd(&s_cnt[1], g); }
+        }
         uint32_t qv[EG_PER_THREAD], sv[EG_PER_THREAD]; uint8_t cv[EG_PER_THREAD];
 #pragma unroll
         for (int it = 0; it < EG_PER_THREAD; ++it) {
@@ -820,6 +857,7 @@
             if (r < nrows) { LQ[r] = qv[it]; const uint32_t fl = s_kf[sv[it]] >> 24; if (fl & SF_MULTI) cv[it] = s_pc[sv[it]]; else if (!a.bwl_il) cv[it] = a.bwlast[qv[it]]; }
         }
         __syncthreads();
+        if constexpr (!MINOR) {
 #pragma unroll
         for (int it = 0; it < EG_PER_THREAD; ++it) {
             const uint32_t r = threadIdx.x + (uint32_t)it * BLOCK;
@@ -840,9 +878,61 @@
                 if (o >= a.w0 && o < a.w1) bwt[o - a.w0] = cv[it];
             }
         }
+        } else {
+#pragma unroll
+        for (int it = 0; it < EG_PER_THREAD; ++it) {
+            const uint32_t r = threadIdx.x + (uint32_t)it * BLOCK;
+            if (r < nrows) {
+                const uint32_t s = sv[it], kf = s_kf[s], q = LQ[r];
+                uint32_t pos = r;
+                if ((kf >> 24) & SF_MULTI) {
+                    const uint32_t sh = s - s_dl[s], k = kf & 0xFFFFFFu, md = s_md[s];
+                    const uint32_t gb = s_eb[sh], ge = s_eb[sh + k];
+                    if (md && qrow && r == gb) {
+                        uint32_t mn = 0xFFFFFFFFu, mx = 0u;
+                        for (uint32_t mm = 0; mm < k; ++mm) {
+                            const uint32_t b = s_eb[sh + mm], e = s_eb[sh + mm + 1];
+                            if (e > b) { const uint32_t h = LQ[b], t = LQ[e - 1]; mn = h < mn ? h : mn; mx = t > mx ? t : mx; }
+                        }
+                        qrow[B0 - a.q0 + gb] = mn; qrow[B0 - a.q0 + ge - 1u] = mx;
+                    }
+                    if (md == 2u) continue;
+                    uint32_t before = 0, pq = 0u, sq = 0xFFFFFFFFu, sqm = s;
+                    for (uint32_t mm = 0; mm < k; ++mm) {
+                        const uint32_t sm = sh + mm;
+                        if (sm != s) {
+                            const uint32_t b = s_eb[sm], len = s_eb[sm + 1] - b, lb = lower_bound_u32(LQ + b, len, q);
+                            before += lb;
+                            if (md) {
+                                if (lb) { const uint32_t v = LQ[b + lb - 1u]; pq = v > pq ? v : pq; }
+                                if (lb < len) { const uint32_t v = LQ[b + lb]; if (v < sq) { sq = v; sqm = sm; } }
+                            }
+                        }
+                    }
+                    pos = gb + before + (r - s_eb[s]);
+                    if (md) {
+                        if (r > s_eb[s]) { const uint32_t v = LQ[r - 1u]; pq = v > pq ? v : pq; }
+                        if (r + 1u < s_eb[s + 1]) { const uint32_t v = LQ[r + 1u]; if (v < sq) { sq = v; sqm = s; } }
+                        if (qrow) {
+                            if (pos > gb) qrow[B0 - a.q0 + pos - 1u] = pq;
+                            if (pos + 1u < ge) qrow[B0 - a.q0 + pos + 1u] = sq;
+                        }
+                        if (a.rstat_detail) {
+                            if (pos == gb) atomicAdd(&s_cnt[2], 1u);
+                            if (pos + 1u == ge) atomicAdd(&s_cnt[3], 1u); else if (s_md[sqm] == 1u) atomicAdd(&s_cnt[4], 1u);
+                        }
+                    }
+                }
+                if (qrow) qrow[B0 - a.q0 + pos] = q;
+                const uint64_t o = s_ob[s] + pos;
+                if (o >= a.w0 && o < a.w1) bwt[o - a.w0] = cv[it];
+            }
+        }
+        }
         __syncthreads();
         j += cut;
     }
+    if (a.rstat && threadIdx.x < 5 && s_cnt[threadIdx.x]) atomicAdd(&a.rstat[threadIdx.x], (unsigned long long)s_cnt[threadIdx.x]);
 }
 
 template <int ITEMS> __device__ __forceinline__ void lds_sort_pairs_u32(uint32_t *keys, uint16_t *vals, uint32_t n, int npass, uint32_t (*wh)[RS_RADIX], uint32_t *red)
@@ -1001,7 +1091,7 @@
             const uint32_t k = k0 + threadIdx.x;
             const EBT cn = k < ns ? cnt[i0 + k] : (EBT)0;
             const uint64_t e = k < ns ? (uint64_t)EB[i0 + k] : 0ULL;
-            const uint8_t pc = k < ns ? a.s_pc[i0 + k] : (uint8_t)0;
+            const uint8_t pc = k < ns ? a.s_fill[i0 + k] : (uint8_t)0;
             const bool has = cn != 0;
             const unsigned long long bal = __ballot(has);
             __syncthreads();
diff --git a/pfbwt-f_amd/csrc/emit_host.h b/pfbwt-f_amd/csrc/emit_host.h
--- a/pfbwt-f_amd/csrc/emit_host.h
+++ b/pfbwt-f_amd/csrc/emit_host.h
@@ -17,6 +17,15 @@
 {
     const uint64_t k = (uint64_t)nslices, s = (uint64_t)slice;
     return total / k * s + (total % k) * s / k;
+}
+static void fetch_rank_stat(pfp_ctx *c, const unsigned long long *d_rstat)
+{
+    unsigned long long h[5];
+    if (hipStreamSynchronize(c->stream) != hipSuccess || hipMemcpy(h, d_rstat, 40, hipMemcpyDeviceToHost) != hipSuccess) return;
+    for (int x = 0; x < 5; ++x) c->emit_rank_stat[x] = h[x];
+    if (c->tun.verbose)
+        fprintf(stderr, "[pfbwt_hip] group-stationary emission (counted once per window that enumerates a group): %llu rows ranked by bisection of %llu rows of multi-member groups taken in batches (%.4f); ranked rows first / last of their group %llu / %llu, followed by another ranked row %llu\n",
+                h[0], h[1], h[1] ? (double)h[0] / (double)h[1] : 0.0, h[2], h[3], h[4]);
 }
 static void print_left_rows(const unsigned long long *d_gstat)
 {
@@ -54,6 +63,8 @@
         PFP_TRY(plan_windows());
         PFP_TRY(alloc_routes());
         struct LeftRows { const EmitArgs &ea; ~LeftRows() { if (ea.gstat) print_left_rows(ea.gstat); } } left_rows{ea};
+        if (!visit) for (uint64_t &v : c->emit_rank_stat) v = 0;
+        struct RankStat { pfp_ctx *c; const EmitArgs &ea; bool publish; ~RankStat() { if (ea.rstat && publish) fetch_rank_stat(c, ea.rstat); } } rank_stat{c, ea, !visit};
         if (visit) return run_visit();
         if (!want_rssa || keep_sa) return run_bwt_then_exact_samples(false);
         bool overflow = false;
@@ -110,12 +121,14 @@
             PFP_ALLOC_HI(c, ea.gleft, uint8_t, (size_t)ea.ecount + 1); PFP_ALLOC_HI(c, ea.tile_left, uint8_t, max_etiles);
             PFP_HIP(c, hipMemsetAsync(ea.gleft, 0, (size_t)ea.ecount + 1, c->stream));
         }
+        ea.rstat_detail = (c->tun.verbose || c->tun.rank_stat_detail) ? 1 : 0;
         ea.qpasses = (bits_for(c->nrows ? c->nrows : 0xFFFFFFFFULL) + 7) / 8;
         if (ea.gleft) {
             const uint32_t cap = ea.group_rows_cap < (uint32_t)EG_BUF ? ea.group_rows_cap : (uint32_t)EG_BUF;
             ea.lgcap = maxq / cap + 2;
             PFP_ALLOC_HI(c, ea.lglist, uint32_t, 2 * ea.lgcap); PFP_ALLOC_HI(c, ea.lgcount, unsigned long long, 2);
         }
+        if (ea.gleft) { PFP_ALLOC_HI(c, ea.rstat, unsigned long long, 5); PFP_HIP(c, hipMemsetAsync(ea.rstat, 0, 40, c->stream)); }
         if (ea.gleft && c->tun.verbose) { PFP_ALLOC_HI(c, ea.gstat, unsigned long long, 12); PFP_HIP(c, hipMemsetAsync(ea.gstat, 0, 96, c->stream)); }
         return PFP_OK;
     }
@@ -144,7 +157,8 @@
         if (ea.gleft) {
             PFP_HIP(c, hipMemsetAsync(ea.tile_left, 0, (size_t)ge, c->stream));
             PFP_HIP(c, hipMemsetAsync(ea.lgcount, 0, 16, c->stream));
-            PFP_LAUNCH(c, K_EMIT, (ea.e1 - ea.e0) * (1 + 4 + (q_at ? 4 : 0)), (k_emit_groups<EBT>), ge, ea, bwt_at, q_at);
+            if (ea.rank_all) PFP_LAUNCH(c, K_EMIT, (ea.e1 - ea.e0) * (1 + 4 + (q_at ? 4 : 0)), (k_emit_groups<EBT, false>), ge, ea, bwt_at, q_at);
+            else PFP_LAUNCH(c, K_EMIT, (ea.e1 - ea.e0) * (1 + 4 + (q_at ? 4 : 0)), (k_emit_groups<EBT, true>), ge, ea, bwt_at, q_at);
             PFP_LAUNCH(c, K_EMIT_LARGE, 0, (k_emit_groups_large<EBT, EG1_BUF>), ge < 1024u ? ge : 1024u, ea, bwt_at, q_at);
             PFP_LAUNCH(c, K_EMIT_LARGE, 0, (k_emit_groups_large<EBT, EG2_BUF>), ge < 512u ? ge : 512u, ea, bwt_at, q_at);
             PFP_LAUNCH(c, K_EMIT_BIG, 0, (k_emit<SAT, EBT>), ge, ea, bwt_at, (SAT *)nullptr, q_at);
@@ -421,6 +435,12 @@
             PFP_LAUNCH(c, K_EMIT_COUNT, (uint64_t)nsp * 50, (k_special_pack<EBT>), nblocks(nsp, BLOCK), ea, nsp, cinfo, cgb);
             PFP_LAUNCH(c, K_EMIT_COUNT, (ntiles2 + 1) * 40, (k_tile_own<EBT>), nblocks(ntiles2 + 1, BLOCK), (const EBT *)ENBc, (const uint4 *)cinfo, (const uint32_t *)ea.etile_slot, (uint64_t)nsp, ntiles2, town);
             ea.cinfo = cinfo; ea.cgb = cgb; ea.town = town;
+            if (c->tun.rank_minority) {
+                uint8_t *s_fill; PFP_ALLOC_HI(c, s_fill, uint8_t, dsize);
+                PFP_HIP(c, hipMemcpyAsync(s_fill, ea.s_pc, dsize, hipMemcpyDeviceToDevice, c->stream));
+                PFP_LAUNCH(c, K_EMIT_COUNT, (uint64_t)nsp * 40, (k_group_majority<EBT>), nblocks(nsp, BLOCK), ea, nsp, cinfo, s_fill);
+                ea.s_fill = s_fill; ea.rank_all = 0;
+            }
         }
         return PFP_OK;
     }
@@ -489,7 +509,7 @@
         ea.use_e0 = (c->n != 0 && c->n + (uint64_t)c->w + 2 < 0xFFFFFFFFULL && !c->tun.no_slot_records) ? 1 : 0;
     }
     ea.wordid = c->d_wordid; ea.use_prec = (maxlen < (1u << PREC_SL_BITS) && !c->tun.no_slot_records) ? 1 : 0;
-    ea.s_sl = s_sl; ea.s_fb = s_fb; ea.s_fl = s_fl; ea.s_pc = s_pc;
+    ea.s_sl = s_sl; ea.s_fb = s_fb; ea.s_fl = s_fl; ea.s_pc = s_pc; ea.s_fill = s_pc;
     if (!visit) { c->have_sa = want_sa != 0; c->have_rssa = want_rssa != 0; }
     const bool force_wide = c->tun.force_wide_rows != 0;
     const bool wide = force_wide || c->n == 0 || c->n + 2 >= 0xFFFFFFFFULL;
diff --git a/pfbwt-f_amd/csrc/pfbwt_hip.hip b/pfbwt-f_amd/csrc/pfbwt_hip.hip
--- a/pfbwt-f_amd/csrc/pfbwt_hip.hip
+++ b/pfbwt-f_amd/csrc/pfbwt_hip.hip
@@ -88,7 +88,7 @@
 
 static const char *const tunable_names[] = {"verbose", "seg_grid", "seg_stage", "sort_k", "sort_no_table", "class_sort_maxrange", "dedup_table_log2", "no_trigger_table",
                                             "emit_chunk_rows", "fill_subs", "sample_cap", "no_runaware", "big_group_members", "force_wide_rows", "fasta_chunk_bytes", "ingest_block_bytes", "emit_group_rows", "no_slot_records", "dict_text_rounds", "int_key_symbols", "force_run_round",
-                                            "ingest_readers", "expand_dma", "parse_rec", "parse_rec_p2", "parse_rec_min", "parse_rec_depth", "parse_rec_tile_rows", "parse_rec_table_log2", "dict_rec", "dict_rec_p2", "dedup_variant", "dedup_phases", "dedup_period", "dedup_chunk", "doc_lds_max", "dedup_packed", "group_reduce", "scan_waves", "lcp_long_min", "thr_long_min", "thr_tile", "thr_window_rows", "plcp_block_log2", "fill_masks", "fill_skip", "ms_dir_log2", "ms_long_min"};
+                                            "ingest_readers", "expand_dma", "parse_rec", "parse_rec_p2", "parse_rec_min", "parse_rec_depth", "parse_rec_tile_rows", "parse_rec_table_log2", "dict_rec", "dict_rec_p2", "dedup_variant", "dedup_phases", "dedup_period", "dedup_chunk", "doc_lds_max", "dedup_packed", "group_reduce", "scan_waves", "lcp_long_min", "thr_long_min", "thr_tile", "thr_window_rows", "plcp_block_log2", "fill_masks", "fill_skip", "rank_minority", "rank_stat_detail", "ms_dir_log2", "ms_long_min"};
 static int set_tunable(pfp_ctx *c, const char *key, long long v)
 {
     Tunables &t = c->tun;
@@ -104,6 +104,8 @@
     else if (!strcmp(key, "fill_subs")) t.fill_subs = (uint32_t)v;
     else if (!strcmp(key, "fill_masks")) t.fill_masks = (int)v;
     else if (!strcmp(key, "fill_skip")) t.fill_skip = (int)v;
+    else if (!strcmp(key, "rank_minority")) t.rank_minority = (int)v;
+    else if (!strcmp(key, "rank_stat_detail")) t.rank_stat_detail = (int)v;
     else if (!strcmp(key, "sample_cap")) t.sample_cap = v < 0 ? ~0ULL : (uint64_t)v;
     else if (!strcmp(key, "no_runaware")) t.no_runaware = (int)v;
     else if (!strcmp(key, "big_group_members")) t.big_group_members = (long)v;
@@ -1683,6 +1685,13 @@
     out[0] = r; out[1] = h[1]; out[2] = h[2];
     return PFP_OK;
 }
+int pfp_debug_emit_rank_stat(pfp_ctx *c, uint64_t out[5])
+{
+    if (!c || !out) return PFP_E_ARG;
+    if (c->stage < 3) return PFP_E_STATE;
+    for (int x = 0; x < 5; ++x) out[x] = c->emit_rank_stat[x];
+    return PFP_OK;
+}
 int pfp_host_register(void *p, uint64_t bytes) { if (!p || !bytes) return PFP_E_ARG; if (hipHostRegister(p, (size_t)bytes, hipHostRegisterDefault) != hipSuccess) { (void)hipGetLastError(); return PFP_E_HIP; } return PFP_OK; }
 int pfp_host_unregister(void *p) { if (!p) return PFP_E_ARG; if (hipHostUnregister(p) != hipSuccess) { (void)hipGetLastError(); return PFP_E_HIP; } return PFP_OK; }
 
diff --git a/pfbwt-f_amd/python/pfbwt_hip.py b/pfbwt-f_amd/python/pfbwt_hip.py
--- a/pfbwt-f_amd/python/pfbwt_hip.py
+++ b/pfbwt-f_amd/python/pfbwt_hip.py
@@ -120,6 +120,8 @@
     L.pfp_debug_check_sa.argtypes = [vp, C.POINTER(u64)]
     L.pfp_parse_feed_device_view.argtypes = [vp, vp, u64, u64, u64]
     L.pfp_debug_check_samples.argtypes = [vp, C.POINTER(u64)]
+    if hasattr(L, "pfp_debug_emit_rank_stat"):
+        L.pfp_debug_emit_rank_stat.argtypes = [vp, C.POINTER(u64)]
     L.pfp_sharded_create.restype = vp
     L.pfp_sharded_create.argtypes = [i32, u64, C.c_uint, i32, C.POINTER(i32), u64, C.POINTER(i32)]
     L.pfp_sharded_destroy.argtypes = [vp]; L.pfp_sharded_destroy.restype = None
@@ -247,6 +249,11 @@
         self._check(self.L.pfp_debug_check_samples(self.h, o))
         return {"runs": int(o[0]), "row_errors": int(o[1]), "value_errors": int(o[2])}
 
+    def emit_rank_stat(self):
+        o = (C.c_uint64 * 5)()
+        self._check(self.L.pfp_debug_emit_rank_stat(self.h, o))
+        return {"ranked": int(o[0]), "group_rows": int(o[1]), "ranked_first": int(o[2]), "ranked_last": int(o[3]), "ranked_adjacent": int(o[4])}
+
     def bwt_get_expanded(self, host_bwt_ptr, ssa=None, threads=16):
         self._check(self.L.pfp_bwt_get_expanded(self.h, C.c_void_p(host_bwt_ptr), _ptr(ssa), int(threads)))
 
```
